# soedinglab/plass

Hardware: AMD Instinct MI355X
Metric: read-overlaps/s per assembly iteration (higher is better)
Workload: dtype u8/u64 (integer hash, byte compare; f32 ratios)

## Files before the change

plass_amd/csrc/asm_rules.hpp:

```cpp
#pragma once
#include <cmath>
#include <cstdlib>
#if defined(__HIPCC__)
#define PLASSHIP_AR_HD __host__ __device__ __forceinline__
#else
#define PLASSHIP_AR_HD static inline __attribute__((always_inline))
#endif
namespace plasship {

struct AlnCoords { int qStart, qEnd, dbStart, dbEnd; };
struct DiagSpan { bool hit = false; unsigned qo = 0, to = 0, len = 0; };

PLASSHIP_AR_HD int alnLengthOf(int qStart, int qEnd, int dbStart, int dbEnd) {
    const int aq = (qStart == -1) ? 0 : qStart, ad = (dbStart == -1) ? 0 : dbStart;
    const int dq = abs(qEnd - aq), dd = abs(dbEnd - ad);
    return (dq > dd ? dq : dd) + 1;
}
PLASSHIP_AR_HD int rawScoreOfBits(int bitScore, double ln2, double logK, double lambda) {
    return (int) (fma((double) bitScore, ln2, logK) / lambda + 0.5);
}
template <typename S> PLASSHIP_AR_HD int scorePerCol100(S score, unsigned alnLen) {
    const float scorePerCol = (float) score / (float) ((double) alnLen + 0.5);
    return (int) (scorePerCol * 100);
}
PLASSHIP_AR_HD DiagSpan diagonalSpan(int diag, unsigned qLen, unsigned tLen) {
    const unsigned dist = (unsigned) abs(diag);
    DiagSpan s;
    if (diag >= 0 && dist < qLen) { s.hit = true; s.qo = dist; s.len = tLen < qLen - dist ? tLen : qLen - dist; }
    else if (diag < 0 && dist < tLen) { s.hit = true; s.to = dist; s.len = tLen - dist < qLen ? tLen - dist : qLen; }
    return s;
}
template <typename F> PLASSHIP_AR_HD void forEachWrap(unsigned d16, unsigned qLen, unsigned tLen, F &&f) {
    for (unsigned j = 1; j <= 1u + tLen / 32768u; j++) {
        const int real = (int) (d16 - j * 65536u);
        const DiagSpan s = diagonalSpan(real, qLen, tLen);
        if (s.hit) f(real, s);
    }
    for (unsigned j = 0; j <= qLen / 65536u; j++) {
        const int real = (int) (j * 65536u + d16);
        const DiagSpan s = diagonalSpan(real, qLen, tLen);
        if (s.hit) f(real, s);
    }
}
PLASSHIP_AR_HD AlnCoords alnOnDiagonal(int diag, int startPos, int endPos) {
    const int dist = abs(diag);
    AlnCoords c;
    if (diag >= 0) { c.qStart = startPos + dist; c.qEnd = endPos + dist; c.dbStart = startPos; c.dbEnd = endPos; }
    else { c.qStart = startPos; c.qEnd = endPos; c.dbStart = startPos + dist; c.dbEnd = endPos + dist; }
    return c;
}
PLASSHIP_AR_HD float rescoredSeqId(int ids, int qStart, int qEnd) {
    return (float) ids / ((float) qEnd - (float) qStart);
}
PLASSHIP_AR_HD bool isBranchType(int qStart, int qEnd, unsigned qLen, int dbStart, int dbEnd, unsigned dbLen) {
    const bool notBoth = !(dbStart == 0 && qStart == 0);
    const bool rightStart = dbStart == 0 && (dbEnd != (int) dbLen - 1);
    const bool leftStart = qStart == 0 && (qEnd != (int) qLen - 1);
    return (rightStart || leftStart) && notBoth;
}
PLASSHIP_AR_HD unsigned rightFragLen(unsigned tLen, int dbEnd) { return tLen - ((unsigned) dbEnd + 1); }
PLASSHIP_AR_HD bool canExtendRight(unsigned fragR, int qEnd, unsigned qLen) { return fragR > 0 && (unsigned) qEnd == (qLen - 1); }
PLASSHIP_AR_HD bool canExtendLeft(int dbStart, int dbEnd, unsigned tLen) { return dbStart > 0 && (unsigned) dbEnd == (tLen - 1); }
PLASSHIP_AR_HD bool deferredRight(unsigned fragR, int qEnd, unsigned qLen, unsigned rightOff) {
    return fragR > rightOff && (unsigned) qEnd == (qLen - 1) && rightOff > 0;
}
PLASSHIP_AR_HD bool deferredLeft(int dbStart, int dbEnd, unsigned tLen, unsigned leftOff) {
    return dbStart > (int) leftOff && (unsigned) dbEnd == (tLen - 1) && leftOff > 0;
}
PLASSHIP_AR_HD AlnCoords mirrorReverseHit(int qStart, int qEnd, int dbStart, int dbEnd, unsigned dbLen) {
    AlnCoords c;
    c.qStart = qEnd; c.qEnd = qStart;
    c.dbStart = (int) (dbLen - (unsigned) dbEnd - 1); c.dbEnd = (int) (dbLen - (unsigned) dbStart - 1);
    return c;
}

}
```

plass_amd/csrc/assemble.hip:

```cpp
#include "common.hpp"
#include "device_utils.hpp"
#include "posterior_class.hpp"
#include "ref_rules.hpp"
#include "asm_rules.hpp"
#include "host_util.hpp"
#include <algorithm>
#include <memory>
#include <cstring>

namespace plasship {

struct Item {
    uint32_t target; int32_t score; uint32_t alnLength; float seqId;
    int32_t qStart, qEnd; uint32_t qLen; int32_t dbStart, dbEnd; uint32_t dbLen;
    uint32_t state;
    uint32_t pad;
};

struct AsmArgs {
    SeqView s;
    const uint64_t *qoff; const AlnRec *recs;
    Item *items;
    const uint64_t *arenaOff;
    const uint32_t *leftCap;
// ... 894 lines not shown
                        curLen += fragLen; rightOff += fragLen;
                        if (GUIDED) {
                            const unsigned aaFrag = (tLen / 3 - dbEnd / 3) - 1;
                            if (aaStart + aaLen + aaFrag > a.aaArenaOff[id + 1] - a.aaArenaOff[id]) atomicAdd(&a.stats[12], 1ull);
                            else { copyBytesSerial(aaBuf + aaStart + aaLen, aaT + dbEnd / 3 + 1, aaFrag); aaLen += aaFrag; }
                        }
                        used[nUsed++] = best.target;
                    } else if (qStart == 0 && dbEnd == (tLen - 1)) {
                        if (leftOff > 0) { def[nDef++] = bi; continue; }
                        const unsigned fragLen = dbStart;
                        if (curLen + fragLen >= a.maxSeqLen) { brokeOut = true; break; }
                        if (!copied) { job[0].dst = buf + curStart; job[0].src = orig; job[0].n = origLen; job[0].rev = 0; copied = true; }
                        curStart -= fragLen;
                        job[2].dst = buf + curStart; job[2].src = rev ? tSeq + (tLen - dbStart) : tSeq; job[2].n = fragLen; job[2].rev = rev ? 1u : 0u;
                        curLen += fragLen; leftOff += fragLen;
                        if (GUIDED) {
                            const unsigned aaFrag = fragLen / 3 + ((aaT[0] == '*') ? 1u : 0u);
                            if (aaFrag > aaStart) atomicAdd(&a.stats[12], 1ull);
                            else { aaStart -= aaFrag; copyBytesSerial(aaBuf + aaStart, aaT, aaFrag); aaLen += aaFrag; }
                        }
                        used[nUsed++] = best.target;
                    }
                }
                if (cmp.abort) active = false;
            }
#pragma unroll
            for (int k = 0; k < 3; k++) {
                unsigned long long m = __ballot(job[k].n > 0);
                while (m) {
                    const int j = __ffsll((long long) m) - 1; m &= m - 1;
                    char *dst = bcast(job[k].dst, j); const char *src = bcast(job[k].src, j);
                    const unsigned n = bcast(job[k].n, j), rv = bcast(job[k].rev, j);
                    if (rv) copyRevCompWave(dst, src, n, sComp, lane); else copyBytesG<64>(dst, src, n, lane);
                }
            }
            waveMemSync();
            if (active) {
                if (leftOff > 0 || rightOff > 0) couldExtend = true;
                if (brokeOut && nHeap > 0) active = false;
            }
            querySeqLen = (unsigned) curLen;
            const char *qs = buf + curStart;
            const uint32_t myDef = active ? nDef : 0u;
            uint32_t maxDef = myDef;
#pragma unroll
            for (int o = 32; o > 0; o >>= 1) maxDef = max(maxDef, (uint32_t) __shfl_xor((int) maxDef, o, 64));
            for (uint32_t d = 0; d < maxDef; d++) {
                const bool mine = d < myDef && !cmp.abort;
                uint32_t found = 0; Item x; memset(&x, 0, sizeof(x));
                const char *tSeq = nullptr; unsigned tLen = 0; int diag = 0; DiagSpan sp;
                if (mine) {
                    found = def[d];
                    x = it[found];
                    tSeq = a.s.data + seqOff(a.s, x.target);
                    tLen = seqLen(a.s, x.target);
                    diag = (int) ((unsigned) x.qStart + leftOff) - x.dbStart;
                    sp = diagonalSpan(diag, querySeqLen, tLen);
                }
                int startPos = -1, endPos = -1, sc = 0, ids = 0;
                unsigned long long m = __ballot(mine && sp.hit && sp.len > 0);
                while (m) {
                    const int j = __ffsll((long long) m) - 1; m &= m - 1;
                    const char *jq = bcast(qs + sp.qo, j); const char *jt = bcast(tSeq, j);
                    const unsigned jTo = bcast(sp.to, j), jLen = bcast(sp.len, j), jTLen = bcast(tLen, j), jRev = bcast((unsigned) x.pad, j);
                    unsigned first = 0, last = 0; int s = 0, idn = 0;
                    if (jRev) scoreColumnsRevWave(jq, jt, jTLen - 1 - jTo, jLen, smat, sComp, lane, first, last, s, idn);
                    else scoreColumnsG<64>(jq, jt + jTo, jLen, smat, lane, first, last, s, idn);
                    s = waveReduceSum(s); idn = waveReduceSum(idn);
                    if (lane == j) { startPos = (int) first; endPos = (int) last; sc = s; ids = idn; }
                }
                if (mine) {
                    const unsigned score = (unsigned) max(sc, 0);
                    qResc++; qRescRes += sp.len;
                    const AlnCoords c = alnOnDiagonal(diag, startPos, endPos);
                    const float seqId = rescoredSeqId(ids, c.qStart, c.qEnd);
                    x.seqId = seqId; x.qLen = querySeqLen; x.dbLen = tLen; x.alnLength = sp.len;
                    x.score = scorePerCol100(score, x.alnLength);
                    x.qStart = c.qStart; x.qEnd = c.qEnd; x.dbStart = c.dbStart; x.dbEnd = c.dbEnd;
                    it[found] = x;
                    if (seqId >= a.seqIdThr) heapPush(hp, nHeap, found, it, cmp);
                }
            }
            active = active && nHeap > 0 && !cmp.abort;
        }
        if (valid) {
            if (cmp.abort) a.redoList[atomicAdd(a.redoCount, 1u)] = id;
            else {
                nAln += h; nQRes += seqLen(a.s, id); nResc += qResc; nRescRes += qRescRes;
                for (uint32_t i = 0; i < nUsed; i++) atomicOr(&a.flags[used[i]], 0x80u);
                if (couldExtend) {
                    atomicOr(&a.flags[id], 0x20u); a.newLen[id] = (uint32_t) curLen; a.newStart[id] = aoff + curStart;
                    if (GUIDED) { a.aaNewLen[id] = (uint32_t) aaLen; a.aaNewStart[id] = a.aaArenaOff[id] + aaStart; }
                    nExt++;
                }
            }
        }
    }
    nExt = waveReduceSumU64(nExt); nResc = waveReduceSumU64(nResc); nRescRes = waveReduceSumU64(nRescRes); nAln = waveReduceSumU64(nAln); nQRes = waveReduceSumU64(nQRes);
    if (laneId() == 0) {
        if (nExt) atomicAdd(&a.stats[0], nExt); if (nResc) atomicAdd(&a.stats[1], nResc); if (nRescRes) atomicAdd(&a.stats[2], nRescRes);
        if (nAln) { atomicAdd(&a.stats[3], nAln); atomicAdd(&a.stats[4], nQRes); atomicAdd(&a.stats[5], nRescRes); }
    }
}

template <int G> __device__ __forceinline__ int groupSum(int v) {
    v = rowSum<(G < 16 ? G : 16)>(v);
#pragma unroll
    for (int o = 16; o < G; o <<= 1) v += __shfl_xor(v, o, G);
    return v;
}
template <int G> __device__ __forceinline__ unsigned long long groupMax(unsigned long long v) {
    v = rowMax<(G < 16 ? G : 16)>(v);
#pragma unroll
    for (int o = 16; o < G; o <<= 1) { const unsigned long long ok = __shfl_xor(v, o, G); v = (ok > v) ? ok : v; }
    return v;
}
template <int G> __device__ __forceinline__ uint32_t groupRank(uint32_t mine) {
    if (G == 8) return rowCountLess8(mine);
    uint32_t r = rowCountLess16(mine, mine, false);
#pragma unroll
    for (int o = 16; o < G; o += 16) r += rowCountLess16((uint32_t) __shfl_xor((int) mine, o, G), mine, true);
    return r;
}
template <int G> __device__ __forceinline__ unsigned long long groupBallot(bool p) {
    const unsigned long long m = __ballot(p);
    if (G == 64) return m;
    return (m >> ((laneId() / G) * G)) & ((1ULL << G) - 1ULL);
}

template <int G>
__device__ __forceinline__ Rescored rescoreOnDiagonalG(const char *q, unsigned qLen, const char *t, unsigned tLen, int diagonal,
                                                       const signed char *smat, int gl) {
    Rescored r; r.startPos = -1; r.endPos = -1; r.score = 0; r.diagonalLen = 0; r.idExcl = 0;
    const unsigned dist = (unsigned) abs(diagonal);
    unsigned qo, to, len;
    if (diagonal >= 0 && dist < qLen) { qo = dist; to = 0; len = min(tLen, qLen - dist); }
    else if (diagonal < 0 && dist < tLen) { qo = 0; to = dist; len = min(tLen - dist, qLen); }
    else return r;
    r.diagonalLen = len;
    if (len == 0) return r;
    unsigned first, last;
    int s = 0, ids = 0;
    scoreColumnsG<G>(q + qo, t + to, len, smat, gl, first, last, s, ids);
    s = groupSum<G>(s); ids = groupSum<G>(ids);
    r.score = (unsigned) max(s, 0); r.startPos = (int) first; r.endPos = (int) last; r.idExcl = ids;
    return r;
}

constexpr int ASM8_WPE = 5;
template <int G, int WPE>
__global__ __launch_bounds__(256) __attribute__((amdgpu_waves_per_eu(WPE, WPE))) void assembleGroupKernel(AsmArgs a) {
    __shared__ signed char smat[123 * 123 + 7];
    stageScoreTable(smat, a.mat, 256);
    __syncthreads();
    const int gl = threadIdx.x & (G - 1);
    const uint32_t groupsTotal = gridDim.x * (256 / G);
    const uint32_t nWork = (G == 64) ? a.nMid : ((G == 32) ? a.nMid32 : ((G == 16) ? a.nSmall : a.nNarrow));
    unsigned long long nExt = 0, nResc = 0, nRescRes = 0, nAln = 0, nQRes = 0;
    const uint32_t *workList = (G == 64) ? a.midList : ((G == 32) ? a.mid32List : ((G == 16) ? a.smallList : a.narrowList));
    auto loadWord = [&](uint32_t pid) -> uint64_t {
        uint64_t v = 0;
        if (pid != 0xFFFFFFFFu) {
            if (gl == 0) v = a.qoff[pid]; else if (gl == 1) v = a.qoff[pid + 1]; else if (gl == 2) v = a.arenaOff[pid]; else if (gl == 3) v = a.s.offLen[pid]; else if (gl == 4) v = a.leftCap[pid];
        }
        return v;
    };
    uint32_t w = blockIdx.x * (256 / G) + threadIdx.x / G;
    uint32_t idNext = (w < nWork) ? workList[w] : 0xFFFFFFFFu;
    uint64_t wordNext = loadWord(idNext);
    uint32_t idAhead = (w + groupsTotal < nWork) ? workList[w + groupsTotal] : 0xFFFFFFFFu;
    for (; w < nWork; w += groupsTotal) {
        const uint32_t id = idNext;
        const uint64_t h0 = __shfl(wordNext, 0, G), h1 = __shfl(wordNext, 1, G), aoff = __shfl(wordNext, 2, G), qOffLen = __shfl(wordNext, 3, G), qLeftCap = __shfl(wordNext, 4, G);
        idNext = idAhead; wordNext = loadWord(idNext);
        idAhead = (w + 2u * groupsTotal < nWork) ? workList[w + 2u * groupsTotal] : 0xFFFFFFFFu;
        const uint32_t h = (uint32_t) (h1 - h0);
        const char *orig = a.s.data + (qOffLen >> 24);
        unsigned querySeqLen = (unsigned) ((uint32_t) qOffLen & 0xFFFFFFu);
        if (gl == 0) { nAln += h; nQRes += querySeqLen; }
        uint32_t xTarget = 0xFFFFFFFFu, xAlnLen = 0, xQLen = 0, xDbLen = 0, xState = 2, xTLen = 0; uint64_t xTOff = 0;
        int xScore = 0, xQStart = 0, xQEnd = 0, xDbStart = 0, xDbEnd = 0;
        if ((uint32_t) gl < h) {
            const AlnRec r = a.recs[h0 + gl];
            xTarget = r.target;
            xAlnLen = (uint32_t) alnLengthOf(r.qStart, r.qEnd, r.dbStart, r.dbEnd);
            xScore = scorePerCol100(rawScoreOfBits(r.bitScore, a.ln2, a.logK, a.lambda), xAlnLen);
            xQStart = r.qStart; xQEnd = r.qEnd; xQLen = (uint32_t) r.qLen; xDbStart = r.dbStart; xDbEnd = r.dbEnd; xDbLen = (uint32_t) r.dbLen;
            xState = (xTarget == id || !r.accepted) ? 2u : 0u;
            const bool branchType = ((xDbStart == 0 && xDbEnd != (int) xDbLen - 1) || (xQStart == 0 && xQEnd != (int) xQLen - 1)) && !(xDbStart == 0 && xQStart == 0);
            if (xState == 0 && branchType) { xTOff = seqOff(a.s, xTarget); xTLen = seqLen(a.s, xTarget); }
        }
        const uint32_t tRank = groupRank<G>(xTarget);
        char *buf = a.arena + aoff;
        uint64_t curStart = qLeftCap;
        copyBytesG<G>(buf + curStart, orig, querySeqLen, gl);
        uint64_t curLen = querySeqLen;
        bool couldExtend = false;
        uint32_t inQueue = (uint32_t) __popcll(groupBallot<G>(xState == 0));
        while (inQueue > 0) {
            unsigned leftOff = 0, rightOff = 0;
            bool brokeOut = false;
            if (xState == 1) xState = 2;
            unsigned long long key = 0;
            bool rType = false, lType = false, rBranch = false, lBranch = false;
            unsigned fragR = 0;
            if (xState == 0) {
                key = ((unsigned long long) ((uint32_t) xScore ^ 0x80000000u) << 32) | ((unsigned long long) xAlnLen << 6) | (unsigned long long) (63u - tRank);
                if (isBranchType(xQStart, xQEnd, xQLen, xDbStart, xDbEnd, xDbLen)) {
                    if (xDbStart == 0) { rBranch = true; fragR = rightFragLen(xTLen, xDbEnd); rType = canExtendRight(fragR, xQEnd, querySeqLen); }
                    else if (xQStart == 0) { lBranch = true; lType = canExtendLeft(xDbStart, xDbEnd, xTLen); }
                }
            }
            const unsigned long long bestR = groupMax<G>(rType ? key : 0ULL), bestL = groupMax<G>(lType ? key : 0ULL);
            const bool rFirst = bestR != 0 && bestR > bestL;
            const bool isR = rType && key == bestR, isL = lType && key == bestL;
            auto extendRight = [&]() {
                const int bi = __ffsll((long long) groupBallot<G>(isR)) - 1;
                const char *tSeq = a.s.data + __shfl(xTOff, bi, G);
                const uint32_t bTarget = __shfl(xTarget, bi, G);
                const unsigned fragLen = __shfl(fragR, bi, G), dbEnd = (unsigned) __shfl(xDbEnd, bi, G);
                copyBytesG<G>(buf + curStart + curLen, tSeq + dbEnd + 1, fragLen, gl);
                curLen += fragLen; rightOff += fragLen;
                if (gl == 0) atomicOr(&a.flags[bTarget], 0x80u);
            };
            if (rFirst) extendRight();
            if (bestL != 0) {
                const int bi = __ffsll((long long) groupBallot<G>(isL)) - 1;
                const unsigned fragLen = (unsigned) __shfl(xDbStart, bi, G);
                if (curLen + fragLen >= a.maxSeqLen) brokeOut = true;
                else {
                    const char *tSeq = a.s.data + __shfl(xTOff, bi, G);
                    const uint32_t bTarget = __shfl(xTarget, bi, G);
                    curStart -= fragLen;
                    copyBytesG<G>(buf + curStart, tSeq, fragLen, gl);
                    curLen += fragLen; leftOff += fragLen;
                    if (gl == 0) atomicOr(&a.flags[bTarget], 0x80u);
                }
            }
            if (bestR != 0 && !rFirst && !brokeOut) extendRight();
            if (xState == 0 && (!brokeOut || key >= bestL)) {
                uint32_t st = 2;
                if (!(isR && (rFirst || !brokeOut)) && !isL) {
                    if (rBranch) { if (deferredRight(fragR, xQEnd, querySeqLen, rightOff)) st = 1; }
                    else if (lBranch) { if (deferredLeft(xDbStart, xDbEnd, xTLen, leftOff)) st = 1; }
                }
                xState = st;
            }
            inQueue = (uint32_t) __popcll(groupBallot<G>(xState == 0));
            if (leftOff > 0 || rightOff > 0) couldExtend = true;
            if (brokeOut && inQueue > 0) break;
            querySeqLen = (unsigned) curLen;
            const char *qs = buf + curStart;
            unsigned long long deferred = groupBallot<G>(xState == 1);
            if (deferred) waveMemSync();
            if (G >= 32 && (uint32_t) __popcll(deferred) >= a.ownLaneMin) {
                if (xState == 1) {
                    const char *tSeq = a.s.data + xTOff;
                    const int diag = (int) ((unsigned) xQStart + leftOff) - xDbStart;
                    const DiagSpan sp = diagonalSpan(diag, querySeqLen, xTLen);
                    unsigned first = 0, last = 0; int sc = 0, ids = 0; int startPos = -1, endPos = -1;
                    if (sp.hit && sp.len > 0) { scoreColumnsSerial(qs + sp.qo, tSeq + sp.to, sp.len, smat, first, last, sc, ids); startPos = (int) first; endPos = (int) last; }
                    const unsigned score = (unsigned) max(sc, 0);
                    nResc += 1; nRescRes += sp.len;
                    const AlnCoords c = alnOnDiagonal(diag, startPos, endPos);
                    xQLen = querySeqLen; xDbLen = xTLen; xAlnLen = sp.len; xScore = scorePerCol100(score, sp.len);
                    xQStart = c.qStart; xQEnd = c.qEnd; xDbStart = c.dbStart; xDbEnd = c.dbEnd;
                    xState = (rescoredSeqId(ids, c.qStart, c.qEnd) >= a.seqIdThr) ? 0u : 2u;
                }
                deferred = 0;
            }
            while (deferred) {
                const int dl = __ffsll((long long) deferred) - 1;
                deferred &= deferred - 1;
                const int dqs = __shfl(xQStart, dl, G), dds = __shfl(xDbStart, dl, G);
                const char *tSeq = a.s.data + __shfl(xTOff, dl, G);
                const unsigned tLen = __shfl(xTLen, dl, G);
                const int diag = (int) ((unsigned) dqs + leftOff) - dds;
                const Rescored rs = rescoreOnDiagonalG<G>(qs, querySeqLen, tSeq, tLen, diag, smat, gl);
                nResc += (gl == 0); nRescRes += (gl == 0) ? rs.diagonalLen : 0;
                const AlnCoords c = alnOnDiagonal(diag, rs.startPos, rs.endPos);
                const float seqId = rescoredSeqId(rs.idExcl, c.qStart, c.qEnd);
                if (gl == dl) {
                    xQLen = querySeqLen; xDbLen = tLen; xAlnLen = rs.diagonalLen; xScore = scorePerCol100(rs.score, rs.diagonalLen);
                    xQStart = c.qStart; xQEnd = c.qEnd; xDbStart = c.dbStart; xDbEnd = c.dbEnd;
                    xState = (seqId >= a.seqIdThr) ? 0u : 2u;
                }
            }
            inQueue = (uint32_t) __popcll(groupBallot<G>(xState == 0));
        }
        if (couldExtend) {
            if (gl == 0) { atomicOr(&a.flags[id], 0x20u); a.newLen[id] = (uint32_t) curLen; a.newStart[id] = aoff + curStart; nExt++; }
        }
    }
    nExt = waveReduceSumU64(nExt); nResc = waveReduceSumU64(nResc); nRescRes = waveReduceSumU64(nRescRes); nAln = waveReduceSumU64(nAln); nQRes = waveReduceSumU64(nQRes);
    if (laneId() == 0) {
        if (nExt) atomicAdd(&a.stats[0], nExt); if (nResc) atomicAdd(&a.stats[1], nResc); if (nRescRes) atomicAdd(&a.stats[2], nRescRes);
        const int tier = (G <= 16) ? 0 : 1;
        if (nAln) { atomicAdd(&a.stats[3 + 3 * tier], nAln); atomicAdd(&a.stats[4 + 3 * tier], nQRes); atomicAdd(&a.stats[5 + 3 * tier], nRescRes); }
    }
}

__global__ __launch_bounds__(256) void arenaSumKernel(const AlnRec *__restrict__ recs, uint64_t nAln, uint64_t maxSeqLen, unsigned long long *__restrict__ qSum,
                                                      unsigned long long *__restrict__ qSumAa, uint32_t *__restrict__ qCan, int mirror) {
    const int lane = laneId();
    for (uint64_t i = (uint64_t) blockIdx.x * blockDim.x + threadIdx.x; i < nAln; i += (uint64_t) gridDim.x * blockDim.x) {
        const AlnRec r = recs[i];
        const uint32_t id = r.query;
        uint32_t add = 0, addAa = 0; bool can = false;
        if (r.target != id && r.accepted) {
            add = (uint32_t) r.dbLen; addAa = (uint32_t) r.dbLen / 3 + 2;
            AlnCoords c; c.qStart = r.qStart; c.qEnd = r.qEnd; c.dbStart = r.dbStart; c.dbEnd = r.dbEnd;
            if (mirror && c.qStart > c.qEnd) c = mirrorReverseHit(r.qStart, r.qEnd, r.dbStart, r.dbEnd, (unsigned) r.dbLen);
            if (isBranchType(c.qStart, c.qEnd, (unsigned) r.qLen, c.dbStart, c.dbEnd, (unsigned) r.dbLen)) {
                if (c.dbStart == 0) can = canExtendRight(rightFragLen((unsigned) r.dbLen, c.dbEnd), c.qEnd, (unsigned) r.qLen);
                else if (c.qStart == 0) can = canExtendLeft(c.dbStart, c.dbEnd, (unsigned) r.dbLen) && ((uint64_t) r.qLen + (uint64_t) c.dbStart < maxSeqLen);
            }
        }
        const unsigned long long act = __ballot(1);
        const uint32_t prevId = (uint32_t) __shfl_up((int) id, 1, 64);
        const bool head = lane == 0 || prevId != id;
        const unsigned long long heads = __ballot(head), cans = __ballot(can);
        const int segStart = 63 - __clzll((long long) (heads & (lane == 63 ? ~0ULL : ((2ULL << lane) - 1ULL))));
        const unsigned long long later = lane == 63 ? 0ULL : (heads & ~((2ULL << lane) - 1ULL));
        const int segEnd = (later ? __ffsll((long long) later) - 1 : (int) __popcll(act)) - 1;
#pragma unroll
        for (int d = 1; d < 64; d <<= 1) {
            const uint32_t t = (uint32_t) __shfl_up((int) add, d, 64), ta = (uint32_t) __shfl_up((int) addAa, d, 64);
            if (lane - d >= segStart) { add += t; addAa += ta; }
        }
        if (lane == segEnd) {
            const unsigned long long seg = (segEnd == 63 ? ~0ULL : ((2ULL << segEnd) - 1ULL)) & ~((1ULL << segStart) - 1ULL);
            if (add) atomicAdd(&qSum[id], (unsigned long long) add);
            if (qSumAa && addAa) atomicAdd(&qSumAa[id], (unsigned long long) addAa);
            if (cans & seg) atomicOr(&qCan[id], 1u);
        }
    }
}
constexpr int N_TIERS = 5;
constexpr uint8_t TIER_NARROW = 4, TIER_NONE = 0xFF;
__global__ void arenaSizeKernel(SeqView s, const uint64_t *__restrict__ qoff, const unsigned long long *__restrict__ qSum, const unsigned long long *__restrict__ qSumAa,
                                const uint32_t *__restrict__ qCan, uint32_t *__restrict__ leftCap,
                                uint64_t *__restrict__ bytes, int nuclTiers, uint64_t threadBytes,
                                uint8_t *__restrict__ tierOf,
                                const uint32_t *__restrict__ aaLen, uint32_t *__restrict__ aaLeftCap, uint64_t *__restrict__ aaBytes) {
    for (uint32_t id = blockIdx.x * blockDim.x + threadIdx.x; id < s.n; id += gridDim.x * blockDim.x) {
        int tier = -1;
        const uint64_t sum = qSum[id], sumAa = aaBytes ? qSumAa[id] : 0;
        const bool can = qCan[id] != 0;
        leftCap[id] = (uint32_t) std::min<uint64_t>(sum, 0xFFFFFFFFull);
        const uint64_t slice = (sum && can) ? (2 * sum + s.len[id] + 40) : 0;
        bytes[id] = slice;
        if (aaBytes) { aaLeftCap[id] = (uint32_t) std::min<uint64_t>(sumAa, 0xFFFFFFFFull); aaBytes[id] = (sum && can) ? (2 * sumAa + aaLen[id] + 8) : 0; }
        if (sum && can) { const uint64_t h = qoff[id + 1] - qoff[id]; tier = nuclTiers ? ((h <= 256 && slice <= threadBytes) ? 0 : 1) : (h <= 8 ? (int) TIER_NARROW : (h <= 16 ? 0 : (h <= 32 ? 1 : (h <= 64 ? 2 : 3)))); }
        tierOf[id] = (tier < 0) ? TIER_NONE : (uint8_t) tier;
    }
}
static_assert(SCAN_TILE < (1 << 12) && N_TIERS * 12 <= 64 && SCAN_BLOCK == 256, "tier counters of a tile: 12-bit fields of one 64-bit word");
__device__ __forceinline__ unsigned long long tierField(uint8_t t) { return (t < N_TIERS) ? (1ull << (12 * t)) : 0ull; }
__device__ __forceinline__ uint64_t loadTierBytes(const uint8_t *__restrict__ tierOf, uint32_t n, uint64_t base) {
    static_assert(SCAN_ITEMS == 8, "eight tier bytes per thread");
    if (base + 8 <= n) return *reinterpret_cast<const uint64_t *>(tierOf + base);
    uint64_t w = ~0ull;
    for (int k = 0; k < 8; k++) if (base + k < n) w = (w & ~(0xFFull << (8 * k))) | ((uint64_t) tierOf[base + k] << (8 * k));
    return w;
}
__global__ __launch_bounds__(SCAN_BLOCK) void tierCountKernel(const uint8_t *__restrict__ tierOf, uint32_t n, uint64_t *__restrict__ partial, uint32_t nTiles) {
    __shared__ unsigned long long wsum[SCAN_BLOCK / WAVE];
    const uint64_t w = loadTierBytes(tierOf, n, (uint64_t) blockIdx.x * SCAN_TILE + (uint64_t) threadIdx.x * SCAN_ITEMS);
    unsigned long long s = 0;
#pragma unroll
    for (int k = 0; k < 8; k++) s += tierField((uint8_t) (w >> (8 * k)));
    s = waveReduceSumU64(s);
    if (laneId() == 0) wsum[threadIdx.x >> 6] = s;
    __syncthreads();
    if (threadIdx.x < N_TIERS) {
        unsigned long long t = 0;
        for (int j = 0; j < SCAN_BLOCK / WAVE; j++) t += wsum[j];
        partial[(size_t) threadIdx.x * (nTiles + 1) + blockIdx.x] = (t >> (12 * threadIdx.x)) & 0xFFFull;
    }
}
struct TierLists { uint32_t *list[N_TIERS]; };
__global__ __launch_bounds__(SCAN_BLOCK) void tierListKernel(const uint8_t *__restrict__ tierOf, uint32_t n, const uint64_t *__restrict__ tileOff, uint32_t nTiles,
                                                             TierLists lists) {
    __shared__ unsigned long long wsum[SCAN_BLOCK / WAVE];
    const uint64_t base = (uint64_t) blockIdx.x * SCAN_TILE + (uint64_t) threadIdx.x * SCAN_ITEMS;
    const uint64_t w = loadTierBytes(tierOf, n, base);
    unsigned long long s = 0;
#pragma unroll
    for (int k = 0; k < 8; k++) s += tierField((uint8_t) (w >> (8 * k)));
    const unsigned long long incl = waveInclusiveScanU64(s);
    const int wv = threadIdx.x >> 6;
    if (laneId() == 63) wsum[wv] = incl;
    __syncthreads();
    unsigned long long run = incl - s;
#pragma unroll
    for (int j = 0; j < SCAN_BLOCK / WAVE; j++) if (j < wv) run += wsum[j];
    if (s == 0) return;
#pragma unroll
    for (int k = 0; k < 8; k++) {
        const uint8_t t = (uint8_t) (w >> (8 * k));
        if (t < N_TIERS) {
            const uint64_t *row = tileOff + (size_t) t * (nTiles + 1);
            const uint32_t pos = (uint32_t) (row[blockIdx.x] - row[0]) + (uint32_t) ((run >> (12 * t)) & 0xFFFull);
            uint32_t *list = (t == 0) ? lists.list[0] : ((t == 1) ? lists.list[1] : ((t == 2) ? lists.list[2] : ((t == 3) ? lists.list[3] : lists.list[4])));
            list[pos] = (uint32_t) (base + k);
            run += 1ull << (12 * t);
        }
    }
}

constexpr int NW_CLASSES = 16;
__device__ __forceinline__ int nuclWorkClass(uint64_t slice) {
    const int k = 63 - __clzll((long long) (slice | 1ull));
    return NW_CLASSES - 1 - (min(max(k, 9), 9 + NW_CLASSES - 1) - 9);
}
__global__ __launch_bounds__(256) void nuclClassCountKernel(const uint32_t *__restrict__ list, uint32_t n, const uint64_t *__restrict__ bytes, uint32_t *__restrict__ counts) {
    __shared__ uint32_t sCnt[NW_CLASSES];
    if (threadIdx.x < NW_CLASSES) sCnt[threadIdx.x] = 0;
    __syncthreads();
    for (uint32_t i = blockIdx.x * 256 + threadIdx.x; i < n; i += gridDim.x * 256) atomicAdd(&sCnt[nuclWorkClass(bytes[list[i]])], 1u);
    __syncthreads();
    if (threadIdx.x < NW_CLASSES && sCnt[threadIdx.x]) atomicAdd(&counts[threadIdx.x], sCnt[threadIdx.x]);
}
__global__ __launch_bounds__(256) void nuclClassScatterKernel(const uint32_t *__restrict__ list, uint32_t n, const uint64_t *__restrict__ bytes, uint32_t *__restrict__ counts,
                                                              uint32_t *__restrict__ out) {
    __shared__ uint32_t sCnt[NW_CLASSES], sBase[NW_CLASSES];
    for (uint32_t t0 = blockIdx.x * 256; t0 < n; t0 += gridDim.x * 256) {
        if (threadIdx.x < NW_CLASSES) sCnt[threadIdx.x] = 0;
        __syncthreads();
        const uint32_t i = t0 + threadIdx.x;
        uint32_t id = 0, r = 0; int c = -1;
        if (i < n) { id = list[i]; c = nuclWorkClass(bytes[id]); r = atomicAdd(&sCnt[c], 1u); }
        __syncthreads();
        if (threadIdx.x < NW_CLASSES) {
            uint32_t before = 0;
            for (int k = 0; k < (int) threadIdx.x; k++) before += counts[k];
            sBase[threadIdx.x] = before + (sCnt[threadIdx.x] ? atomicAdd(&counts[NW_CLASSES + threadIdx.x], sCnt[threadIdx.x]) : 0u);
        }
        __syncthreads();
        if (c >= 0) out[sBase[c] + r] = id;
        __syncthreads();
    }
}

__global__ void outLenKernel(SeqView s, const uint32_t *__restrict__ flags, const uint32_t *__restrict__ newLen, int keepTarget,
                             uint64_t *__restrict__ outBytes, uint32_t *__restrict__ keep, uint64_t *__restrict__ appBytes) {
    for (uint32_t id = blockIdx.x * blockDim.x + threadIdx.x; id < s.n; id += gridDim.x * blockDim.x) {
        const uint32_t f = flags[id];
        uint64_t b = 0, ap = 0; uint32_t k = 0;
        if (f & 0x20u) { b = (uint64_t) newLen[id] + 2; k = 1; ap = b; }
        else if (keepTarget || !(f & 0x80u)) { b = (uint64_t) s.len[id] + 2; k = 1; }
        outBytes[id] = b; keep[id] = k;
        if (appBytes) appBytes[id] = ap;
    }
}

__global__ __launch_bounds__(256) void appendOutKernel(SeqView s, const uint32_t *__restrict__ flags, const uint32_t *__restrict__ newLen,
                                                       const uint64_t *__restrict__ newStart, const char *arena,
                                                       const uint64_t *__restrict__ appOff, uint64_t heapBase, const uint32_t *__restrict__ keep,
                                                       const uint64_t *__restrict__ keepPos, const uint32_t *__restrict__ inKey,
                                                       char *heap, uint64_t *__restrict__ outOffArr, uint32_t *__restrict__ outLen, uint32_t *__restrict__ outKey,
                                                       unsigned char *__restrict__ changedOut) {
    const int lane = laneId();
    for (uint32_t id0 = (blockIdx.x * 256 + (threadIdx.x & ~63u)); id0 < s.n; id0 += gridDim.x * 256) {
        const uint32_t id = id0 + (uint32_t) lane;
        bool ext = false; uint32_t L = 0; uint64_t srcOff = 0, o = 0;
        if (id < s.n && keep[id]) {
            ext = (flags[id] & 0x20u) != 0;
            if (ext) { L = newLen[id]; o = heapBase + appOff[id]; srcOff = newStart[id]; }
            else { L = s.len[id]; o = s.off[id]; }
            const uint64_t j = keepPos[id];
            outOffArr[j] = o; outLen[j] = L; outKey[j] = inKey[id];
            if (changedOut) changedOut[j] = ext ? 1 : 0;
        }
        unsigned long long m = __ballot(ext);
        while (m) {
            const int src = __ffsll((long long) m) - 1;
            m &= m - 1;
            const uint32_t cl = (uint32_t) __shfl((int) L, src, 64);
            const uint64_t co = (uint64_t) __shfl((unsigned long long) o, src, 64), cs = (uint64_t) __shfl((unsigned long long) srcOff, src, 64);
            const char *from = arena + cs; char *dst = heap + co;
            for (unsigned p = 8u * (unsigned) lane; p < cl; p += 512u) {
                const uint64_t x = loadU64Unaligned(from + p);
                if (p + 8 <= cl) storeU64Unaligned(dst + p, x); else storeTail(dst + p, x, cl - p);
            }
            if (lane == 0) { dst[cl] = '\n'; dst[cl + 1] = '\0'; }
        }
    }
}

__global__ __launch_bounds__(256) void originOutKernel(uint32_t n, const uint32_t *__restrict__ flags, const uint32_t *__restrict__ keep, const uint64_t *__restrict__ keepPos,
                                                       const uint32_t *__restrict__ srcOrigin, uint32_t *__restrict__ outOrigin) {
    for (uint32_t id = blockIdx.x * 256 + threadIdx.x; id < n; id += gridDim.x * 256)
        if (keep[id]) outOrigin[keepPos[id]] = (flags[id] & 0x20u) ? 0xFFFFFFFFu : (srcOrigin ? srcOrigin[id] : id);
}

template <int G, int U>
__global__ __launch_bounds__(256) void writeOutKernel(SeqView s, const uint32_t *__restrict__ flags, const uint32_t *__restrict__ newLen,
                                                      const uint64_t *__restrict__ newStart, const char *__restrict__ arena,
                                                      const uint64_t *__restrict__ outOff, const uint32_t *__restrict__ keep,
                                                      const uint64_t *__restrict__ keepPos, const uint32_t *__restrict__ inKey,
                                                      char *__restrict__ outData, uint64_t *__restrict__ outOffArr, uint32_t *__restrict__ outLen, uint32_t *__restrict__ outKey,
                                                      unsigned char *__restrict__ changedOut) {
    const int gl = threadIdx.x & (G - 1);
    constexpr int groupsPerBlock = 256 / G;
    const uint32_t stride = gridDim.x * groupsPerBlock;
    for (uint32_t id0 = blockIdx.x * groupsPerBlock + (threadIdx.x / G); id0 < s.n; id0 += stride * U) {
        uint32_t L[U]; const char *src[U]; uint64_t o[U]; bool k[U]; uint64_t w[U];
#pragma unroll
        for (int u = 0; u < U; u++) {
            const uint32_t id = id0 + (uint32_t) u * stride;
            k[u] = id < s.n && keep[id] != 0;
            L[u] = 0; src[u] = s.data; o[u] = 0;
            if (k[u]) {
                const uint32_t f = flags[id]; const uint32_t l0 = s.len[id]; const uint64_t o0 = s.off[id];
                o[u] = outOff[id];
                const bool ext = (f & 0x20u) != 0;
                L[u] = ext ? newLen[id] : l0;
                src[u] = ext ? (arena + newStart[id]) : (s.data + o0);
            }
        }
#pragma unroll
        for (int u = 0; u < U; u++) w[u] = (k[u] && 8u * (unsigned) gl < L[u]) ? loadU64Unaligned(src[u] + 8 * gl) : 0ULL;
#pragma unroll
        for (int u = 0; u < U; u++) {
            if (!k[u]) continue;
            const uint32_t id = id0 + (uint32_t) u * stride;
            const unsigned i = 8u * (unsigned) gl;
            char *dst = outData + o[u];
            if (i + 8 <= L[u]) storeU64Unaligned(dst + i, w[u]);
            else if (i < L[u]) storeTail(dst + i, w[u], L[u] - i);
            for (unsigned p = i + 8u * G; p < L[u]; p += 8u * G) {
                const uint64_t x = loadU64Unaligned(src[u] + p);
                if (p + 8 <= L[u]) storeU64Unaligned(dst + p, x);
                else storeTail(dst + p, x, L[u] - p);
            }
            if (gl == 0) {
                dst[L[u]] = '\n'; dst[L[u] + 1] = '\0';
                const uint64_t j = keepPos[id];
                outOffArr[j] = o[u]; outLen[j] = L[u]; outKey[j] = inKey[id];
                if (changedOut) changedOut[j] = (flags[id] & 0x20u) ? 1 : 0;
            }
        }
    }
}
struct __attribute__((aligned(16))) ExtMeta { uint32_t id, len, aaLen, pad; };
__global__ void extMarkKernel(uint32_t n, const uint32_t *__restrict__ flags, const uint32_t *__restrict__ newLen, const uint32_t *__restrict__ aaNewLen,
                              uint32_t *__restrict__ keep, uint64_t *__restrict__ bytes, uint64_t *__restrict__ aaBytes) {
    for (uint32_t id = blockIdx.x * blockDim.x + threadIdx.x; id < n; id += gridDim.x * blockDim.x) {
        const bool ext = (flags[id] & 0x20u) != 0;
        keep[id] = ext ? 1u : 0u; bytes[id] = ext ? newLen[id] : 0u;
        if (aaBytes) aaBytes[id] = ext ? aaNewLen[id] : 0u;
    }
}
__global__ __launch_bounds__(256) void extPackKernel(uint32_t n, const uint32_t *__restrict__ keep, const uint64_t *__restrict__ pos, const uint64_t *__restrict__ off,
                                                     const uint64_t *__restrict__ aaOff, const uint32_t *__restrict__ newLen, const uint64_t *__restrict__ newStart,
                                                     const char *__restrict__ arena, const uint32_t *__restrict__ aaNewLen, const uint64_t *__restrict__ aaNewStart,
                                                     const char *__restrict__ aaArena, ExtMeta *__restrict__ meta, char *__restrict__ packed, char *__restrict__ aaPacked) {
    const int G = 16, groupsPerBlock = 256 / G;
    const int gl = threadIdx.x & (G - 1);
    for (uint32_t id = blockIdx.x * groupsPerBlock + (threadIdx.x / G); id < n; id += gridDim.x * groupsPerBlock) {
        if (!keep[id]) continue;
        const uint32_t L = newLen[id];
        copyBytesG<G>(packed + off[id], arena + newStart[id], L, gl);
        uint32_t La = 0;
        if (aaPacked) { La = aaNewLen[id]; copyBytesG<G>(aaPacked + aaOff[id], aaArena + aaNewStart[id], La, gl); }
        if (gl == 0) { ExtMeta m; m.id = id; m.len = L; m.aaLen = La; m.pad = 0; meta[pos[id]] = m; }
    }
}
__global__ void extLensKernel(const ExtMeta *__restrict__ meta, uint64_t m, uint64_t *__restrict__ lens, uint64_t *__restrict__ aaLens) {
    for (uint64_t j = (uint64_t) blockIdx.x * blockDim.x + threadIdx.x; j < m; j += (uint64_t) gridDim.x * blockDim.x) { lens[j] = meta[j].len; if (aaLens) aaLens[j] = meta[j].aaLen; }
}
__global__ void extMergeKernel(const ExtMeta *__restrict__ meta, uint64_t m, const uint64_t *__restrict__ start, const uint64_t *__restrict__ aaStart,
                               uint32_t *__restrict__ flags, uint32_t *__restrict__ newLen, uint64_t *__restrict__ newStart,
                               uint32_t *__restrict__ aaNewLen, uint64_t *__restrict__ aaNewStart) {
    for (uint64_t j = (uint64_t) blockIdx.x * blockDim.x + threadIdx.x; j < m; j += (uint64_t) gridDim.x * blockDim.x) {
        const ExtMeta e = meta[j];
        atomicOr(&flags[e.id], 0x20u); newLen[e.id] = e.len; newStart[e.id] = start[j];
        if (aaStart) { aaNewLen[e.id] = e.aaLen; aaNewStart[e.id] = aaStart[j]; }
    }
}
__global__ void orFlagsKernel(const uint32_t *__restrict__ all, uint32_t n, int world, uint32_t *__restrict__ flags) {
    for (uint32_t id = blockIdx.x * blockDim.x + threadIdx.x; id < n; id += gridDim.x * blockDim.x) {
        uint32_t f = flags[id];
        for (int r = 0; r < world; r++) f |= all[(size_t) r * n + id] & 0x80u;
        flags[id] = f;
    }
}

__global__ void maxU32Kernel(const uint32_t *__restrict__ v, uint64_t n, uint32_t *__restrict__ out) {
    uint32_t m = 0;
    for (uint64_t i = (uint64_t) blockIdx.x * blockDim.x + threadIdx.x; i < n; i += (uint64_t) gridDim.x * blockDim.x) m = max(m, v[i]);
    m = (uint32_t) waveReduceMax((int) m);
    if (laneId() == 0) atomicMax(out, m);
}

}
using namespace plasship;

static int ambTableInsert(plasship_ctx *ctx, const uint32_t *tuples, uint32_t n) {
    auto hashOf = [](const uint32_t *k) { return (k[0] * 0x9E3779B1u) ^ (k[1] * 0x85EBCA77u) ^ (k[2] * 0xC2B2AE3Du) ^ (k[3] * 0x27D4EB2Fu); };
    auto insertInto = [&](std::vector<uint32_t> &keys, std::vector<uint8_t> &vals, uint32_t slots, const uint32_t *k, uint8_t v) -> bool {
        uint32_t s = hashOf(k) & (slots - 1);
        while (keys[4 * (size_t) s] != 0) {
            if (memcmp(&keys[4 * (size_t) s], k, 16) == 0) return false;
            s = (s + 1) & (slots - 1);
        }
        memcpy(&keys[4 * (size_t) s], k, 16); vals[s] = v;
        return true;
    };
    size_t have = 0;
    for (size_t i = 0; i < ctx->ambVals.size(); i++) have += ctx->ambKeys[4 * i] != 0;
    uint32_t slots = ctx->ambSlots ? ctx->ambSlots : 1024;
    while ((have + n) * 2 > slots) slots *= 2;
    if (slots != ctx->ambSlots) {
        std::vector<uint32_t> nk((size_t) slots * 4, 0); std::vector<uint8_t> nv(slots, 0);
        for (size_t i = 0; i < ctx->ambVals.size(); i++)
            if (ctx->ambKeys[4 * i] != 0) insertInto(nk, nv, slots, &ctx->ambKeys[4 * i], ctx->ambVals[i]);
        ctx->ambKeys.swap(nk); ctx->ambVals.swap(nv); ctx->ambSlots = slots;
        ctx->d_ambKeys.release(); ctx->d_ambVals.release();
        if (ctx->d_ambKeys.alloc((size_t) slots * 16) != hipSuccess || ctx->d_ambVals.alloc(slots) != hipSuccess) { setError("plasship_assemble: out of device memory"); return PLASSHIP_ERR_DEVICE; }
    }
    for (uint32_t i = 0; i < n; i++) {
        const uint32_t *k = tuples + 4 * (size_t) i;
        if (k[0] == 0) continue;
        insertInto(ctx->ambKeys, ctx->ambVals, slots, k, (uint8_t) nuclPosteriorClass(k[0], k[1], k[2], k[3]));
    }
    PH_COPY_SYNC(ctx->stream, ctx->d_ambKeys.p, ctx->ambKeys.data(), (size_t) slots * 16, hipMemcpyHostToDevice);
    PH_COPY_SYNC(ctx->stream, ctx->d_ambVals.p, ctx->ambVals.data(), slots, hipMemcpyHostToDevice);
    return PLASSHIP_OK;
}

static int buildOutputDBImpl(plasship_ctx *ctx, const plasship_seqdb *db, const uint32_t *dFlags, const uint32_t *dNewLen, const uint64_t *dNewStart,
                             const char *dArena, int keepTarget, void *dTmp, size_t tmpBytes, plasship_seqdb **out,
                             const void *dExtra, void *hExtra, size_t extraBytes, hipEvent_t doneEvent, int mode, bool noAppend = false) {
    hipStream_t st = ctx->stream;
    const uint32_t N = (uint32_t) db->n;
    const SeqView sv = db->view();
    const bool useHeaps = mode == 0 && tuneInt("DBHEAP", 1) == 1;
    const bool mayAppend = useHeaps && db->heap != nullptr && !noAppend;
    DevBuf dOutBytes, dKeep, dOutOff, dKeepPos, dMaxLen, dAppBytes, dAppOff;
    if (dOutBytes.alloc(((size_t) N + 1) * 8) != hipSuccess || dKeep.alloc(((size_t) N + 1) * 4) != hipSuccess || dOutOff.alloc(((size_t) N + 2) * 8) != hipSuccess ||
        dKeepPos.alloc(((size_t) N + 2) * 8) != hipSuccess || dMaxLen.alloc(4) != hipSuccess ||
        (mayAppend && (dAppBytes.alloc(((size_t) N + 1) * 8) != hipSuccess || dAppOff.alloc(((size_t) N + 2) * 8) != hipSuccess))) { setError("plasship_assemble: out of device memory"); return PLASSHIP_ERR_DEVICE; }
    if (N) hipLaunchKernelGGL(outLenKernel, dim3(std::min<uint32_t>((N + 255) / 256, 8192)), dim3(256), 0, st, sv, dFlags, dNewLen, keepTarget, dOutBytes.as<uint64_t>(), dKeep.as<uint32_t>(),
                              mayAppend ? dAppBytes.as<uint64_t>() : (uint64_t *) nullptr);
    if (exclusiveScanU64(st, dOutBytes.as<uint64_t>(), dOutOff.as<uint64_t>(), N, dTmp, tmpBytes) ||
        exclusiveScanU32(st, dKeep.as<uint32_t>(), dKeepPos.as<uint64_t>(), N, dTmp, tmpBytes) ||
        (mayAppend && exclusiveScanU64(st, dAppBytes.as<uint64_t>(), dAppOff.as<uint64_t>(), N, dTmp, tmpBytes))) { setError("plasship_assemble: scan failed"); return PLASSHIP_ERR_DEVICE; }
    uint64_t outBytes = 0, outN = 0, appTotal = 0;
    PH_CHECK(hipMemcpyAsync(&outBytes, dOutOff.as<uint64_t>() + N, 8, hipMemcpyDeviceToHost, st));
    PH_CHECK(hipMemcpyAsync(&outN, dKeepPos.as<uint64_t>() + N, 8, hipMemcpyDeviceToHost, st));
    if (mayAppend) PH_CHECK(hipMemcpyAsync(&appTotal, dAppOff.as<uint64_t>() + N, 8, hipMemcpyDeviceToHost, st));
    PH_CHECK(plasship::streamSync(st));
    PH_CHECK(hipGetLastError());
    std::unique_ptr<plasship_seqdb> holder(new plasship_seqdb());
    plasship_seqdb *o = holder.get();
    o->dbtype = db->dbtype; o->n = (size_t) outN; o->dataBytes = outBytes; o->residues = outBytes - 2 * outN; o->hostIndexValid = false;
    if (o->d_off.allocLong((outN + 1) * 8) != hipSuccess || o->d_len.allocLong((outN + 1) * 4) != hipSuccess || o->d_key.allocLong((outN + 1) * 4) != hipSuccess) {
        setError("plasship_assemble: out of device memory for the output DB's index"); return PLASSHIP_ERR_DEVICE;
    }
    if (outN && mode == 0) {
        if (o->d_changed.allocLong((size_t) outN) != hipSuccess) { setError("plasship_assemble: out of device memory"); return PLASSHIP_ERR_DEVICE; }
        o->ancestorGen = db->gen;
        if (outN == N) o->parentGen = db->gen;
    }
    if (outN && mode == 0 && ctx->kmPosCache.valid && ctx->kmPosCache.gen != 0) {
        const uint64_t anchor = ctx->kmPosCache.gen;
        const bool isAnchor = db->gen == anchor, descends = !isAnchor && db->originGen == anchor && db->d_origin.p != nullptr;
        if (isAnchor || descends) {
            if (o->d_origin.allocLong((size_t) outN * 4) != hipSuccess) { setError("plasship_assemble: out of device memory"); return PLASSHIP_ERR_DEVICE; }
            o->originGen = anchor;
            hipLaunchKernelGGL(originOutKernel, dim3(std::min<uint32_t>((N + 255) / 256, 4096)), dim3(256), 0, st, N, dFlags, (const uint32_t *) dKeep.as<uint32_t>(), (const uint64_t *) dKeepPos.as<uint64_t>(),
                               descends ? (const uint32_t *) db->d_origin.as<uint32_t>() : (const uint32_t *) nullptr, o->d_origin.as<uint32_t>());
        }
    }
    bool append = false; uint64_t heapBase = 0;
    if (mayAppend) {
        uint64_t cur = db->heap->used.load();
        while (cur + appTotal + 64 <= db->heap->buf.bytes) {
            if (db->heap->used.compare_exchange_weak(cur, cur + appTotal)) { heapBase = cur; append = true; break; }
        }
    }
    if (append) {
        o->heap = db->heap; o->contiguous = false;
        if (N) hipLaunchKernelGGL(appendOutKernel, dim3(std::min<uint32_t>((N + 255) / 256, (uint32_t) ctx->numCU * 16u)), dim3(256), 0, st, sv, dFlags, dNewLen, dNewStart, dArena,
                                  (const uint64_t *) dAppOff.as<uint64_t>(), heapBase, (const uint32_t *) dKeep.as<uint32_t>(), (const uint64_t *) dKeepPos.as<uint64_t>(), (const uint32_t *) db->d_key.as<uint32_t>(),
                                  db->heap->buf.as<char>(), o->d_off.as<uint64_t>(), o->d_len.as<uint32_t>(), o->d_key.as<uint32_t>(), o->d_changed.as<unsigned char>());
    } else {
        char *dst = nullptr;
        if (useHeaps && !noAppend) {
            o->heap = std::make_shared<SeqHeap>();
            const uint64_t cap = outBytes + std::min<uint64_t>(outBytes, (uint64_t) tuneInt("DBHEAP_GB", 16) << 30) + 4096;
            if (o->heap->buf.allocLong(cap) == hipSuccess) { o->heap->used = outBytes; dst = o->heap->buf.as<char>(); }
            else o->heap.reset();
        }
        if (!dst) {
            if (o->d_data.allocLong(outBytes + 64) != hipSuccess) {
                size_t fr = 0, tt = 0; (void) hipMemGetInfo(&fr, &tt);
                setError("plasship_assemble: out of device memory for the output DB (" + std::to_string(outBytes) + " bytes, " + std::to_string(outN) + " sequences; device free " + std::to_string(fr) + " of " + std::to_string(tt) + ")"); return PLASSHIP_ERR_DEVICE;
            }
            dst = o->d_data.as<char>();
        }
        o->contiguous = true;
        PH_CHECK(hipMemsetAsync(dst + outBytes, 0, 64, st));
        if (N) {
            const unsigned woGrid = std::min<uint32_t>((N + 15) / 16, (uint32_t) ctx->numCU * 16u);
            hipLaunchKernelGGL((writeOutKernel<8, 1>), dim3(woGrid), dim3(256), 0, st, sv, dFlags, dNewLen,
                               dNewStart, dArena, dOutOff.as<uint64_t>(), dKeep.as<uint32_t>(), dKeepPos.as<uint64_t>(), db->d_key.as<uint32_t>(),
                               dst, o->d_off.as<uint64_t>(), o->d_len.as<uint32_t>(), o->d_key.as<uint32_t>(), o->d_changed.as<unsigned char>());
        }
    }
    PH_CHECK(hipMemcpyAsync(o->d_off.as<uint64_t>() + outN, &outBytes, 8, hipMemcpyHostToDevice, st));
    PH_CHECK(hipMemsetAsync(dMaxLen.p, 0, 4, st));
    if (outN) hipLaunchKernelGGL(maxU32Kernel, dim3(std::min<uint64_t>((outN + 255) / 256, 1024)), dim3(256), 0, st, o->d_len.as<uint32_t>(), outN, dMaxLen.as<uint32_t>());
    uint32_t maxLen = 0;
    if (doneEvent) PH_CHECK(hipEventRecord(doneEvent, st));
    PH_CHECK(hipMemcpyAsync(&maxLen, dMaxLen.p, 4, hipMemcpyDeviceToHost, st));
    if (dExtra) PH_CHECK(hipMemcpyAsync(hExtra, dExtra, extraBytes, hipMemcpyDeviceToHost, st));
    PH_CHECK(plasship::streamSync(st));
    PH_CHECK(hipGetLastError());
    o->maxEntryLen = maxLen + 2;
    o->buildAppendedBytes = append ? appTotal : 0; o->buildCopiedBytes = append ? 0 : outBytes;
    *out = holder.release();
    return PLASSHIP_OK;
}
int plasship::buildOutputDB(plasship_ctx *ctx, const plasship_seqdb *db, const uint32_t *dFlags, const uint32_t *dNewLen, const uint64_t *dNewStart,
                            const char *dArena, int keepTarget, void *dTmp, size_t tmpBytes, plasship_seqdb **out,
                            const void *dExtra, void *hExtra, size_t extraBytes, hipEvent_t doneEvent, bool noAppend) {
    return buildOutputDBImpl(ctx, db, dFlags, dNewLen, dNewStart, dArena, keepTarget, dTmp, tmpBytes, out, dExtra, hExtra, extraBytes, doneEvent, 0, noAppend);
}
int plasship::packedCopyOf(plasship_ctx *ctx, const plasship_seqdb *db, std::unique_ptr<plasship_seqdb> &out) {
    const uint32_t N = (uint32_t) db->n;
    DevBuf dFlags, dTmp; const size_t tmpBytes = exclusiveScanTmpBytes((size_t) N + 2);
    if (dFlags.alloc(((size_t) N + 1) * 4) != hipSuccess || dTmp.alloc(tmpBytes) != hipSuccess) { setError("plasship: out of device memory while packing a sequence DB"); return PLASSHIP_ERR_DEVICE; }
    PH_CHECK(hipMemsetAsync(dFlags.p, 0, ((size_t) N + 1) * 4, ctx->stream));
    plasship_seqdb *o = nullptr;
    const int rc = buildOutputDBImpl(ctx, db, dFlags.as<uint32_t>(), nullptr, nullptr, nullptr, 1, dTmp.p, tmpBytes, &o, nullptr, nullptr, 0, nullptr, 1);
    if (rc) return rc;
    o->maxEntryLen = db->maxEntryLen;
    out.reset(o);
    return PLASSHIP_OK;
}

static int mergeExtended(plasship_ctx *ctx, uint32_t N, bool guided, int keepTarget, uint32_t *dFlags, uint32_t *dNewLen, uint64_t *dNewStart, const char *dArena,
                         uint32_t *dAaNewLen, uint64_t *dAaNewStart, const char *dAaArena, void *dTmp, size_t tmpBytes, DevBuf &gathered, DevBuf &gatheredAa) {
    hipStream_t st = ctx->stream;
    const plasship_comm *cm = commOf(ctx);
    const int W = cm->world;
    DevBuf dKeep, dBytes, dAaBytes, dPos, dOff, dAaOff;
    if (dKeep.alloc(((size_t) N + 1) * 4) != hipSuccess || dBytes.alloc(((size_t) N + 1) * 8) != hipSuccess || dPos.alloc(((size_t) N + 2) * 8) != hipSuccess ||
        dOff.alloc(((size_t) N + 2) * 8) != hipSuccess || (guided && (dAaBytes.alloc(((size_t) N + 1) * 8) != hipSuccess || dAaOff.alloc(((size_t) N + 2) * 8) != hipSuccess))) {
        setError("plasship_assemble: out of device memory"); return PLASSHIP_ERR_DEVICE;
    }
    const unsigned gridN = std::min<uint32_t>((N + 255) / 256 + 1, 8192);
    hipLaunchKernelGGL(extMarkKernel, dim3(gridN), dim3(256), 0, st, N, dFlags, dNewLen, guided ? dAaNewLen : (const uint32_t *) nullptr, dKeep.as<uint32_t>(), dBytes.as<uint64_t>(),
                       guided ? dAaBytes.as<uint64_t>() : (uint64_t *) nullptr);
    if (exclusiveScanU32(st, dKeep.as<uint32_t>(), dPos.as<uint64_t>(), N, dTmp, tmpBytes) || exclusiveScanU64(st, dBytes.as<uint64_t>(), dOff.as<uint64_t>(), N, dTmp, tmpBytes) ||
        (guided && exclusiveScanU64(st, dAaBytes.as<uint64_t>(), dAaOff.as<uint64_t>(), N, dTmp, tmpBytes))) { setError("plasship_assemble: scan failed"); return PLASSHIP_ERR_DEVICE; }
    uint64_t nExt = 0, extBytes = 0, aaExtBytes = 0;
    PH_CHECK(hipMemcpyAsync(&nExt, dPos.as<uint64_t>() + N, 8, hipMemcpyDeviceToHost, st));
    PH_CHECK(hipMemcpyAsync(&extBytes, dOff.as<uint64_t>() + N, 8, hipMemcpyDeviceToHost, st));
    if (guided) PH_CHECK(hipMemcpyAsync(&aaExtBytes, dAaOff.as<uint64_t>() + N, 8, hipMemcpyDeviceToHost, st));
    PH_CHECK(plasship::streamSync(st));
    DevBuf dMeta, dPacked, dAaPacked;
    if (dMeta.alloc(std::max<uint64_t>(nExt, 1) * sizeof(ExtMeta)) != hipSuccess || dPacked.alloc(extBytes + 64) != hipSuccess || (guided && dAaPacked.alloc(aaExtBytes + 64) != hipSuccess)) {
        setError("plasship_assemble: out of device memory"); return PLASSHIP_ERR_DEVICE;
    }
    if (N) hipLaunchKernelGGL(extPackKernel, dim3(std::min<uint32_t>((N + 15) / 16, (uint32_t) ctx->numCU * 16)), dim3(256), 0, st, N, dKeep.as<uint32_t>(), dPos.as<uint64_t>(), dOff.as<uint64_t>(),
                              guided ? dAaOff.as<uint64_t>() : (const uint64_t *) nullptr, dNewLen, dNewStart, dArena, dAaNewLen, dAaNewStart, dAaArena,
                              dMeta.as<ExtMeta>(), dPacked.as<char>(), guided ? dAaPacked.as<char>() : (char *) nullptr);
    PH_TRACE(st, "assemble: packed the extended sequences");
    DevBuf gMeta; std::vector<uint64_t> rb(W), rbMeta(W), rbSeq(W), rbAa(W);
    uint64_t M = 0;
    {
        const uint64_t mine[3] = {nExt, extBytes, aaExtBytes}; std::vector<uint64_t> all(3 * (size_t) W);
        const int rc0 = commAllgatherHost(ctx, mine, all.data(), 24); if (rc0) return rc0;
        for (int r = 0; r < W; r++) { M += all[3 * (size_t) r]; rbMeta[r] = all[3 * (size_t) r] * sizeof(ExtMeta); rbSeq[r] = all[3 * (size_t) r + 1]; rbAa[r] = all[3 * (size_t) r + 2]; }
    }
    int rc = commAllgathervBytesKnown(ctx, dMeta.p, nExt * sizeof(ExtMeta), gMeta, rbMeta); if (rc) return rc;
    rc = commAllgathervBytesKnown(ctx, dPacked.p, extBytes, gathered, rbSeq); if (rc) return rc;
    if (guided) { rc = commAllgathervBytesKnown(ctx, dAaPacked.p, aaExtBytes, gatheredAa, rbAa); if (rc) return rc; }
    PH_TRACE(st, "assemble: gathered the extended sequences");
    DevBuf dLens, dStart, dAaLens, dAaStart, dTmp2; const size_t tmp2Bytes = exclusiveScanTmpBytes(M + 2);
    if (dLens.alloc((M + 1) * 8) != hipSuccess || dStart.alloc((M + 2) * 8) != hipSuccess || dTmp2.alloc(tmp2Bytes) != hipSuccess ||
        (guided && (dAaLens.alloc((M + 1) * 8) != hipSuccess || dAaStart.alloc((M + 2) * 8) != hipSuccess))) { setError("plasship_assemble: out of device memory"); return PLASSHIP_ERR_DEVICE; }
    if (M) {
        const unsigned gridM = (unsigned) std::min<uint64_t>((M + 255) / 256, 8192);
        hipLaunchKernelGGL(extLensKernel, dim3(gridM), dim3(256), 0, st, gMeta.as<ExtMeta>(), M, dLens.as<uint64_t>(), guided ? dAaLens.as<uint64_t>() : (uint64_t *) nullptr);
        if (exclusiveScanU64(st, dLens.as<uint64_t>(), dStart.as<uint64_t>(), M, dTmp2.p, tmp2Bytes) ||
            (guided && exclusiveScanU64(st, dAaLens.as<uint64_t>(), dAaStart.as<uint64_t>(), M, dTmp2.p, tmp2Bytes))) { setError("plasship_assemble: scan failed"); return PLASSHIP_ERR_DEVICE; }
        hipLaunchKernelGGL(extMergeKernel, dim3(gridM), dim3(256), 0, st, gMeta.as<ExtMeta>(), M, dStart.as<uint64_t>(), guided ? dAaStart.as<uint64_t>() : (const uint64_t *) nullptr,
                           dFlags, dNewLen, dNewStart, dAaNewLen, dAaNewStart);
    }
    PH_TRACE(st, "assemble: merged the extended sequences");
    if (!keepTarget) {
        DevBuf gFlags;
        rc = commAllgathervBytes(ctx, dFlags, (uint64_t) N * 4, gFlags, rb); if (rc) return rc;
        if (N) hipLaunchKernelGGL(orFlagsKernel, dim3(gridN), dim3(256), 0, st, gFlags.as<uint32_t>(), N, W, dFlags);
        PH_CHECK(plasship::streamSync(st));
    }
    PH_CHECK(plasship::streamSync(st));
    PH_CHECK(hipGetLastError());
    return PLASSHIP_OK;
}

static bool asmHistOn() { return getenv("PLASSHIP_DEBUG_ASMHIST") != nullptr; }
static int asmHistRecord(hipStream_t st, uint32_t N, const uint64_t *dQoff, const uint32_t *dBigList, uint32_t nBig, const uint32_t *dRounds, const uint32_t *dCycles,
                         uint32_t cap, const uint32_t *tierQueries) {
    static int call = 0;
    std::vector<uint32_t> ids(nBig), rounds(N), cycles(N);
    std::vector<uint64_t> qoff((size_t) N + 1);
    if (nBig) PH_COPY_SYNC(st, ids.data(), dBigList, (size_t) nBig * 4, hipMemcpyDeviceToHost);
    PH_COPY_SYNC(st, qoff.data(), dQoff, ((size_t) N + 1) * 8, hipMemcpyDeviceToHost);
    PH_COPY_SYNC(st, rounds.data(), dRounds, (size_t) N * 4, hipMemcpyDeviceToHost);
    PH_COPY_SYNC(st, cycles.data(), dCycles, (size_t) N * 4, hipMemcpyDeviceToHost);
    constexpr int NH = 5, NR = 8;
    uint64_t hq[NH] = {}, hx[NH] = {}, hr[NH] = {}, hc[NH] = {}, hm[NH] = {}, rq[NR] = {}, ct = 0, over = 0, maxH = 0;
    for (uint32_t w = 0; w < nBig; w++) {
        const uint32_t id = ids[w], h = (uint32_t) (qoff[id + 1] - qoff[id]), r = rounds[id] & 0x7FFFFFFFu;
        int b = 0; while (b < NH - 1 && h > (128u << b)) b++;
        int k = 0; if (r) { k = 1; uint32_t e = 1; while (k < NR - 1 && r > e) { e <<= 1; k++; } }
        hq[b]++; hx[b] += rounds[id] >> 31; hr[b] += r; hm[b] = std::max<uint64_t>(hm[b], r); hc[b] += cycles[id]; ct += cycles[id];
        rq[k]++; over += h > cap; maxH = std::max<uint64_t>(maxH, h);
    }
    std::string s = "asmHist call " + std::to_string(call++) + " big queries " + std::to_string(nBig) + " (max h " + std::to_string(maxH) + ", over cap " +
                    std::to_string(cap) + ": " + std::to_string(over) + ") | h bins <=128,<=256,<=512,<=1024,more: queries/extended/mean rounds/max rounds/% ticks";
    for (int b = 0; b < NH; b++) {
        char t[96];
        snprintf(t, sizeof(t), " [%llu %llu %.2f %llu %.1f%%]", (unsigned long long) hq[b], (unsigned long long) hx[b], hq[b] ? (double) hr[b] / hq[b] : 0.0,
                 (unsigned long long) hm[b], ct ? 100.0 * hc[b] / ct : 0.0);
        s += t;
    }
    s += " | rounds 0,1,2,<=4,<=8,<=16,<=32,more:";
    for (int k = 0; k < NR; k++) s += " " + std::to_string(rq[k]);
    s += " | tier queries <=8,<=16,<=32,<=64,more:";
    for (int t = 0; t < 5; t++) s += " " + std::to_string(tierQueries[t]);
    fprintf(stderr, "%s\n", s.c_str());
    return PLASSHIP_OK;
}

static int assembleImpl(plasship_ctx *ctx, const plasship_seqdb *db, const plasship_seqdb *aaDb, const plasship_alns *al,
                        const plasship_assemble_params *par, plasship_seqdb **out, plasship_seqdb **outAa, plasship_assemble_stats *stats) {
    const bool guided = aaDb != nullptr;
    const bool nucl = db->dbtype == PLASSHIP_DBTYPE_NUCLEOTIDES;
    if (!nucl && db->dbtype != PLASSHIP_DBTYPE_AMINO_ACIDS) { setError("plasship_assemble: the sequence DB is neither amino acids nor nucleotides"); return PLASSHIP_ERR_ARG; }
    if (par->rescore_mode != 3) { setError("plasship_assemble: only --rescore-mode 3"); return PLASSHIP_ERR_UNSUPPORTED; }
    if (al->nQueries != db->n) { setError("plasship_assemble: alignment list does not belong to the DB"); return PLASSHIP_ERR_ARG; }
    PH_ENTER(ctx);
    hipStream_t st = ctx->stream;
    const uint32_t N = (uint32_t) db->n;
    if (nucl) { const int rcS = finishSelfAlns(ctx, al); if (rcS) return rcS; }
    const uint64_t nLines = al->nSlots;
    DevBuf dLeftCap, dBytes, dArenaOff, dTmp, dItems, dFlags, dNewLen, dNewStart, dMat, dStats, dArena;
    const size_t tmpBytes = exclusiveScanTmpBytes((size_t) N + 2);
    if (dLeftCap.alloc(((size_t) N + 1) * 4) != hipSuccess || dBytes.alloc(((size_t) N + 1) * 8) != hipSuccess || dArenaOff.alloc(((size_t) N + 2) * 8) != hipSuccess ||
        dTmp.alloc(tmpBytes) != hipSuccess || dItems.alloc(std::max<uint64_t>(nLines, 1) * sizeof(Item)) != hipSuccess || dFlags.alloc(((size_t) N + 1) * 4) != hipSuccess ||
        dNewLen.alloc(((size_t) N + 1) * 4) != hipSuccess || dNewStart.alloc(((size_t) N + 1) * 8) != hipSuccess || dMat.alloc(123 * 123) != hipSuccess || dStats.alloc(128) != hipSuccess) {
        setError("plasship_assemble: out of device memory"); return PLASSHIP_ERR_DEVICE;
    }
    PH_CHECK(hipMemsetAsync(dFlags.p, 0, ((size_t) N + 1) * 4, st));
    PH_CHECK(hipMemsetAsync(dNewLen.p, 0, ((size_t) N + 1) * 4, st));
    PH_CHECK(hipMemsetAsync(dStats.p, 0, 128, st));
    PH_CHECK(hipMemcpyAsync(dMat.p, asciiSubMat(nucl), 123 * 123, hipMemcpyHostToDevice, st));
    { const int rcOL = ensureOffLen(ctx, db); if (rcOL) return rcOL; }
    const SeqView sv = db->view();
    PH_CHECK(hipEventRecord(ctx->ev[0], st));
    const uint32_t nTiles = (uint32_t) (((size_t) N + SCAN_TILE - 1) / SCAN_TILE);
    DevBuf dBigList, dMidList, dMid32List, dSmallList, dNarrowList, dTierOf, dTierPart, dAaLeftCap, dAaBytes, dAaArenaOff, dAaArena, dAaNewLen, dAaNewStart;
    if (guided && (dAaLeftCap.alloc(((size_t) N + 1) * 4) != hipSuccess || dAaBytes.alloc(((size_t) N + 1) * 8) != hipSuccess || dAaArenaOff.alloc(((size_t) N + 2) * 8) != hipSuccess ||
                   dAaNewLen.alloc(((size_t) N + 1) * 4) != hipSuccess || dAaNewStart.alloc(((size_t) N + 1) * 8) != hipSuccess)) { setError("plasship_assemble: out of device memory"); return PLASSHIP_ERR_DEVICE; }
    if (guided) PH_CHECK(hipMemsetAsync(dAaNewLen.p, 0, ((size_t) N + 1) * 4, st));
    if (dBigList.alloc(((size_t) N + 1) * 4) != hipSuccess || dMidList.alloc(((size_t) N + 1) * 4) != hipSuccess || dMid32List.alloc(((size_t) N + 1) * 4) != hipSuccess ||
        dSmallList.alloc(((size_t) N + 1) * 4) != hipSuccess || (!nucl && dNarrowList.alloc(((size_t) N + 1) * 4) != hipSuccess) || dTierOf.alloc((size_t) N + 8) != hipSuccess ||
        dTierPart.alloc(((size_t) N_TIERS * (nTiles + 1) + 1) * 8) != hipSuccess) { setError("plasship_assemble: out of device memory"); return PLASSHIP_ERR_DEVICE; }
    DevBuf dQSum, dQSumAa, dQCan;
    if (dQSum.alloc(((size_t) N + 1) * 8) != hipSuccess || dQCan.alloc(((size_t) N + 1) * 4) != hipSuccess || (guided && dQSumAa.alloc(((size_t) N + 1) * 8) != hipSuccess)) { setError("plasship_assemble: out of device memory"); return PLASSHIP_ERR_DEVICE; }
    PH_CHECK(hipMemsetAsync(dQSum.p, 0, ((size_t) N + 1) * 8, st));
    PH_CHECK(hipMemsetAsync(dQCan.p, 0, ((size_t) N + 1) * 4, st));
    if (guided) PH_CHECK(hipMemsetAsync(dQSumAa.p, 0, ((size_t) N + 1) * 8, st));
    if (nLines) hipLaunchKernelGGL(arenaSumKernel, dim3((unsigned) std::min<uint64_t>((nLines + 255) / 256, (uint64_t) ctx->numCU * 32)), dim3(256), 0, st, al->d_recs.as<AlnRec>(), (uint64_t) nLines,
                                       (uint64_t) par->max_seq_len, dQSum.as<unsigned long long>(), guided ? dQSumAa.as<unsigned long long>() : (unsigned long long *) nullptr, dQCan.as<uint32_t>(),
                                       (nucl && !guided) ? 1 : 0);
    if (N) hipLaunchKernelGGL(arenaSizeKernel, dim3(std::min<uint32_t>((N + 255) / 256, 8192)), dim3(256), 0, st, sv, al->d_qoff.as<uint64_t>(), (const unsigned long long *) dQSum.as<unsigned long long>(),
                              (const unsigned long long *) dQSumAa.as<unsigned long long>(), (const uint32_t *) dQCan.as<uint32_t>(), dLeftCap.as<uint32_t>(), dBytes.as<uint64_t>(), nucl ? 1 : 0, (uint64_t) 1 << 30,
                              dTierOf.as<uint8_t>(),
                              guided ? aaDb->d_len.as<uint32_t>() : (const uint32_t *) nullptr, dAaLeftCap.as<uint32_t>(), guided ? dAaBytes.as<uint64_t>() : (uint64_t *) nullptr);
    if (guided && exclusiveScanU64(st, dAaBytes.as<uint64_t>(), dAaArenaOff.as<uint64_t>(), N, dTmp.p, tmpBytes)) { setError("plasship_assemble: scan failed"); return PLASSHIP_ERR_DEVICE; }
    PH_CHECK(hipMemsetAsync(dTierPart.p, 0, ((size_t) N_TIERS * (nTiles + 1) + 1) * 8, st));
    if (nTiles) hipLaunchKernelGGL(tierCountKernel, dim3(nTiles), dim3(SCAN_BLOCK), 0, st, (const uint8_t *) dTierOf.as<uint8_t>(), N, dTierPart.as<uint64_t>(), nTiles);
    if (exclusiveScanU64(st, dTierPart.as<uint64_t>(), dTierPart.as<uint64_t>(), (size_t) N_TIERS * (nTiles + 1), dTmp.p, tmpBytes)) { setError("plasship_assemble: scan failed"); return PLASSHIP_ERR_DEVICE; }
    {
        TierLists tl;
        tl.list[0] = dSmallList.as<uint32_t>(); tl.list[1] = dMid32List.as<uint32_t>(); tl.list[2] = dMidList.as<uint32_t>(); tl.list[3] = dBigList.as<uint32_t>();
        tl.list[TIER_NARROW] = dNarrowList.as<uint32_t>();
        if (nTiles) hipLaunchKernelGGL(tierListKernel, dim3(nTiles), dim3(SCAN_BLOCK), 0, st, (const uint8_t *) dTierOf.as<uint8_t>(), N, (const uint64_t *) dTierPart.as<uint64_t>(), nTiles, tl);
    }
    if (exclusiveScanU64(st, dBytes.as<uint64_t>(), dArenaOff.as<uint64_t>(), N, dTmp.p, tmpBytes)) { setError("plasship_assemble: scan failed"); return PLASSHIP_ERR_DEVICE; }
    uint64_t arenaBytes = 0, aaArenaBytes = 0;
    uint64_t rowStart[N_TIERS + 1] = {};
    if (guided) PH_CHECK(hipMemcpyAsync(&aaArenaBytes, dAaArenaOff.as<uint64_t>() + N, 8, hipMemcpyDeviceToHost, st));
    PH_CHECK(hipMemcpyAsync(&arenaBytes, dArenaOff.as<uint64_t>() + N, 8, hipMemcpyDeviceToHost, st));
    PH_CHECK(hipMemcpy2DAsync(rowStart, 8, dTierPart.p, (size_t) (nTiles + 1) * 8, 8, N_TIERS + 1, hipMemcpyDeviceToHost, st));
    PH_CHECK(plasship::streamSync(st));
    uint32_t cnts[N_TIERS];
    for (int t = 0; t < N_TIERS; t++) cnts[t] = (uint32_t) (rowStart[t + 1] - rowStart[t]);
    if (dArena.alloc(arenaBytes + 64) != hipSuccess || (guided && dAaArena.alloc(aaArenaBytes + 64) != hipSuccess)) {
        size_t fr = 0, tt = 0; (void) hipMemGetInfo(&fr, &tt);
        setError("plasship_assemble: out of device memory for the extension arena (" + std::to_string(arenaBytes) + " bytes; device free " + std::to_string(fr) + " of " + std::to_string(tt) + ")"); return PLASSHIP_ERR_DEVICE;
    }
    HostEvaluer ev(nucl, db->residues);
    AsmArgs a; memset(&a, 0, sizeof(a));
    a.s = sv; a.qoff = al->d_qoff.as<uint64_t>(); a.recs = al->d_recs.as<AlnRec>(); a.items = dItems.as<Item>(); a.arenaOff = dArenaOff.as<uint64_t>();
    a.leftCap = dLeftCap.as<uint32_t>(); a.arena = dArena.as<char>(); a.flags = dFlags.as<uint32_t>(); a.newLen = dNewLen.as<uint32_t>(); a.newStart = dNewStart.as<uint64_t>();
    a.mat = dMat.as<signed char>(); a.lambda = ev.g[0]; a.logK = ev.logK; a.ln2 = ev.ln2; a.seqIdThr = par->seq_id_thr; a.maxSeqLen = par->max_seq_len; a.rescoreMode = par->rescore_mode;
    a.ownLaneMin = 6;
    a.stats = dStats.as<unsigned long long>();
    a.smallList = dSmallList.as<uint32_t>(); a.nSmall = cnts[0];
    a.narrowList = dNarrowList.as<uint32_t>(); a.nNarrow = cnts[TIER_NARROW];
    a.mid32List = dMid32List.as<uint32_t>(); a.nMid32 = cnts[1];
    a.midList = dMidList.as<uint32_t>(); a.nMid = cnts[2];
    a.bigList = dBigList.as<uint32_t>(); a.nBig = cnts[3];
    if (!nucl && a.nBig) { const int rcS = finishSelfAlns(ctx, al, dBigList.as<uint32_t>(), a.nBig); if (rcS) return rcS; }
    std::unique_ptr<plasship_seqdb> aaPacked;
    if (guided && !aaDb->contiguous) {
        const int rcP = packedCopyOf(ctx, aaDb, aaPacked); if (rcP) return rcP;
    }
    if (guided) {
        a.aa = (aaPacked ? aaPacked.get() : aaDb)->view(); a.aaArena = dAaArena.as<char>(); a.aaArenaOff = dAaArenaOff.as<uint64_t>(); a.aaLeftCap = dAaLeftCap.as<uint32_t>();
        a.aaNewLen = dAaNewLen.as<uint32_t>(); a.aaNewStart = dAaNewStart.as<uint64_t>();
    }
    DevBuf dHeap, dNeed, dRedo[2], dCnt;
    if (nucl) {
        const uint32_t needCap = 1u << 16;
        if (dHeap.alloc(std::max<uint64_t>(nLines, 1) * 12) != hipSuccess || dNeed.alloc((size_t) needCap * 16) != hipSuccess || dRedo[0].alloc(((size_t) N + 1) * 4) != hipSuccess ||
            dRedo[1].alloc(((size_t) N + 1) * 4) != hipSuccess || dCnt.alloc(8) != hipSuccess) { setError("plasship_assemble: out of device memory"); return PLASSHIP_ERR_DEVICE; }
        a.heap = dHeap.as<uint32_t>();
        if (!ctx->d_cmpCache.p) {
            const size_t cb = (size_t) CMP_LEN * CMP_MM * CMP_LEN * CMP_MM;
            if (ctx->d_cmpCache.alloc(cb) != hipSuccess) { setError("plasship_assemble: out of device memory"); return PLASSHIP_ERR_DEVICE; }
            PH_CHECK(hipMemsetAsync(ctx->d_cmpCache.p, 0, cb, st));
        }
        a.cmpCache = ctx->d_cmpCache.as<uint8_t>();
        a.needKeys = dNeed.as<uint32_t>(); a.needCount = dCnt.as<uint32_t>(); a.needCap = needCap; a.redoCount = dCnt.as<uint32_t>() + 1;
        PH_CHECK(hipEventRecord(ctx->ev[2], st));
        uint32_t nWork = cnts[0] + cnts[1];
        for (int pass = 0; nWork > 0; pass++) {
            if (pass > 256) { setError("plasship_assemble: comparator table did not converge"); return PLASSHIP_ERR_DEVICE; }
            a.ambKeys = ctx->d_ambKeys.as<uint32_t>(); a.ambVals = ctx->d_ambVals.as<uint8_t>(); a.ambMask = ctx->ambSlots ? ctx->ambSlots - 1 : 0;
            a.redoList = dRedo[pass & 1].as<uint32_t>();
            PH_CHECK(hipMemsetAsync(dCnt.p, 0, 8, st));
            auto launchWave = [&](const uint32_t *list, uint32_t n) {
                if (!n) return;
                a.queryList = list; a.nQueryList = n;
                if (guided) hipLaunchKernelGGL(assembleNuclKernel<true>, dim3(std::min<uint32_t>(n, (uint32_t) ctx->numCU * 16)), dim3(64), 0, st, a);
                else hipLaunchKernelGGL(assembleNuclKernel<false>, dim3(std::min<uint32_t>(n, (uint32_t) ctx->numCU * 16)), dim3(64), 0, st, a);
            };
            if (pass == 0) {
                if (cnts[0]) {
                    DevBuf dCls;
                    if (dCls.alloc(2 * NW_CLASSES * 4) != hipSuccess) { setError("plasship_assemble: out of device memory"); return PLASSHIP_ERR_DEVICE; }
                    PH_CHECK(hipMemsetAsync(dCls.p, 0, 2 * NW_CLASSES * 4, st));
                    const unsigned g = std::min<uint32_t>((cnts[0] + 255) / 256, (uint32_t) ctx->numCU * 8);
                    hipLaunchKernelGGL(nuclClassCountKernel, dim3(g), dim3(256), 0, st, (const uint32_t *) dSmallList.as<uint32_t>(), cnts[0], (const uint64_t *) dBytes.as<uint64_t>(), dCls.as<uint32_t>());
                    hipLaunchKernelGGL(nuclClassScatterKernel, dim3(g), dim3(256), 0, st, (const uint32_t *) dSmallList.as<uint32_t>(), cnts[0], (const uint64_t *) dBytes.as<uint64_t>(), dCls.as<uint32_t>(),
                                       dMidList.as<uint32_t>());
                    a.queryList = dMidList.as<uint32_t>(); a.nQueryList = cnts[0];
                    const uint32_t grid = std::min<uint32_t>((cnts[0] + NT_BLOCK - 1) / NT_BLOCK, (uint32_t) ctx->numCU * 8);
                    if (guided) hipLaunchKernelGGL(assembleNuclThreadKernel<true>, dim3(grid), dim3(NT_BLOCK), 0, st, a);
                    else hipLaunchKernelGGL(assembleNuclThreadKernel<false>, dim3(grid), dim3(NT_BLOCK), 0, st, a);
                }
                launchWave(dMid32List.as<uint32_t>(), cnts[1]);
            } else launchWave(dRedo[(pass + 1) & 1].as<uint32_t>(), nWork);
            uint32_t cnt[2] = {0, 0};
            PH_CHECK(hipMemcpyAsync(cnt, dCnt.p, 8, hipMemcpyDeviceToHost, st));
            PH_CHECK(plasship::streamSync(st));
            PH_CHECK(hipGetLastError());
            nWork = cnt[1];
            if (nWork == 0) break;
            const uint32_t nNeed = std::min(cnt[0], needCap);
            if (nNeed == 0) { setError("plasship_assemble: queries aborted without a missing comparator tuple"); return PLASSHIP_ERR_DEVICE; }
            std::vector<uint32_t> need((size_t) nNeed * 4);
            PH_COPY_SYNC(ctx->stream, need.data(), dNeed.p, need.size() * 4, hipMemcpyDeviceToHost);
            const int rc = ambTableInsert(ctx, need.data(), nNeed);
            if (rc != PLASSHIP_OK) return rc;
        }
        PH_CHECK(hipEventRecord(ctx->ev[3], st));
        for (int e = 4; e <= 7; e++) PH_CHECK(hipEventRecord(ctx->ev[e], st));
    } else {
    const dim3 g16(std::min<uint32_t>((a.nSmall + 15) / 16, (uint32_t) ctx->numCU * 5u)), g64(std::min<uint32_t>((a.nMid + 3) / 4, (uint32_t) ctx->numCU * 4u));
    PH_CHECK(hipEventRecord(ctx->ev[2], st));
    if (a.nNarrow) hipLaunchKernelGGL((assembleGroupKernel<8, ASM8_WPE>), dim3(std::min<uint32_t>((a.nNarrow + 31) / 32, (uint32_t) ctx->numCU * ASM8_WPE)), dim3(256), 0, st, a);
    if (a.nSmall) hipLaunchKernelGGL((assembleGroupKernel<16, 5>), g16, dim3(256), 0, st, a);
    PH_CHECK(hipEventRecord(ctx->ev[3], st));
    PH_CHECK(hipEventRecord(ctx->ev[4], st));
    if (a.nMid32) hipLaunchKernelGGL((assembleGroupKernel<32, 5>), dim3(std::min<uint32_t>((a.nMid32 + 7) / 8, (uint32_t) ctx->numCU * 5u)), dim3(256), 0, st, a);
    if (a.nMid) hipLaunchKernelGGL((assembleGroupKernel<64, 4>), g64, dim3(256), 0, st, a);
    PH_CHECK(hipEventRecord(ctx->ev[5], st));
    PH_CHECK(hipEventRecord(ctx->ev[6], st));
    DevBuf dDbgRounds, dDbgCycles;
    const bool hist = asmHistOn();
    const uint32_t tierQ[5] = {a.nNarrow, a.nSmall, a.nMid32, a.nMid, a.nBig};
    if (hist) {
        if (dDbgRounds.alloc(((size_t) N + 1) * 4) != hipSuccess || dDbgCycles.alloc(((size_t) N + 1) * 4) != hipSuccess) { setError("plasship_assemble: out of device memory"); return PLASSHIP_ERR_DEVICE; }
        PH_CHECK(hipMemsetAsync(dDbgRounds.p, 0, ((size_t) N + 1) * 4, st));
        PH_CHECK(hipMemsetAsync(dDbgCycles.p, 0, ((size_t) N + 1) * 4, st));
        a.dbgRounds = dDbgRounds.as<uint32_t>(); a.dbgCycles = dDbgCycles.as<uint32_t>();
    }
    const bool onChip = tuneInt("ASMQ", 1) != 2;
    const uint32_t qCap = (uint32_t) std::max(0, std::min(tuneInt("ASMQ_CAP", (int) ASMQ_CAP), (int) ASMQ_CAP));
    const dim3 gBig(std::min<uint32_t>((a.nBig + 3) / 4, (uint32_t) ctx->numCU * 4u));
    DevBuf dOverList[2], dOverCount;
    if (a.nBig && onChip) {
        if (dOverList[0].alloc(((size_t) a.nBig + 1) * 4) != hipSuccess || dOverList[1].alloc(((size_t) a.nBig + 1) * 4) != hipSuccess || dOverCount.alloc(8) != hipSuccess) {
            setError("plasship_assemble: out of device memory"); return PLASSHIP_ERR_DEVICE;
        }
        PH_CHECK(hipMemsetAsync(dOverCount.p, 0, 8, st));
        AsmArgs q1 = a; q1.overList = dOverList[0].as<uint32_t>(); q1.overCount = dOverCount.as<uint32_t>(); q1.queueCap = qCap;
        hipLaunchKernelGGL((assembleQueueKernel<ASMQ_CAP1, 4>), dim3(std::min<uint32_t>((a.nBig + 3) / 4, (uint32_t) ctx->numCU * 4u)), dim3(256), 0, st, q1);
        AsmArgs q2 = q1; q2.bigList = dOverList[0].as<uint32_t>(); q2.bigCount = dOverCount.as<uint32_t>(); q2.overList = dOverList[1].as<uint32_t>(); q2.overCount = dOverCount.as<uint32_t>() + 1;
        hipLaunchKernelGGL((assembleQueueKernel<ASMQ_CAP, 2>), dim3(std::min<uint32_t>((a.nBig + 3) / 4, (uint32_t) ctx->numCU * 2u)), dim3(256), 0, st, q2);
        AsmArgs o = a; o.bigList = dOverList[1].as<uint32_t>(); o.bigCount = dOverCount.as<uint32_t>() + 1;
        hipLaunchKernelGGL(assembleBigKernel, gBig, dim3(256), 0, st, o);
    } else if (a.nBig) hipLaunchKernelGGL(assembleBigKernel, gBig, dim3(256), 0, st, a);
    PH_CHECK(hipEventRecord(ctx->ev[7], st));
    if (hist) { const int rcH = asmHistRecord(st, N, a.qoff, a.bigList, a.nBig, a.dbgRounds, a.dbgCycles, onChip ? qCap : 64, tierQ); if (rcH) return rcH; }
    }
    PH_TRACE(st, "assemble: extension kernels");
    plasship_seqdb *o = nullptr, *oAa = nullptr;
    unsigned long long hs[16] = {0};
    DevBuf dGathered, dGatheredAa;
    const char *arenaP = dArena.as<char>(), *aaArenaP = dAaArena.as<char>();
    if (commOf(ctx)) {
        const int rc = mergeExtended(ctx, N, guided, par->keep_target, dFlags.as<uint32_t>(), dNewLen.as<uint32_t>(), dNewStart.as<uint64_t>(), dArena.as<char>(),
                                     dAaNewLen.as<uint32_t>(), dAaNewStart.as<uint64_t>(), dAaArena.as<char>(), dTmp.p, tmpBytes, dGathered, dGatheredAa);
        if (rc != PLASSHIP_OK) return rc;
        arenaP = dGathered.as<char>(); aaArenaP = dGatheredAa.as<char>();
    }
    int rcOut = buildOutputDB(ctx, db, dFlags.as<uint32_t>(), dNewLen.as<uint32_t>(), dNewStart.as<uint64_t>(), arenaP, par->keep_target, dTmp.p, tmpBytes, &o,
                              dStats.p, hs, 128, guided ? (hipEvent_t) nullptr : ctx->ev[1], guided);
    if (rcOut != PLASSHIP_OK) return rcOut;
    std::unique_ptr<plasship_seqdb> holdO(o), holdAa;
    if (guided) {
        rcOut = buildOutputDB(ctx, aaDb, dFlags.as<uint32_t>(), dAaNewLen.as<uint32_t>(), dAaNewStart.as<uint64_t>(), aaArenaP, par->keep_target, dTmp.p, tmpBytes, &oAa,
                              nullptr, nullptr, 0, nullptr, true);
        if (rcOut != PLASSHIP_OK) return rcOut;
        holdAa.reset(oAa);
    }
    if (guided) { PH_CHECK(hipEventRecord(ctx->ev[1], st)); PH_CHECK(plasship::streamSync(st)); }
    if (hs[12]) { setError("plasship_guided_assemble: an alignment asks for a protein fragment the twin does not have (coordinates are not codon aligned)"); return PLASSHIP_ERR_ARG; }
    if (stats) {
        stats->n_extended = hs[0]; stats->n_rescored = hs[1]; stats->out_residues = o->residues;
        float ms = 0; (void) hipEventElapsedTime(&ms, ctx->ev[0], ctx->ev[1]); stats->ms_kernel = ms;
        float sum = 0;
        for (int t = 0; t < 3; t++) {
            ms = 0; (void) hipEventElapsedTime(&ms, ctx->ev[2 + 2 * t], ctx->ev[3 + 2 * t]); stats->ms_tier_kernel[t] = ms; sum += ms;
            stats->tier_alignments[t] = hs[3 + 3 * t]; stats->tier_query_residues[t] = hs[4 + 3 * t]; stats->tier_rescored_residues[t] = hs[5 + 3 * t];
        }
        stats->ms_assemble_kernel = sum;
        stats->n_alignments = al->nLines; stats->rescored_residues = hs[2];
        stats->db_appended_bytes = o->buildAppendedBytes; stats->db_copied_bytes = o->buildCopiedBytes;
    }
    *out = holdO.release();
    if (guided) *outAa = holdAa.release();
    return PLASSHIP_OK;
}

extern "C" int plasship_assemble(plasship_ctx *ctx, const plasship_seqdb *db, const plasship_alns *al,
                                 const plasship_assemble_params *par, plasship_seqdb **out, plasship_assemble_stats *stats) {
    if (!ctx || !db || !al || !par || !out) { setError("plasship_assemble: bad argument"); return PLASSHIP_ERR_ARG; }
    return commFinish(ctx, assembleImpl(ctx, db, nullptr, al, par, out, nullptr, stats));
}

extern "C" int plasship_guided_assemble(plasship_ctx *ctx, const plasship_seqdb *nucl_db, const plasship_seqdb *aa_db, const plasship_alns *al,
                                        const plasship_assemble_params *par, plasship_seqdb **out_nucl, plasship_seqdb **out_aa,
                                        plasship_assemble_stats *stats) {
    if (!ctx || !nucl_db || !aa_db || !al || !par || !out_nucl || !out_aa) { setError("plasship_guided_assemble: bad argument"); return PLASSHIP_ERR_ARG; }
    if (nucl_db->dbtype != PLASSHIP_DBTYPE_NUCLEOTIDES || aa_db->dbtype != PLASSHIP_DBTYPE_AMINO_ACIDS) { setError("plasship_guided_assemble: needs a nucleotide DB and its protein twin DB"); return PLASSHIP_ERR_ARG; }
    if (nucl_db->n != aa_db->n) { setError("plasship_guided_assemble: the two DBs differ in size"); return PLASSHIP_ERR_ARG; }
    PH_ENTER(ctx);
    bool differ = false;
    { const int rc = deviceKeysDiffer(ctx, nucl_db->d_key.as<uint32_t>(), aa_db->d_key.as<uint32_t>(), nucl_db->n, &differ); if (rc) return commFinish(ctx, rc); }
    if (differ) { setError("plasship_guided_assemble: nucleotide and protein DB have different keys"); return commFinish(ctx, PLASSHIP_ERR_ARG); }
    return commFinish(ctx, assembleImpl(ctx, nucl_db, aa_db, al, par, out_nucl, out_aa, stats));
}
```

plass_amd/csrc/common.hpp:

```cpp
#pragma once
#include <hip/hip_runtime.h>
#include <algorithm>
#include <cstdint>
#include <cstddef>
#include <cstdio>
#include <atomic>
#include <functional>
#include <memory>
#include <mutex>
#include <string>
#include <map>
#include <vector>
#include "../../include/plasship.h"

namespace plasship {

void setError(const std::string &msg);
hipError_t streamSync(hipStream_t st);
}
struct plasship_seqdb; struct plasship_ctx;
namespace plasship {
int ensureOffLen(plasship_ctx *ctx, const plasship_seqdb *db);
std::string hipErrStr(hipError_t e, const char *what, const char *file, int line);

#define PH_CHECK(call)                                                                   \
    do {                                                                                 \
        hipError_t e_ = (call);                                                          \
        if (e_ != hipSuccess) {                                                          \
            plasship::setError(plasship::hipErrStr(e_, #call, __FILE__, __LINE__));     \
            return PLASSHIP_ERR_DEVICE;                                                  \
        }                                                                                \
    } while (0)
#define PH_COPY_SYNC(st, dst, src, bytes, kind)                                          \
    do {                                                                                 \
        PH_CHECK(hipMemcpyAsync((dst), (src), (bytes), (kind), (st)));                   \
        PH_CHECK(plasship::streamSync(st));                                              \
    } while (0)

int tuneInt(const char *name, int dflt);
bool traceOn();
#define PH_TRACE(st, what)                                                                \
    do {                                                                                 \
        if (plasship::traceOn()) {                                                       \
            hipError_t e_ = plasship::streamSync(st);                                    \
            fprintf(stderr, "[plasship] %s: %s\n", (what), hipGetErrorString(e_));       \
        }                                                                                \
    } while (0)

hipError_t poolMalloc(void **p, size_t n, bool longLived = false);
void poolEnter(hipStream_t stream);
void watchEnter(const plasship_ctx *ctx);
void watchCollective(const char *what);
#define PH_ENTER(ctx)                                                                    \
    do {                                                                                 \
        PH_CHECK(hipSetDevice((ctx)->device));                                           \
        plasship::poolEnter((ctx)->stream);                                              \
        plasship::watchEnter(ctx);                                                       \
    } while (0)
void poolFree(void *p);
void poolTrim();

struct DevBuf {
    void *p = nullptr; size_t bytes = 0;
    DevBuf() {}
    DevBuf(const DevBuf &) = delete; DevBuf &operator=(const DevBuf &) = delete;
    ~DevBuf() { release(); }
    hipError_t alloc(size_t n, bool longLived = false) { release(); bytes = n; if (n == 0) { p = nullptr; return hipSuccess; } return poolMalloc(&p, n, longLived); }
    hipError_t allocLong(size_t n) { return alloc(n, true); }
    void release() { if (p) { poolFree(p); p = nullptr; } bytes = 0; }
    template <typename T> T *as() const { return reinterpret_cast<T *>(p); }
};

struct SeqView {
    const char *data;
    const uint64_t *off;
    const uint32_t *len;
    const uint64_t *offLen;
    uint32_t n;
    int nucl;
};

#ifdef __HIPCC__
__device__ __forceinline__ uint64_t seqOff(const SeqView &s, uint32_t id) { return s.offLen[id] >> 24; }
__device__ __forceinline__ uint32_t seqLen(const SeqView &s, uint32_t id) { return (uint32_t) s.offLen[id] & 0xFFFFFFu; }
#endif

struct __attribute__((aligned(8))) CandHit { uint32_t target; int32_t prefScore; uint32_t diag16; uint32_t query; };

struct AlnRec {
    uint32_t query, target;
    int32_t bitScore, rawScore;
    float seqId;
    int32_t qStart, qEnd, qLen, dbStart, dbEnd, dbLen, alnLen;
    int32_t reversed;
    int32_t accepted;
    int32_t fromText;
    int32_t btKind;
};
constexpr int32_t ALN_SELF_PENDING = 3;

}

struct plasship_ctx {
    int device = 0;
    hipStream_t stream = nullptr;
    hipEvent_t ev[16] = {};
    int numCU = 0;
    std::vector<uint32_t> ambKeys;
    std::vector<uint8_t> ambVals;
    plasship::DevBuf d_ambKeys, d_ambVals;
    plasship::DevBuf d_cmpCache;
    uint32_t ambSlots = 0;
    char *stage[2] = {nullptr, nullptr};
    hipEvent_t stageEv[2] = {nullptr, nullptr};
    size_t stageBytes = 0;
    void *pinnedTable = nullptr;
    bool hasComm = false;
    plasship_comm comm = {};
    int debugFailCollective = -1;
    struct KmCache {
        plasship::DevBuf lines; uint64_t n = 0, gen = 0; bool valid = false, seenEligible = false;
        int k = 0, alph = 0, kps = 0, ignoreMulti = 0, hashShift = 0;
    } kmCache;
    struct KmPosCache {
        plasship::DevBuf pos, slotOff, idHash; uint64_t n = 0, gen = 0; bool valid = false, seen = false, lng = false;
        int k = 0, kps = 0, ignoreMulti = 0, hashShift = 0; float scale = 0;
    } kmPosCache;
    uint64_t kmermatchCalls = 0;
    uint64_t cycKnownGen = 0, cycKnownMaxLen = 0;
    std::map<int, plasship::DevBuf> gencodeTables;
};

namespace plasship {
uint64_t newDbGeneration();
struct SeqHeap { DevBuf buf; std::atomic<uint64_t> used{0}; };
}
struct plasship_seqdb {
    int dbtype = 0;
    uint64_t gen = plasship::newDbGeneration(), parentGen = 0, ancestorGen = 0;
    plasship::DevBuf d_changed;
    uint64_t originGen = 0;
    plasship::DevBuf d_origin;
    size_t n = 0;
    uint64_t dataBytes = 0, residues = 0;
    uint32_t maxEntryLen = 0;
    plasship::DevBuf d_data, d_off, d_len, d_key;
    std::shared_ptr<plasship::SeqHeap> heap;
    bool contiguous = true;
    uint64_t buildAppendedBytes = 0, buildCopiedBytes = 0;
    const char *borrowedData = nullptr;
    const char *dataPtr() const { return heap ? heap->buf.as<char>() : borrowedData ? borrowedData : d_data.as<char>(); }
    plasship::DevBuf d_fileRank;
    mutable plasship::DevBuf d_offLen;
    mutable std::mutex offLenMu; mutable hipEvent_t offLenEv = nullptr; mutable hipStream_t offLenStream = nullptr;
    ~plasship_seqdb() { if (offLenEv) (void) hipEventDestroy(offLenEv); }
    bool hostIndexValid = false;
    std::vector<uint32_t> h_key, h_elen;
    std::vector<uint64_t> h_off;
    plasship::SeqView view() const {
        plasship::SeqView v; v.data = dataPtr(); v.off = d_off.as<uint64_t>(); v.len = d_len.as<uint32_t>(); v.offLen = d_offLen.as<uint64_t>();
        v.n = (uint32_t) n; v.nucl = (dbtype == PLASSHIP_DBTYPE_NUCLEOTIDES); return v;
    }
};

struct plasship_cands {
    bool reverseCapable = false;
    size_t nQueries = 0;
    uint64_t nHits = 0;
    uint64_t nNonSelf = 0;
    plasship::DevBuf d_qoff;
    plasship::DevBuf d_hits;
    std::vector<uint8_t> h_present;
};

namespace plasship {
struct PairList {
    size_t n = 0;
    uint64_t nClusters = 0;
    uint64_t dbGen = 0;
    DevBuf d_pairs;
};
}
struct plasship_clusters : plasship::PairList {
    plasship::DevBuf d_repOf;
};
struct plasship_merged : plasship::PairList {};

struct plasship_alns {
    size_t nQueries = 0;
    uint64_t nLines = 0;
    uint64_t nSlots = 0;
    bool sparse = false;
    mutable bool selfPending = false;
    plasship_rescore_params rsPar = {};
    bool rsSameDB = false; int rsReverseCapable = 0;
    bool nucl = false;
    bool addBacktrace = false;
    uint64_t dbResidues = 0;
    int gappedOpen = 0, gappedExtend = 0;
    plasship::DevBuf d_qoff;
    plasship::DevBuf d_recs;
    const plasship_seqdb *qdb = nullptr, *tdb = nullptr;
};

namespace plasship {
inline int refuseSharded(const plasship_ctx *ctx, const char *what) {
    if (ctx->hasComm && ctx->comm.world > 1) { setError(std::string(what) + ": not part of a sharded run (a communicator of more than one rank is set)"); return PLASSHIP_ERR_UNSUPPORTED; }
    return PLASSHIP_OK;
}
inline int refuseForeign(const char *what, const PairList *list, const plasship_seqdb *db) {
    if (list->n != db->n || list->dbGen != db->gen) { setError(std::string(what) + ": the clustering does not belong to this DB"); return PLASSHIP_ERR_ARG; }
    return PLASSHIP_OK;
}
inline int refuseWideIds(const char *what, const plasship_seqdb *db) {
    if (db->n >= 0xFFFFFFFFull) { setError(std::string(what) + ": ids are 32-bit"); return PLASSHIP_ERR_UNSUPPORTED; }
    return PLASSHIP_OK;
}
inline unsigned flatGrid(uint64_t n, int numCU) { return (unsigned) std::max<uint64_t>(1, std::min<uint64_t>((n + 255) / 256, (uint64_t) numCU * 32)); }

inline const plasship_comm *commOf(const plasship_ctx *ctx) { return ctx->hasComm ? &ctx->comm : nullptr; }
inline uint64_t ownedBegin(uint64_t n, int r, int world) { return ((uint64_t) r * n + (uint64_t) world - 1) / (uint64_t) world; }
int commAllgatherHost(plasship_ctx *ctx, const void *send, void *recv, uint64_t bytesPerRank);
int commAllReduceSumU64(plasship_ctx *ctx, uint64_t *v, size_t n);
int commAllReduceMaxU64(plasship_ctx *ctx, uint64_t *v, size_t n);
int commAllReduceMinU64(plasship_ctx *ctx, uint64_t *v, size_t n);
int commAgreeOk(plasship_ctx *ctx, bool ok, const char *what);
int commFinish(plasship_ctx *ctx, int rc);
int commAlltoallvRecords(plasship_ctx *ctx, const void *dSend, const uint64_t *sendCount, size_t recordBytes, DevBuf &recv,
                         uint64_t *recvTotal, uint64_t slackRecords, uint64_t *allTotal = nullptr);
int commAllgathervBytes(plasship_ctx *ctx, const void *dSend, uint64_t sendBytes, DevBuf &recv, std::vector<uint64_t> &recvBytes);
int commAllgathervBytesKnown(plasship_ctx *ctx, const void *dSend, uint64_t sendBytes, DevBuf &recv, const std::vector<uint64_t> &recvBytes);
int packedCopyOf(plasship_ctx *ctx, const plasship_seqdb *db, std::unique_ptr<plasship_seqdb> &out);
int buildOutputDB(plasship_ctx *ctx, const plasship_seqdb *db, const uint32_t *dFlags, const uint32_t *dNewLen, const uint64_t *dNewStart,
                  const char *dArena, int keepTarget, void *dTmp, size_t tmpBytes, plasship_seqdb **out,
                  const void *dExtra = nullptr, void *hExtra = nullptr, size_t extraBytes = 0, hipEvent_t doneEvent = nullptr, bool noAppend = false);
int stagedUpload(plasship_ctx *ctx, void *dDst, uint64_t total, const std::function<void(char *, uint64_t, uint64_t)> &produce,
                 uint64_t chunk = 0, const std::function<int(uint64_t)> *enqueued = nullptr);
int stagedDownload(plasship_ctx *ctx, const void *dSrc, uint64_t total, const std::function<bool(const char *, uint64_t, uint64_t)> &consume);
void *ctxPinnedTable(plasship_ctx *ctx, size_t bytes);
int stagedCopyToDevice(plasship_ctx *ctx, void *dDst, const void *hSrc, uint64_t bytes);
int stagedCopyToHost(plasship_ctx *ctx, void *hDst, const void *dSrc, uint64_t bytes);
int deviceKeysDiffer(plasship_ctx *ctx, const uint32_t *a, const uint32_t *b, size_t n, bool *differ);
int gencodeInfo(int table, char residues[65], char starts[65]);
int extractOrfsGencode(plasship_ctx *ctx, const plasship_seqdb *reads, const plasship_orf_params *par, plasship_seqdb **out_orfs, plasship_orfhdr **out_hdr, plasship_orf_stats *stats);
int translateNucsGencode(plasship_ctx *ctx, const plasship_seqdb *orfs, const plasship_orfhdr *hdr, const plasship_translate_params *par, plasship_seqdb **out_aa, plasship_orf_stats *stats);
int compactCsr(plasship_ctx *ctx, const char *what, const uint64_t *dInQoff, uint64_t nQ, const void *dRecs, size_t recBytes, const uint32_t *dKeep,
               uint64_t nRecs, uint64_t nKept, DevBuf &outQoff, DevBuf &outRecs);
struct HostEvaluer;
int evalueGateTable(plasship_ctx *ctx, const char *what, const plasship_seqdb *qdb, const HostEvaluer &ev, double evalThr, DevBuf &dMinScore,
                    std::vector<uint32_t> &hMinScore);
enum RescoreStat { RL_KEPT, RL_RESIDUES, RL_VISIBLE, RL_BAD, RL_NSTATS };
struct RescoreListArgs {
    const CandHit *hits;
    uint64_t nHits;
    uint32_t *keep;
    const uint32_t *minScore;
    uint32_t minScoreLen;
    const signed char *mat;
    int reverseCapable;
    double lambda, logK, ln2;
    unsigned long long *stats;
};
struct RescoreList {
    plasship_ctx *ctx; const char *what;
    const plasship_seqdb *qdb, *tdb;
    const plasship_cands *c;
    bool nucl = false; size_t slotBytes = 0;
    uint64_t residues = 0;
    DevBuf dKeep, dSlots, dStats, dMinScore, dMat;
    std::vector<uint32_t> hMinScore;
    RescoreListArgs args = {};
    uint64_t nKept = 0, nNonSelf = 0;
    int prepare(size_t slotBytes, bool wrapped, const double *evalThr, const plasship_clusters *subset);
    int collect(DevBuf &outQoff, DevBuf &outRecs, plasship_rescore_stats *stats);
};
int denseAlnsCopy(plasship_ctx *ctx, const plasship_alns *a, DevBuf &qoffBuf, DevBuf &recsBuf, const uint64_t **qoff, const AlnRec **recs);
int finishSelfAlns(plasship_ctx *ctx, const plasship_alns *a, const uint32_t *dQueryList = nullptr, uint32_t nQueryList = 0);
}
```

plass_amd/csrc/core.hip:

```cpp
#include "common.hpp"
#include "host_util.hpp"
#include "device_utils.hpp"
#include <algorithm>
#include <atomic>
#include <condition_variable>
#include <thread>
#include <memory>
#include <chrono>
#include <cstdio>
#include <cstdlib>
#include <cstring>
#include <map>
#include <mutex>
#include <numeric>
#include <unordered_map>
#include <unistd.h>

namespace plasship {
namespace {
std::mutex g_poolMu;
constexpr size_t POOL_ALIGN = 256;
struct FreeRange { size_t size; hipStream_t stream; bool mixed; };
struct Slab { char *base; size_t size; size_t used; std::map<size_t, FreeRange> free; };
struct DevicePool { std::vector<Slab> slabs; size_t total = 0; };
std::map<int, DevicePool> g_pools;
struct PoolLive { int device; int slab; size_t off, size; hipStream_t stream; };
std::unordered_map<void *, PoolLive> g_poolLive;
thread_local hipStream_t tl_poolStream = nullptr;
int g_ctxCount = 0;
std::mutex g_reserveMu; std::condition_variable g_reserveCv; int g_reserving = 0;
thread_local bool tl_isReserver = false;
struct ReserveJoin { ~ReserveJoin() { std::unique_lock<std::mutex> lk(g_reserveMu); g_reserveCv.wait(lk, [] { return g_reserving == 0; }); } } g_reserveJoin;
size_t g_poolHits = 0, g_poolMisses = 0; double g_poolMissMs = 0, g_poolMissBytes = 0;

bool takeRange(DevicePool &dp, int dev, size_t n, void **p, hipStream_t *waitFor, bool *waitAll, bool longLived) {
    int bs = -1; size_t bo = 0, bsz = ~(size_t) 0; const char *bestEnd = nullptr;
    for (size_t i = 0; i < dp.slabs.size(); i++)
        for (auto &kv : dp.slabs[i].free) {
            if (kv.second.size < n) continue;
            if (longLived) {
                const char *end = dp.slabs[i].base + kv.first + kv.second.size;
                if (bs < 0 || dp.slabs[i].size > dp.slabs[bs].size || (dp.slabs[i].size == dp.slabs[bs].size && end > bestEnd)) { bs = (int) i; bo = kv.first; bsz = kv.second.size; bestEnd = end; }
            } else if (kv.second.size < bsz) { bs = (int) i; bo = kv.first; bsz = kv.second.size; }
        }
    if (bs < 0) return false;
    Slab &sl = dp.slabs[bs];
    const FreeRange fr = sl.free[bo];
    sl.free.erase(bo);
    size_t at = bo;
    if (longLived) { at = bo + fr.size - n; if (fr.size > n) sl.free[bo] = FreeRange{fr.size - n, fr.stream, fr.mixed}; }
    else if (fr.size > n) sl.free[bo + n] = FreeRange{fr.size - n, fr.stream, fr.mixed};
    sl.used += n;
    *p = sl.base + at;
    bo = at;
    g_poolLive[*p] = PoolLive{dev, bs, bo, n, tl_poolStream};
    *waitAll = fr.mixed; *waitFor = (!fr.mixed && fr.stream != tl_poolStream) ? fr.stream : nullptr;
    return true;
}
void trimLocked(int onlyDevice) {
    int cur = 0; (void) hipGetDevice(&cur);
    for (auto &dv : g_pools) {
        if (onlyDevice >= 0 && dv.first != onlyDevice) continue;
        bool any = false; for (auto &sl : dv.second.slabs) any |= (sl.used == 0 && sl.base != nullptr);
        if (!any) continue;
        (void) hipSetDevice(dv.first); (void) hipDeviceSynchronize();
        for (auto &sl : dv.second.slabs) if (sl.used == 0 && sl.base) { (void) hipFree(sl.base); dv.second.total -= sl.size; sl.base = nullptr; sl.size = 0; sl.free.clear(); }
    }
    (void) hipSetDevice(cur);
}
}
static int poisonByte() { static const int v = [] { const char *e = getenv("PLASSHIP_POOL_POISON"); return e ? atoi(e) : -1; }(); return v; }
static hipError_t poolMallocRaw(void **p, size_t n, bool longLived);
hipError_t poolMalloc(void **p, size_t n, bool longLived) {
    const hipError_t e = poolMallocRaw(p, n, longLived);
    if (e == hipSuccess && poisonByte() >= 0) { (void) hipDeviceSynchronize(); (void) hipMemset(*p, poisonByte(), n); (void) hipDeviceSynchronize(); }
    return e;
}
void poolEnter(hipStream_t stream) { tl_poolStream = stream; }
static void poolForgetStream(hipStream_t stream) {
    std::lock_guard<std::mutex> g(g_poolMu);
    for (auto &dv : g_pools) for (auto &sl : dv.second.slabs) for (auto &kv : sl.free) if (!kv.second.mixed && kv.second.stream == stream) kv.second.stream = nullptr;
    for (auto &kv : g_poolLive) if (kv.second.stream == stream) kv.second.stream = nullptr;
    if (tl_poolStream == stream) tl_poolStream = nullptr;
}
static double poolFraction() { static const double v = [] { const char *e = getenv("PLASSHIP_POOL_FRACTION"); const double x = e ? atof(e) : 0.0; return (x > 0.05 && x <= 0.98) ? x : 0.88; }(); return v; }
static hipError_t poolMallocRaw(void **p, size_t n, bool longLived) {
    n = std::max<size_t>((n + POOL_ALIGN - 1) / POOL_ALIGN * POOL_ALIGN, POOL_ALIGN);
    int dev = 0; (void) hipGetDevice(&dev);
    const size_t MB2 = (size_t) 2 << 20;
    for (int fails = 0;;) {
        hipStream_t waitFor = nullptr; bool waitAll = false, hit = false;
        size_t slabBytes = 0;
        {
            std::lock_guard<std::mutex> g(g_poolMu);
            DevicePool &dp = g_pools[dev];
            hit = takeRange(dp, dev, n, p, &waitFor, &waitAll, longLived);
            if (hit) g_poolHits++;
            else {
                size_t fr = 0, tt = 0; (void) hipMemGetInfo(&fr, &tt);
                const size_t keepFree = (size_t) 3 << 29;
                const size_t most = std::min<size_t>((size_t) ((double) fr * poolFraction()), fr > keepFree ? fr - keepFree : 0);
                bool haveBigSlab = false;
                for (const auto &sl : dp.slabs) if (sl.base && sl.size >= ((size_t) 16 << 30)) haveBigSlab = true;
                const bool bigJob = !haveBigSlab && (dp.total >= ((size_t) 8 << 30) || n >= ((size_t) 4 << 30));
                slabBytes = bigJob ? most : std::min<size_t>(std::max<size_t>(2 * n, (size_t) 1 << 30), most);
                if (slabBytes < n || fails) slabBytes = n;
                slabBytes = (slabBytes + MB2 - 1) / MB2 * MB2;
            }
        }
        if (hit) {
            if (waitAll) (void) hipDeviceSynchronize();
            else if (waitFor) (void) plasship::streamSync(waitFor);
            return hipSuccess;
        }
        if (!tl_isReserver) {
            std::unique_lock<std::mutex> lk(g_reserveMu);
            if (g_reserving) { g_reserveCv.wait(lk, [] { return g_reserving == 0; }); continue; }
        }
        const auto t0 = std::chrono::steady_clock::now();
        void *base = nullptr;
        const hipError_t e = hipMalloc(&base, slabBytes);
        const double ms = std::chrono::duration<double, std::milli>(std::chrono::steady_clock::now() - t0).count();
        std::lock_guard<std::mutex> g(g_poolMu);
        if (e != hipSuccess) {
            (void) hipGetLastError();
            if (++fails >= 3) return e;
            trimLocked(dev);
            continue;
        }
        DevicePool &dp = g_pools[dev];
        Slab sl; sl.base = static_cast<char *>(base); sl.size = slabBytes; sl.used = 0; sl.free[0] = FreeRange{slabBytes, nullptr, false};
        size_t idx = dp.slabs.size();
        for (size_t i = 0; i < dp.slabs.size(); i++) if (!dp.slabs[i].base) { idx = i; break; }
        if (idx == dp.slabs.size()) dp.slabs.push_back(std::move(sl)); else dp.slabs[idx] = std::move(sl);
        dp.total += slabBytes; g_poolMisses++; g_poolMissMs += ms; g_poolMissBytes += (double) slabBytes;
    }
}
void poolFree(void *p) {
    std::lock_guard<std::mutex> g(g_poolMu);
    auto it = g_poolLive.find(p);
    if (it == g_poolLive.end()) { (void) hipFree(p); return; }
    const PoolLive lv = it->second;
    g_poolLive.erase(it);
    Slab &sl = g_pools[lv.device].slabs[lv.slab];
    sl.used -= lv.size;
    size_t off = lv.off, size = lv.size; hipStream_t stream = lv.stream; bool mixed = (tl_poolStream != nullptr && tl_poolStream != lv.stream);
    auto nx = sl.free.lower_bound(off);
    if (nx != sl.free.end() && off + size == nx->first) {
        if (nx->second.mixed || nx->second.stream != stream) mixed = !(nx->second.stream == nullptr && !nx->second.mixed) || mixed;
        size += nx->second.size; nx = sl.free.erase(nx);
    }
    if (nx != sl.free.begin()) {
        auto pv = std::prev(nx);
        if (pv->first + pv->second.size == off) {
            if (pv->second.mixed || pv->second.stream != stream) mixed = !(pv->second.stream == nullptr && !pv->second.mixed) || mixed;
            off = pv->first; size += pv->second.size; sl.free.erase(pv);
        }
    }
    sl.free[off] = FreeRange{size, stream, mixed};
}
void poolTrim() {
    std::lock_guard<std::mutex> g(g_poolMu);
    trimLocked(-1);
}
static thread_local std::string g_err;
int tuneInt(const char *name, int dflt) {
    char key[96]; snprintf(key, sizeof(key), "PLASSHIP_TUNE_%s", name);
    const char *e = getenv(key); const int v = e ? atoi(e) : 0;
    return v > 0 ? v : dflt;
}
static const char *const TUNE_NAMES[] = {"AGGWAVE", "AGGWAVE_CAP", "ASMQ", "ASMQ_CAP", "ROWTIER", "KMCACHE", "FORCE_LONG", "CYC_PASSES", "CYCSKIP", "SHARD_EXTRACT",
                                         "FASTA_CHUNK_MB", "DBHEAP", "DBHEAP_GB", "LAZY_SELF", "FASTQ_CHUNK_KB", "PART_BITS", "GROUP_SHAPE"};
static void reportUnknownTunes() {
    static const char PREFIX[] = "PLASSHIP_TUNE_";
    for (char **e = environ; e && *e; e++) {
        if (strncmp(*e, PREFIX, sizeof(PREFIX) - 1) != 0) continue;
        const char *x = *e + sizeof(PREFIX) - 1, *eq = strchr(x, '=');
        const std::string name(x, eq ? (size_t) (eq - x) : strlen(x));
        bool known = false;
        for (const char *k : TUNE_NAMES) known = known || name == k;
        if (!known) fprintf(stderr, "[plasship] PLASSHIP_TUNE_%s is not a switch of this build (ignored)\n", name.c_str());
    }
}
bool traceOn() { static const bool v = getenv("PLASSHIP_TRACE") != nullptr; return v; }
void setError(const std::string &msg) { g_err = msg; }
static std::atomic<unsigned long long> g_hostSyncs(0);
thread_local int tl_watchRank = -1, tl_watchWorld = 1;
thread_local const char *tl_watchLast = "none yet";
thread_local unsigned long long tl_watchCount = 0;
thread_local std::string tl_watchMsg;
void watchEnter(const plasship_ctx *ctx) {
    if (ctx && ctx->hasComm && ctx->comm.world > 1) { tl_watchRank = ctx->comm.rank; tl_watchWorld = ctx->comm.world; }
    else { tl_watchRank = -1; tl_watchWorld = 1; }
    tl_watchMsg.clear();
}
void watchCollective(const char *what) { tl_watchLast = what; tl_watchCount++; }
static double commTimeoutSeconds() { static const double v = [] { const char *e = getenv("PLASSHIP_COMM_TIMEOUT_S"); return e ? atof(e) : 300.0; }(); return v; }
hipError_t streamSync(hipStream_t st) {
    g_hostSyncs++;
    const double limit = tl_watchWorld > 1 ? commTimeoutSeconds() : 0.0;
    if (limit <= 0.0) return hipStreamSynchronize(st);
    const auto t0 = std::chrono::steady_clock::now();
    for (unsigned spins = 0;; spins++) {
        const hipError_t e = hipStreamQuery(st);
        if (e != hipErrorNotReady) return e;
        if (spins < 512) continue;
        const double el = std::chrono::duration<double>(std::chrono::steady_clock::now() - t0).count();
        if (el > limit) {
            tl_watchMsg = "sharded run, rank " + std::to_string(tl_watchRank) + " of " + std::to_string(tl_watchWorld) + ": the stream did not drain within " + std::to_string((int) limit) +
                          " s (PLASSHIP_COMM_TIMEOUT_S); last collective enqueued: " + tl_watchLast + " (#" + std::to_string(tl_watchCount) + " on this thread) - a peer that left the call, "
                          "or a link that is down (NCCL_DEBUG=INFO shows RCCL's view)";
            fprintf(stderr, "[plasship] %s\n", tl_watchMsg.c_str());
            return hipErrorNotReady;
        }
        std::this_thread::sleep_for(std::chrono::microseconds(el < 0.01 ? 20 : 200));
    }
}
std::string hipErrStr(hipError_t e, const char *what, const char *file, int line) {
    const std::string std_ = std::string("HIP error ") + hipGetErrorString(e) + " in " + what + " at " + file + ":" + std::to_string(line);
    if (!tl_watchMsg.empty()) { const std::string m = tl_watchMsg + " [" + std_ + "]"; tl_watchMsg.clear(); return m; }
    return std_;
}
__global__ void keysDifferKernel(const uint32_t *__restrict__ a, const uint32_t *__restrict__ b, uint32_t n, uint32_t *__restrict__ flag) {
    for (uint32_t i = blockIdx.x * blockDim.x + threadIdx.x; i < n; i += gridDim.x * blockDim.x) if (a[i] != b[i]) *flag = 1u;
}
int deviceKeysDiffer(plasship_ctx *ctx, const uint32_t *a, const uint32_t *b, size_t n, bool *differ) {
    DevBuf dFlag; uint32_t d = 0;
    if (dFlag.alloc(4) != hipSuccess) { setError("out of device memory"); return PLASSHIP_ERR_DEVICE; }
    PH_CHECK(hipMemsetAsync(dFlag.p, 0, 4, ctx->stream));
    if (n) hipLaunchKernelGGL(keysDifferKernel, dim3(std::min<uint32_t>(((uint32_t) n + 255) / 256, 1024)), dim3(256), 0, ctx->stream, a, b, (uint32_t) n, dFlag.as<uint32_t>());
    PH_COPY_SYNC(ctx->stream, &d, dFlag.p, 4, hipMemcpyDeviceToHost);
    *differ = d != 0;
    return PLASSHIP_OK;
}
}
using namespace plasship;

extern "C" const char *plasship_last_error(void) { return g_err.c_str(); }
extern "C" const char *plasship_version(void) { return "plasship 0.1 (gfx950)"; }

extern "C" int plasship_ctx_create(int device_ordinal, plasship_ctx **out) {
    if (!out) { setError("plasship_ctx_create: out is NULL"); return PLASSHIP_ERR_ARG; }
    static std::once_flag tunesChecked;
    std::call_once(tunesChecked, reportUnknownTunes);
    int count = 0;
    hipError_t e = hipGetDeviceCount(&count);
    if (e != hipSuccess || count == 0) {
        setError("plasship_ctx_create: no HIP device available (this library has no CPU fallback)");
        return PLASSHIP_ERR_DEVICE;
    }
    if (device_ordinal < 0) {
        const char *lr = getenv("LOCAL_RANK");
        device_ordinal = lr ? atoi(lr) % count : 0;
    }
    if (device_ordinal >= count) { setError("plasship_ctx_create: device ordinal out of range"); return PLASSHIP_ERR_ARG; }
    PH_CHECK(hipSetDevice(device_ordinal));
    std::unique_ptr<plasship_ctx> holder(new plasship_ctx());
    plasship_ctx *c = holder.get();
    c->device = device_ordinal;
    hipDeviceProp_t prop;
    PH_CHECK(hipGetDeviceProperties(&prop, device_ordinal));
    c->numCU = prop.multiProcessorCount;
    PH_CHECK(hipStreamCreateWithFlags(&c->stream, hipStreamNonBlocking));
    poolEnter(c->stream);
    for (auto &ev : c->ev) PH_CHECK(hipEventCreate(&ev));
    { std::lock_guard<std::mutex> g(g_poolMu); g_ctxCount++; }
    *out = holder.release();
    return PLASSHIP_OK;
}

extern "C" int plasship_ctx_reserve_async(plasship_ctx *ctx) {
    if (!ctx) { setError("plasship_ctx_reserve_async: ctx is NULL"); return PLASSHIP_ERR_ARG; }
    {
        std::lock_guard<std::mutex> g(g_poolMu);
        for (const auto &sl : g_pools[ctx->device].slabs) if (sl.base && sl.size >= ((size_t) 16 << 30)) return PLASSHIP_OK;
    }
    { std::lock_guard<std::mutex> lk(g_reserveMu); if (g_reserving) return PLASSHIP_OK; g_reserving = 1; }
    const int dev = ctx->device;
    std::thread([dev] {
        (void) hipSetDevice(dev);
        tl_isReserver = true;
        void *p = nullptr;
        if (poolMalloc(&p, (size_t) 4 << 30) == hipSuccess) poolFree(p);
        { std::lock_guard<std::mutex> lk(g_reserveMu); g_reserving = 0; }
        g_reserveCv.notify_all();
    }).detach();
    return PLASSHIP_OK;
}

uint64_t plasship::newDbGeneration() { static std::atomic<uint64_t> g(0); return ++g; }

extern "C" void plasship_ctx_destroy(plasship_ctx *ctx) {
    if (!ctx) return;
    (void) hipSetDevice(ctx->device);
    (void) plasship::streamSync(ctx->stream);
    for (auto &ev : ctx->ev) if (ev) (void) hipEventDestroy(ev);
    for (int i = 0; i < 2; i++) { if (ctx->stage[i]) (void) hipHostFree(ctx->stage[i]); if (ctx->stageEv[i]) (void) hipEventDestroy(ctx->stageEv[i]); }
    if (ctx->pinnedTable) (void) hipHostFree(ctx->pinnedTable);
    { std::unique_lock<std::mutex> lk(g_reserveMu); g_reserveCv.wait(lk, [] { return g_reserving == 0; }); }
    ctx->kmCache.lines.release(); ctx->d_cmpCache.release(); ctx->d_ambKeys.release(); ctx->d_ambVals.release(); ctx->gencodeTables.clear();
    if (ctx->stream) { poolForgetStream(ctx->stream); (void) hipStreamDestroy(ctx->stream); }
    bool last; { std::lock_guard<std::mutex> g(g_poolMu); last = (--g_ctxCount <= 0); }
    if (last) {
        if (getenv("PLASSHIP_POOL_STATS")) fprintf(stderr, "plasship pool: %zu hits, %zu misses (%.1f ms in hipMalloc, %.1f MB)\n", g_poolHits, g_poolMisses, g_poolMissMs, g_poolMissBytes / 1e6);
        poolTrim();
    }
    delete ctx;
}

extern "C" int plasship_ctx_sync(plasship_ctx *ctx) {
    if (!ctx) { setError("ctx is NULL"); return PLASSHIP_ERR_ARG; }
    PH_CHECK(plasship::streamSync(ctx->stream));
    return PLASSHIP_OK;
}
extern "C" unsigned long long plasship_host_syncs(void) { return plasship::g_hostSyncs.load(); }
extern "C" void *plasship_ctx_stream(plasship_ctx *ctx) { return ctx ? (void *) ctx->stream : nullptr; }

namespace plasship {
static int stageReady(plasship_ctx *ctx) {
    if (ctx->stageBytes) return PLASSHIP_OK;
    size_t want = 32u << 20;
    if (const char *e = getenv("PLASSHIP_STAGE_MB")) { const long v = atol(e); if (v >= 1 && v <= 4096) want = (size_t) v << 20; }
    for (int i = 0; i < 2; i++) {
        PH_CHECK(hipHostMalloc((void **) &ctx->stage[i], want, hipHostMallocDefault));
        PH_CHECK(hipEventCreateWithFlags(&ctx->stageEv[i], hipEventDisableTiming));
    }
    ctx->stageBytes = want;
    return PLASSHIP_OK;
}
void *ctxPinnedTable(plasship_ctx *ctx, size_t bytes) {
    if (bytes > (1u << 20)) return nullptr;
    if (!ctx->pinnedTable && hipHostMalloc(&ctx->pinnedTable, 1u << 20, hipHostMallocDefault) != hipSuccess) { ctx->pinnedTable = nullptr; (void) hipGetLastError(); }
    return ctx->pinnedTable;
}
int stagedUpload(plasship_ctx *ctx, void *dDst, uint64_t total, const std::function<void(char *, uint64_t, uint64_t)> &produce,
                 uint64_t chunk, const std::function<int(uint64_t)> *enqueued) {
    if (!total) return PLASSHIP_OK;
    int rc = stageReady(ctx); if (rc) return rc;
    const uint64_t CH = chunk ? std::min<uint64_t>(chunk, ctx->stageBytes) : ctx->stageBytes; int b = 0; bool used[2] = {false, false};
    for (uint64_t o = 0; o < total; o += CH, b ^= 1) {
        const uint64_t n = std::min<uint64_t>(CH, total - o);
        if (used[b]) PH_CHECK(hipEventSynchronize(ctx->stageEv[b]));
        produce(ctx->stage[b], o, n);
        PH_CHECK(hipMemcpyAsync((char *) dDst + o, ctx->stage[b], n, hipMemcpyHostToDevice, ctx->stream));
        PH_CHECK(hipEventRecord(ctx->stageEv[b], ctx->stream)); used[b] = true;
        if (enqueued) { rc = (*enqueued)(o + n); if (rc) { (void) plasship::streamSync(ctx->stream); return rc; } }
    }
    PH_CHECK(plasship::streamSync(ctx->stream));
    return PLASSHIP_OK;
}
int stagedDownload(plasship_ctx *ctx, const void *dSrc, uint64_t total, const std::function<bool(const char *, uint64_t, uint64_t)> &consume) {
    if (!total) return PLASSHIP_OK;
    int rc = stageReady(ctx); if (rc) return rc;
    const uint64_t CH = ctx->stageBytes;
    auto issue = [&](uint64_t o, int b) -> int {
        const uint64_t n = std::min<uint64_t>(CH, total - o);
        PH_CHECK(hipMemcpyAsync(ctx->stage[b], (const char *) dSrc + o, n, hipMemcpyDeviceToHost, ctx->stream));
        PH_CHECK(hipEventRecord(ctx->stageEv[b], ctx->stream));
        return PLASSHIP_OK;
    };
    rc = issue(0, 0); if (rc) return rc;
    int b = 0;
    for (uint64_t o = 0; o < total; o += CH, b ^= 1) {
        if (o + CH < total) { rc = issue(o + CH, b ^ 1); if (rc) return rc; }
        PH_CHECK(hipEventSynchronize(ctx->stageEv[b]));
        if (!consume(ctx->stage[b], o, std::min<uint64_t>(CH, total - o))) { (void) plasship::streamSync(ctx->stream); return PLASSHIP_ERR_IO; }
    }
    return PLASSHIP_OK;
}
static void parallelCopy(char *dst, const char *src, uint64_t n) {
    const size_t SL = 1u << 20;
    parallelRanges((size_t) ((n + SL - 1) / SL), [&](int, size_t b, size_t e) {
        const uint64_t o = (uint64_t) b * SL, end = std::min<uint64_t>(n, (uint64_t) e * SL);
        if (end > o) memcpy(dst + o, src + o, (size_t) (end - o));
    }, nullptr, 4);
}
int stagedCopyToDevice(plasship_ctx *ctx, void *dDst, const void *hSrc, uint64_t bytes) {
    return stagedUpload(ctx, dDst, bytes, [&](char *dst, uint64_t o, uint64_t n) { parallelCopy(dst, (const char *) hSrc + o, n); });
}
int stagedCopyToHost(plasship_ctx *ctx, void *hDst, const void *dSrc, uint64_t bytes) {
    return stagedDownload(ctx, dSrc, bytes, [&](const char *src, uint64_t o, uint64_t n) { parallelCopy((char *) hDst + o, src, n); return true; });
}
}
using namespace plasship;

namespace plasship {
__global__ __launch_bounds__(256) void validateBytesKernel(const uint4 *__restrict__ data, uint64_t nWords, const uint64_t *__restrict__ off, uint64_t n, unsigned long long *__restrict__ counts) {
    unsigned long long hi = 0, zero = 0, bad = 0;
    for (uint64_t i = (uint64_t) blockIdx.x * 256 + threadIdx.x; i < nWords; i += (uint64_t) gridDim.x * 256) {
        const uint4 w = data[i];
        const uint32_t v[4] = {w.x, w.y, w.z, w.w};
#pragma unroll
        for (int j = 0; j < 4; j++) {
            const uint32_t x = v[j];
            hi += (unsigned) __popc((((x & 0x7F7F7F7Fu) + 0x05050505u) | x) & 0x80808080u);
            zero += (unsigned) __popc(~(((x & 0x7F7F7F7Fu) + 0x7F7F7F7Fu) | x | 0x7F7F7F7Fu));
        }
    }
    const char *bytes = reinterpret_cast<const char *>(data);
    for (uint64_t i = (uint64_t) blockIdx.x * 256 + threadIdx.x; i < n; i += (uint64_t) gridDim.x * 256) bad += bytes[off[i + 1] - 1] != 0;
    hi = waveReduceSumU64(hi); zero = waveReduceSumU64(zero); bad = waveReduceSumU64(bad);
    if ((threadIdx.x & 63) == 0) { if (hi) atomicAdd(&counts[0], hi); if (zero) atomicAdd(&counts[1], zero); if (bad) atomicAdd(&counts[2], bad); }
}
}

extern "C" int plasship_seqdb_upload(plasship_ctx *ctx, const char *data, size_t data_bytes, const uint64_t *off,
                                     const uint32_t *elen, const uint32_t *key, size_t n, int dbtype,
                                     plasship_seqdb **out) {
    if (!ctx || !out || (n && (!data || !off || !elen || !key))) { setError("plasship_seqdb_upload: bad argument"); return PLASSHIP_ERR_ARG; }
    if (dbtype != PLASSHIP_DBTYPE_AMINO_ACIDS && dbtype != PLASSHIP_DBTYPE_NUCLEOTIDES) {
        setError("plasship_seqdb_upload: dbtype must be amino acids (0) or nucleotides (1)"); return PLASSHIP_ERR_UNSUPPORTED;
    }
    if (n >= 0xFFFFFFFFull) { setError("plasship_seqdb_upload: too many sequences"); return PLASSHIP_ERR_UNSUPPORTED; }
    PH_ENTER(ctx);
    std::vector<uint32_t> perm(n);
    std::atomic<bool> sortedA(true);
    parallelRanges(n, [&](int, size_t b, size_t e) {
        bool ok = true;
        for (size_t i = b; i < e; i++) { perm[i] = (uint32_t) i; if (i > 0 && key[i - 1] > key[i]) ok = false; }
        if (!ok) sortedA = false;
    });
    const bool sorted = sortedA;
    const double tu0 = ioNow();
    if (!sorted) std::stable_sort(perm.begin(), perm.end(), [&](uint32_t a, uint32_t b) { return key[a] < key[b]; });
    std::unique_ptr<plasship_seqdb> holder(new plasship_seqdb());
    plasship_seqdb *db = holder.get();
    db->dbtype = dbtype; db->n = n;
    db->h_key.resize(n); db->h_elen.resize(n); db->h_off.resize(n);
    std::vector<uint32_t> hlen(n);
    uint64_t total = 0; uint32_t maxE = 0;
    {
        const int maxT = hostThreads();
        std::vector<uint64_t> rangeSum((size_t) maxT + 1, 0), rangeBeg((size_t) maxT + 1, 0); std::vector<uint32_t> rangeMax((size_t) maxT + 1, 0);
        std::vector<std::pair<size_t, size_t>> ranges((size_t) maxT + 1, std::make_pair((size_t) 0, (size_t) 0));
        std::atomic<int> bad(0);
        const int used = parallelRanges(n, [&](int t, size_t b, size_t e) {
            uint64_t sum = 0; uint32_t mx = 0;
            for (size_t i = b; i < e; i++) {
                const uint32_t sI = perm[i];
                if (off[sI] + elen[sI] > data_bytes) { bad = 1; return; }
                if (elen[sI] < 2) { bad = 2; return; }
                sum += elen[sI]; mx = std::max(mx, elen[sI]);
            }
            rangeSum[(size_t) t] = sum; rangeMax[(size_t) t] = mx; ranges[(size_t) t] = std::make_pair(b, e);
        });
        if (bad == 1) { setError("plasship_seqdb_upload: entry beyond data"); return PLASSHIP_ERR_ARG; }
        if (bad == 2) { setError("plasship_seqdb_upload: sequence entry shorter than \"\\n\\0\""); return PLASSHIP_ERR_ARG; }
        std::vector<int> order((size_t) used); for (int t = 0; t < used; t++) order[(size_t) t] = t;
        std::sort(order.begin(), order.end(), [&](int x, int y) { return ranges[(size_t) x].first < ranges[(size_t) y].first; });
        for (int q = 0; q < used; q++) { const int t = order[(size_t) q]; rangeBeg[(size_t) t] = total; total += rangeSum[(size_t) t]; maxE = std::max(maxE, rangeMax[(size_t) t]); }
        std::vector<std::pair<size_t, size_t>> rs(ranges.begin(), ranges.begin() + used);
        parallelRanges((size_t) used, [&](int, size_t qb, size_t qe) {
            for (size_t q = qb; q < qe; q++) {
                uint64_t o = rangeBeg[q];
                for (size_t i = rs[q].first; i < rs[q].second; i++) {
                    const uint32_t sI = perm[i];
                    db->h_key[i] = key[sI]; db->h_elen[i] = elen[sI]; db->h_off[i] = o; hlen[i] = elen[sI] - 2;
                    o += elen[sI];
                }
            }
        }, nullptr, 1);
    }
    db->dataBytes = total; db->maxEntryLen = maxE; db->residues = total - 2 * (uint64_t) n; db->hostIndexValid = true;
    if (db->d_data.allocLong(total + 64) != hipSuccess || db->d_off.allocLong((n + 1) * 8) != hipSuccess ||
        db->d_len.allocLong((n + 1) * 4) != hipSuccess || db->d_key.allocLong((n + 1) * 4) != hipSuccess) {
        setError("plasship_seqdb_upload: out of device memory"); return PLASSHIP_ERR_DEVICE;
    }
    const double tu1 = ioNow();
    PH_CHECK(hipMemsetAsync((char *) db->d_data.p + total, 0, 64, ctx->stream));
    {
        const uint64_t *newOff = db->h_off.data();
        const int rc = stagedUpload(ctx, db->d_data.p, total, [&](char *dst, uint64_t o, uint64_t nb) {
            const size_t first = (size_t) (std::upper_bound(newOff, newOff + n, o) - newOff) - 1;
            const size_t last = (size_t) (std::upper_bound(newOff, newOff + n, o + nb - 1) - newOff);
            parallelRanges(last - first, [&](int, size_t b, size_t e) {
// ... 206 lines not shown
```

plass_amd/csrc/device_utils.hpp:

```cpp
#pragma once
#include <hip/hip_runtime.h>
#include <cstdint>

namespace plasship {

constexpr int WAVE = 64;

__device__ __forceinline__ int laneId() { return (int) (threadIdx.x & 63); }

template <int CTRL> __device__ __forceinline__ uint32_t dppMov(uint32_t v) {
    return (uint32_t) __builtin_amdgcn_mov_dpp((int) v, CTRL, 0xF, 0xF, true);
}
template <int CTRL> __device__ __forceinline__ unsigned long long dppMov64(unsigned long long v) {
    const uint32_t lo = dppMov<CTRL>((uint32_t) v), hi = dppMov<CTRL>((uint32_t) (v >> 32));
    return ((unsigned long long) hi << 32) | lo;
}
template <int W> __device__ __forceinline__ int rowSum(int v) {
    static_assert(W == 8 || W == 16, "a row of 16 lanes or half of one");
    v += (int) dppMov<0xB1>((uint32_t) v); v += (int) dppMov<0x4E>((uint32_t) v);
    v += (int) dppMov<0x141>((uint32_t) v);
    if (W == 16) v += (int) dppMov<0x140>((uint32_t) v);
    return v;
}
template <int W> __device__ __forceinline__ unsigned long long rowMax(unsigned long long v) {
    static_assert(W == 8 || W == 16, "a row of 16 lanes or half of one");
    unsigned long long o;
    o = dppMov64<0xB1>(v); v = o > v ? o : v;
    o = dppMov64<0x4E>(v); v = o > v ? o : v;
    o = dppMov64<0x141>(v); v = o > v ? o : v;
    if (W == 16) { o = dppMov64<0x140>(v); v = o > v ? o : v; }
    return v;
}
__device__ __forceinline__ int rowSum16(int v) { return rowSum<16>(v); }
__device__ __forceinline__ unsigned long long rowMax16(unsigned long long v) { return rowMax<16>(v); }
__device__ __forceinline__ uint32_t rowMin16U32(uint32_t v) {
    uint32_t o;
    o = dppMov<0xB1>(v); v = o < v ? o : v;
    o = dppMov<0x4E>(v); v = o < v ? o : v;
    o = dppMov<0x141>(v); v = o < v ? o : v;
    o = dppMov<0x140>(v); v = o < v ? o : v;
    return v;
}
__device__ __forceinline__ uint32_t rowOr16(uint32_t v) {
    v |= dppMov<0xB1>(v); v |= dppMov<0x4E>(v); v |= dppMov<0x141>(v); v |= dppMov<0x140>(v);
    return v;
}
template <int N> struct RowCountLess {
    static __device__ __forceinline__ uint32_t run(uint32_t other, uint32_t mine) {
        return ((dppMov<0x120 + N>(other) < mine) ? 1u : 0u) + RowCountLess<N - 1>::run(other, mine);
    }
};
template <> struct RowCountLess<0> { static __device__ __forceinline__ uint32_t run(uint32_t, uint32_t) { return 0u; } };
__device__ __forceinline__ uint32_t rowCountLess16(uint32_t other, uint32_t mine, bool includeUnrotated) {
    return RowCountLess<15>::run(other, mine) + ((includeUnrotated && other < mine) ? 1u : 0u);
}

__device__ __forceinline__ uint32_t rowCountLess8(uint32_t mine) {
    const uint32_t far = dppMov<0x141>(mine);
    return ((dppMov<0x39>(mine) < mine) ? 1u : 0u) + ((dppMov<0x4E>(mine) < mine) ? 1u : 0u) + ((dppMov<0x93>(mine) < mine) ? 1u : 0u) +
           ((far < mine) ? 1u : 0u) + ((dppMov<0x39>(far) < mine) ? 1u : 0u) + ((dppMov<0x4E>(far) < mine) ? 1u : 0u) + ((dppMov<0x93>(far) < mine) ? 1u : 0u);
}

__device__ __forceinline__ int waveReduceSum(int v) {
#pragma unroll
    for (int o = 32; o > 0; o >>= 1) v += __shfl_xor(v, o, 64);
    return v;
}
__device__ __forceinline__ unsigned long long waveReduceSumU64(unsigned long long v) {
#pragma unroll
    for (int o = 32; o > 0; o >>= 1) v += __shfl_xor(v, o, 64);
    return v;
}
__device__ __forceinline__ int waveReduceMax(int v) {
#pragma unroll
    for (int o = 32; o > 0; o >>= 1) v = max(v, __shfl_xor(v, o, 64));
    return v;
}
__device__ __forceinline__ unsigned waveInclusiveScan(unsigned v) {
    const int l = laneId();
#pragma unroll
    for (int o = 1; o < 64; o <<= 1) { unsigned t = __shfl_up(v, o, 64); if (l >= o) v += t; }
    return v;
}
__device__ __forceinline__ unsigned long long waveInclusiveScanU64(unsigned long long v) {
    const int l = laneId();
#pragma unroll
    for (int o = 1; o < 64; o <<= 1) { unsigned long long t = __shfl_up(v, o, 64); if (l >= o) v += t; }
    return v;
}

__device__ __forceinline__ uint64_t loadU64Unaligned(const char *p) { uint64_t w; __builtin_memcpy(&w, p, 8); return w; }
__device__ __forceinline__ void storeU64Unaligned(char *p, uint64_t w) { __builtin_memcpy(p, &w, 8); }
__device__ __forceinline__ void storeTail(char *d, uint64_t v, unsigned r) {
    if (r & 4u) { const uint32_t x = (uint32_t) v; __builtin_memcpy(d, &x, 4); d += 4; v >>= 32; }
    if (r & 2u) { const uint16_t x = (uint16_t) v; __builtin_memcpy(d, &x, 2); d += 2; v >>= 16; }
    if (r & 1u) *d = (char) v;
}

constexpr int SCAN_BLOCK = 256;
constexpr int SCAN_ITEMS = 8;
constexpr int SCAN_TILE = SCAN_BLOCK * SCAN_ITEMS;

int exclusiveScanU32(hipStream_t stream, const uint32_t *d_in, uint64_t *d_out, size_t n, void *d_tmp, size_t tmpBytes);
size_t exclusiveScanTmpBytes(size_t n);
int exclusiveScanU64(hipStream_t stream, const uint64_t *d_in, uint64_t *d_out, size_t n, void *d_tmp, size_t tmpBytes);

}
```

plass_amd/csrc/rescore.hip:

```cpp
#include "common.hpp"
#include "device_utils.hpp"
#include "host_util.hpp"
#include "ref_rules.hpp"
#include "asm_rules.hpp"
#include <algorithm>
#include <memory>
#include <cfloat>
#include <cstring>

namespace plasship {

struct RescoreArgs {
    SeqView q, t;
    const uint64_t *qoff;
    const CandHit *hits;
    uint64_t nHits;
    AlnRec *out;
    const uint32_t *minScore;
    uint32_t minScoreLen;
    const signed char *mat;
    int sameDB, includeIdentity, reverseCapable;
    int covMode; float covThr;
    float seqIdThr; int alnLenThr, seqIdMode;
    double lambda, logK, ln2;
    unsigned long long *stats;
    unsigned long long *longList, *longCount;
    uint32_t shortMax;
    int mode, lazySelf;
    const uint32_t *queryList; uint32_t nQueryList;
};

constexpr int RS_BLOCK = 256;
constexpr uint32_t RS_SHORT_MAX = 768;

template <int G> __device__ __forceinline__ int groupReduceSumG(int v) {
#pragma unroll
    for (int o = G / 2; o > 0; o >>= 1) v += __shfl_xor(v, o, G);
    return v;
}
__device__ __forceinline__ uint32_t loadU32Unaligned(const char *p) { uint32_t w; __builtin_memcpy(&w, p, 4); return w; }

struct DiagScore { bool valid; unsigned score; int first, last; unsigned diagLen; int idCnt; };

template <bool REV, int G>
__device__ __forceinline__ DiagScore scoreDiagonal(const char *__restrict__ q, unsigned qLen, const char *__restrict__ t,
                                                   unsigned tLen, int diagonal, const signed char *__restrict__ smat, const unsigned char *__restrict__ comp, int sl) {
    DiagScore r; r.valid = false; r.score = 0; r.first = -1; r.last = -1; r.diagLen = 0; r.idCnt = 0;
    const DiagSpan sp = diagonalSpan(diagonal, qLen, tLen);
    if (!sp.hit) return r;
    const unsigned qo = sp.qo, to = sp.to, len = sp.len;
    r.valid = true; r.diagLen = len;
    if (len == 0) { r.first = 0; r.last = -1; return r; }
    auto Q = [&](unsigned i) -> char { return REV ? (char) comp[(unsigned char) q[qLen - 1 - (qo + i)]] : q[qo + i]; };
    unsigned first, last;
    int s = 0, ids = 0;
    if (G == 1) {
        auto fetchQ = [&](unsigned p, uint32_t *w) {
            if (!REV) __builtin_memcpy(w, q + qo + p, 16);
            else {
                const unsigned rem = qLen - (qo + p);
                if (rem >= 16) {
                    uint32_t v[4]; __builtin_memcpy(v, q + (qLen - 1 - (qo + p)) - 15, 16);
                    w[0] = __builtin_bswap32(v[3]); w[1] = __builtin_bswap32(v[2]); w[2] = __builtin_bswap32(v[1]); w[3] = __builtin_bswap32(v[0]);
                } else {
                    uint64_t lo = 0, hi = 0;
                    for (unsigned j = rem; j-- > 0;) { hi = (hi << 8) | (lo >> 56); lo = (lo << 8) | (uint64_t) (unsigned char) q[qLen - 1 - (qo + p + j)]; }
                    w[0] = (uint32_t) lo; w[1] = (uint32_t) (lo >> 32); w[2] = (uint32_t) hi; w[3] = (uint32_t) (hi >> 32);
                }
            }
        };
        uint32_t qn[4], tn[4];
        __builtin_memcpy(tn, t + to, 16); fetchQ(0, qn);
        const char te = t[to + len - 1];
        const char qeStored = REV ? q[qLen - 1 - (qo + len - 1)] : q[qo + len - 1];
        const char qe = REV ? (char) comp[(unsigned char) qeStored] : qeStored;
        const char t0 = (char) (tn[0] & 0xFFu);
        const char q0 = REV ? (char) comp[qn[0] & 0xFFu] : (char) (qn[0] & 0xFFu);
        first = (q0 == '*' || t0 == '*') ? 1u : 0u;
        last = len - 1;
        if (last > 0 && (qe == '*' || te == '*')) last--;
        for (unsigned p = 0; p <= last; p += 16u) {
            uint32_t qw[4], tw[4];
#pragma unroll
            for (int k = 0; k < 4; k++) { qw[k] = qn[k]; tw[k] = tn[k]; }
            if (p + 16u <= last) { __builtin_memcpy(tn, t + to + p + 16, 16); fetchQ(p + 16, qn); }
            const unsigned n = min(16u, last - p + 1);
            const unsigned skip = p ? 0u : first;
            const unsigned blanks = (16u - n) + skip;
            if (blanks) {
#pragma unroll
                for (int k = 0; k < 4; k++) {
                    const int nb = (int) n - 4 * k;
                    uint32_t m = nb >= 4 ? 0xFFFFFFFFu : (nb <= 0 ? 0u : ((1u << (8 * nb)) - 1u));
                    if (k == 0 && skip) m &= 0xFFFFFF00u;
                    qw[k] &= m; tw[k] &= m;
                }
            }
            if (!REV) {
                int z = 0;
#pragma unroll
                for (int k = 0; k < 4; k++) {
                    const uint32_t x = (qw[k] ^ tw[k]) & 0xDFDFDFDFu;
                    z += __popc(~(((x & 0x7F7F7F7Fu) + 0x7F7F7F7Fu) | x | 0x7F7F7F7Fu));
                }
                ids += z - (int) blanks;
            }
#pragma unroll
            for (unsigned j = 0; j < 16; j++) {
                unsigned a = (qw[j >> 2] >> (8 * (j & 3))) & 0xFFu;
                if (REV) a = (unsigned) comp[a];
                const unsigned b = (tw[j >> 2] >> (8 * (j & 3))) & 0xFFu;
                s += (int) smat[(a << 7) | b];
                if (REV) ids += ((a & ~0x20u) == (b & ~0x20u)) ? 1 : 0;
            }
            if (REV) ids -= (int) blanks;
        }
    } else {
    const char q0 = Q(0), t0 = t[to], qe = Q(len - 1), te = t[to + len - 1];
    first = (q0 == '*' || t0 == '*') ? 1u : 0u;
    last = len - 1;
    if (last > 0 && (qe == '*' || te == '*')) last--;
    for (unsigned p = first + 8u * (unsigned) sl; p <= last; p += 8u * G) {
        uint64_t tw; __builtin_memcpy(&tw, t + to + p, 8);
        uint64_t qw;
        if (REV) {
            const unsigned rem = qLen - (qo + p);
            if (rem >= 8) { uint64_t v; __builtin_memcpy(&v, q + (qLen - 1 - (qo + p)) - 7, 8); qw = __builtin_bswap64(v); }
            else { qw = 0; for (unsigned j = 0; j < rem; j++) qw |= (uint64_t) (unsigned char) q[qLen - 1 - (qo + p + j)] << (8 * j); }
        }
        else __builtin_memcpy(&qw, q + qo + p, 8);
        const unsigned n = min(8u, last - p + 1);
        if (n < 8u) { const uint64_t m = (1ULL << (8 * n)) - 1ULL; qw &= m; tw &= m; }
#pragma unroll
        for (unsigned j = 0; j < 8; j++) {
            unsigned a = (unsigned) (qw >> (8 * j)) & 0xFFu;
            const unsigned b = (unsigned) (tw >> (8 * j)) & 0xFFu;
            if (REV) a = (unsigned) comp[a];
            s += (int) smat[(a << 7) | b];
            ids += ((a & ~0x20u) == (b & ~0x20u)) ? 1 : 0;
        }
        ids -= (int) (8u - n);
    }
    }
    if (G > 1) { s = groupReduceSumG<G>(s); ids = groupReduceSumG<G>(ids); }
    r.score = (unsigned) max(s, 0); r.first = (int) first; r.last = (int) last; r.idCnt = ids;
    return r;
}

template <int G, int WPE, int MODE = -1>
__global__ __launch_bounds__(RS_BLOCK) __attribute__((amdgpu_waves_per_eu(WPE, WPE))) void rescoreKernel(RescoreArgs a) {
    const int mode = MODE >= 0 ? MODE : a.mode;
    __shared__ signed char smat[123 * 128];
    __shared__ unsigned char sComp[256];
    for (int i = threadIdx.x; i < 123 * 128; i += RS_BLOCK) smat[i] = (i & 127) < 123 ? a.mat[(i >> 7) * 123 + (i & 127)] : (signed char) 0;
    for (int i = threadIdx.x; i < 256; i += RS_BLOCK) sComp[i] = i ? nuclComplement((unsigned char) i) : (unsigned char) 0;
    __syncthreads();
    if (threadIdx.x == 0) smat[0] = 0;
    __syncthreads();
    const int groupsPerBlock = RS_BLOCK / G;
    const int sl = threadIdx.x & (G - 1);
    const uint64_t stride = (uint64_t) gridDim.x * groupsPerBlock;
    unsigned long long accLocal = 0, ovLocal = 0;
    const uint64_t nWork = (G == 1) ? (mode == 2 ? (uint64_t) a.nQueryList : a.nHits) : (uint64_t) *a.longCount;
    const bool finish = mode != 0;
    struct Meta { uint64_t qOff, tOff; uint32_t qLen, tLen; };
    auto loadMeta = [&](const CandHit &c) { Meta m; const uint64_t qv = a.q.offLen[c.query], tv = a.t.offLen[c.target]; m.qOff = qv >> 24; m.qLen = (uint32_t) qv & 0xFFFFFFu; m.tOff = tv >> 24; m.tLen = (uint32_t) tv & 0xFFFFFFu; return m; };
    uint64_t w = (uint64_t) blockIdx.x * groupsPerBlock + (threadIdx.x / G);
    CandHit hitNext; Meta metaNext; CandHit hitAfter;
    memset(&hitNext, 0, sizeof(hitNext)); memset(&hitAfter, 0, sizeof(hitAfter)); memset(&metaNext, 0, sizeof(metaNext));
    if (G == 1 && !finish) {
        if (w < nWork) { hitNext = a.hits[w]; metaNext = loadMeta(hitNext); }
        if (w + stride < nWork) hitAfter = a.hits[w + stride];
    }
    for (; w < nWork; w += stride) {
        uint64_t h = (G == 1) ? w : a.longList[w];
        CandHit hit; Meta me;
        if (G == 1 && mode == 2) {
            const uint32_t qq = a.queryList[w];
            uint64_t j = a.qoff[qq]; const uint64_t j1 = a.qoff[qq + 1];
            while (j < j1 && a.out[j].btKind != ALN_SELF_PENDING) j++;
            if (j == j1) continue;
            h = j;
        }
        if (finish) {
            const AlnRec stub = a.out[h];
            if (stub.btKind != ALN_SELF_PENDING) continue;
            hit.query = stub.query; hit.target = stub.target; hit.prefScore = stub.rawScore; hit.diag16 = (uint32_t) stub.qStart;
            me = loadMeta(hit);
        } else if (G == 1) {
            hit = hitNext; me = metaNext;
            hitNext = hitAfter;
            if (w + stride < nWork) metaNext = loadMeta(hitNext);
            if (w + 2 * stride < nWork) hitAfter = a.hits[w + 2 * stride];
        } else { hit = a.hits[h]; me = loadMeta(hit); }
        const uint32_t qid = hit.query, tid = hit.target;
        const char *q = a.q.data + me.qOff;
        const unsigned qLen = me.qLen;
        const char *t = a.t.data + me.tOff;
        const unsigned tLen = me.tLen;
        if (G == 1 && !finish && a.lazySelf && qid == tid && (a.includeIdentity || a.sameDB)) {
            AlnRec stub; memset(&stub, 0, sizeof(stub));
            stub.query = qid; stub.target = tid; stub.rawScore = hit.prefScore; stub.qStart = (int32_t) hit.diag16; stub.qLen = (int) qLen; stub.dbLen = (int) tLen;
            stub.accepted = 1; stub.btKind = ALN_SELF_PENDING;
            a.out[h] = stub;
            accLocal += 1;
            continue;
        }
        if (G == 1) {
            const bool toLong = min(qLen, tLen) > a.shortMax;
            const unsigned long long m = __ballot(toLong);
            if (m) {
                const int leader = __ffsll((long long) m) - 1;
                unsigned long long basePos = 0;
                if (laneId() == leader) basePos = atomicAdd(a.longCount, (unsigned long long) __popcll(m));
                basePos = __shfl(basePos, leader, 64);
                if (toLong) a.longList[basePos + (unsigned long long) __popcll(m & ((1ULL << laneId()) - 1ULL))] = h;
            }
            if (toLong) continue;
        }
        const bool isReverse = a.reverseCapable && hit.prefScore < 0;
        const bool isIdentity = (qid == tid) && (a.includeIdentity || a.sameDB);
        AlnRec rec; memset(&rec, 0, sizeof(rec));
        rec.query = qid; rec.target = tid;
        bool accepted = false;
        if (canBeCovered(a.covThr, a.covMode, (float) qLen, (float) tLen)) {
            int bStart = -1, bEnd = -1, bDiag = 0, bIds = 0; unsigned bScore = 0, bDiagLen = 0, bDist = 0;
            const unsigned d16 = hit.diag16 & 0xFFFFu;
            const unsigned nNeg = 1 + tLen / 32768, nPos = 1 + qLen / 65536;
            const unsigned nWrap = nNeg + nPos;
            auto wrapDiag = [&](unsigned c) -> int { return c < nNeg ? (int) (d16 - (c + 1) * 65536u) : (int) ((c - nNeg) * 65536u + d16); };
            auto nextWrap = [&](unsigned c) -> unsigned {
                for (; c < nWrap; c++) { const int real = wrapDiag(c); const unsigned dist = (unsigned) abs(real); if (real >= 0 ? dist < qLen : dist < tLen) break; }
                return c;
            };
            for (unsigned c = nextWrap(0); c < nWrap; c = nextWrap(c + 1)) {
                const int real = wrapDiag(c);
                const unsigned dist = (unsigned) abs(real);
                DiagScore s = isReverse ? scoreDiagonal<true, G>(q, qLen, t, tLen, real, smat, sComp, sl) : scoreDiagonal<false, G>(q, qLen, t, tLen, real, smat, sComp, sl);
                if (s.score > bScore) { bScore = s.score; bStart = s.first; bEnd = s.last; bDiag = real; bDiagLen = s.diagLen; bDist = dist; bIds = s.idCnt; }
            }
            if (sl == 0) ovLocal += bDiagLen;
            const int distance = (int) bScore;
            const int bitScore = (int) (fma(a.lambda, (double) distance, -a.logK) / a.ln2 + 0.5);
            const int alnLen = (bEnd - bStart) + 1;
            int qS, qE, dS, dE;
            if (bDiag >= 0) { qS = bStart + (int) bDist; qE = bEnd + (int) bDist; dS = bStart; dE = bEnd; }
            else { qS = bStart; qE = bEnd; dS = bStart + (int) bDist; dE = bEnd + (int) bDist; }
            const uint32_t ms = (qLen < a.minScoreLen) ? a.minScore[qLen] : 0xFFFFFFFFu;
            const bool hasEvalue = (uint32_t) distance >= ms;
            int idCnt = bIds;
            if (bStart < 0) idCnt = isIdentity ? 1 : 0;
            float seqId = 0.0f;
            if (hasEvalue || isIdentity) seqId = computeSeqId(a.seqIdMode, idCnt, (int) qLen, (int) tLen, alnLen);
            const float queryCov = computeCov((unsigned) qS, (unsigned) qE, qLen);
            const float targetCov = computeCov((unsigned) dS, (unsigned) dE, tLen);
            if (isReverse) { qS = (int) qLen - qS - 1; qE = (int) qLen - qE - 1; }
            const bool hasCov = hasCoverage(a.covThr, a.covMode, queryCov, targetCov);
            const bool hasSeqId = (double) seqId >= (double) (a.seqIdThr - FLT_EPSILON);
            const bool hasAlnLen = alnLen >= a.alnLenThr;
            accepted = isIdentity || (hasAlnLen && hasCov && hasSeqId && hasEvalue);
            rec.bitScore = bitScore; rec.rawScore = distance; rec.seqId = seqId;
            rec.qStart = qS; rec.qEnd = qE; rec.qLen = (int) qLen; rec.dbStart = dS; rec.dbEnd = dE; rec.dbLen = (int) tLen;
            rec.alnLen = alnLen; rec.reversed = isReverse ? 1 : 0;
        }
        rec.accepted = accepted ? 1 : 0; rec.btKind = 1;
        if (sl == 0) {
            a.out[h] = rec;
            accLocal += accepted ? 1 : 0;
        }
    }
    accLocal = waveReduceSumU64(accLocal); ovLocal = waveReduceSumU64(ovLocal);
    if (laneId() == 0) {
        if (accLocal) atomicAdd(&a.stats[0], accLocal);
        if (ovLocal) atomicAdd(&a.stats[1], ovLocal);
    }
}

__global__ void acceptFlagsKernel(const AlnRec *__restrict__ recs, uint32_t *__restrict__ accept, uint64_t n) {
    for (uint64_t i = (uint64_t) blockIdx.x * blockDim.x + threadIdx.x; i < n; i += (uint64_t) gridDim.x * blockDim.x) accept[i] = recs[i].accepted ? 1u : 0u;
}
__global__ void markLengthsKernel(const uint32_t *__restrict__ len, uint32_t n, uint32_t *__restrict__ present, uint32_t cap) {
    for (uint32_t i = blockIdx.x * blockDim.x + threadIdx.x; i < n; i += gridDim.x * blockDim.x) {
        uint32_t l = len[i];
        if (l < cap) present[l] = 1;
    }
}

int evalueGateTable(plasship_ctx *ctx, const char *what, const plasship_seqdb *qdb, const HostEvaluer &ev, double evalThr, DevBuf &dMinScore,
                    std::vector<uint32_t> &hMinScore) {
    const uint32_t maxQLen = qdb->maxEntryLen >= 2 ? qdb->maxEntryLen - 2 : 0;
    const uint32_t tabLen = maxQLen + 1;
    DevBuf dPresent;
    if (dPresent.alloc((size_t) tabLen * 4) != hipSuccess || dMinScore.alloc((size_t) tabLen * 4) != hipSuccess) {
        setError(std::string(what) + ": out of device memory"); return PLASSHIP_ERR_DEVICE;
    }
    PH_CHECK(hipMemsetAsync(dPresent.p, 0, (size_t) tabLen * 4, ctx->stream));
    if (qdb->n) hipLaunchKernelGGL(markLengthsKernel, dim3(std::min<size_t>(4096, (qdb->n + 255) / 256)), dim3(256), 0, ctx->stream,
                                   qdb->d_len.as<uint32_t>(), (uint32_t) qdb->n, dPresent.as<uint32_t>(), tabLen);
    std::vector<uint32_t> present(tabLen);
    hMinScore.assign(tabLen, 0xFFFFFFFFu);
    PH_CHECK(hipMemcpyAsync(present.data(), dPresent.p, (size_t) tabLen * 4, hipMemcpyDeviceToHost, ctx->stream));
    PH_CHECK(plasship::streamSync(ctx->stream));
    const int maxEntry = qdb->dbtype == PLASSHIP_DBTYPE_NUCLEOTIDES ? 2 : 11;
    int guess = -1;
    for (uint32_t l = 1; l < tabLen; l++)
        if (present[l]) { guess = ev.minScoreForEvalue(evalThr, (int) l, maxEntry * (int) l + 1, guess); hMinScore[l] = (uint32_t) guess; }
    PH_CHECK(hipMemcpyAsync(dMinScore.p, hMinScore.data(), (size_t) tabLen * 4, hipMemcpyHostToDevice, ctx->stream));
    return PLASSHIP_OK;
}

int denseAlnsCopy(plasship_ctx *ctx, const plasship_alns *a, DevBuf &qoffBuf, DevBuf &recsBuf, const uint64_t **qoff, const AlnRec **recs) {
    *qoff = a->d_qoff.as<uint64_t>(); *recs = a->d_recs.as<AlnRec>();
    if (!a->sparse) return PLASSHIP_OK;
    const uint64_t n = a->nSlots;
    DevBuf dAccept;
    if (dAccept.alloc(std::max<uint64_t>(n, 1) * 4) != hipSuccess) { setError("alignment list: out of device memory for the dense copy"); return PLASSHIP_ERR_DEVICE; }
    if (n) hipLaunchKernelGGL(acceptFlagsKernel, dim3((unsigned) std::min<uint64_t>((n + 255) / 256, (uint64_t) ctx->numCU * 32)), dim3(256), 0, ctx->stream, a->d_recs.as<AlnRec>(), dAccept.as<uint32_t>(), n);
    const int rc = compactCsr(ctx, "alignment list: the dense copy", a->d_qoff.as<uint64_t>(), a->nQueries, a->d_recs.p, sizeof(AlnRec), dAccept.as<uint32_t>(), n, a->nLines, qoffBuf, recsBuf);
    if (rc) return rc;
    *qoff = qoffBuf.as<uint64_t>(); *recs = recsBuf.as<AlnRec>();
    return PLASSHIP_OK;
}

int finishSelfAlns(plasship_ctx *ctx, const plasship_alns *al, const uint32_t *dQueryList, uint32_t nQueryList) {
    if (!al->selfPending) return PLASSHIP_OK;
    if (!al->qdb || !al->tdb) { setError("alignment list: the DBs it was made from are gone (they must outlive the list)"); return PLASSHIP_ERR_ARG; }
    const bool nucl = al->nucl;
    const uint64_t n = al->nSlots;
    DevBuf dMat, dStats, dLongList, dLongCount;
    if (dMat.alloc(123 * 123) != hipSuccess || dStats.alloc(16) != hipSuccess || dLongList.alloc(((uint64_t) al->nQueries + 1) * 8) != hipSuccess || dLongCount.alloc(8) != hipSuccess) {
        setError("alignment list: out of device memory"); return PLASSHIP_ERR_DEVICE;
    }
    PH_CHECK(hipMemsetAsync(dStats.p, 0, 16, ctx->stream));
    PH_CHECK(hipMemsetAsync(dLongCount.p, 0, 8, ctx->stream));
    PH_CHECK(hipMemcpyAsync(dMat.p, asciiSubMat(nucl), 123 * 123, hipMemcpyHostToDevice, ctx->stream));
    { int rcOL = ensureOffLen(ctx, al->qdb); if (!rcOL) rcOL = ensureOffLen(ctx, al->tdb); if (rcOL) return rcOL; }
    HostEvaluer ev(nucl, al->dbResidues);
    const plasship_rescore_params &par = al->rsPar;
    RescoreArgs a; memset(&a, 0, sizeof(a));
    a.q = al->qdb->view(); a.t = al->tdb->view(); a.qoff = al->d_qoff.as<uint64_t>(); a.hits = nullptr; a.nHits = n;
    a.out = al->d_recs.as<AlnRec>(); a.minScore = nullptr; a.minScoreLen = 0;
    a.mat = dMat.as<signed char>(); a.sameDB = al->rsSameDB; a.includeIdentity = par.include_identity; a.reverseCapable = al->rsReverseCapable;
    a.covMode = par.cov_mode; a.covThr = par.cov_thr; a.seqIdThr = par.seq_id_thr; a.alnLenThr = par.min_aln_len; a.seqIdMode = par.seq_id_mode;
    a.lambda = ev.g[0]; a.logK = ev.logK; a.ln2 = ev.ln2; a.stats = dStats.as<unsigned long long>();
    a.longList = dLongList.as<unsigned long long>(); a.longCount = dLongCount.as<unsigned long long>();
    a.shortMax = RS_SHORT_MAX;
    a.mode = dQueryList ? 2 : 1; a.lazySelf = 0; a.queryList = dQueryList; a.nQueryList = nQueryList;
    const uint64_t work = dQueryList ? (uint64_t) nQueryList : n;
    if (work) {
        const unsigned grid = (unsigned) std::min<uint64_t>((work + 255) / 256 + 1, (uint64_t) ctx->numCU * 32);
        hipLaunchKernelGGL((rescoreKernel<1, 4>), dim3(grid), dim3(RS_BLOCK), 0, ctx->stream, a);
        hipLaunchKernelGGL((rescoreKernel<16, 6>), dim3((unsigned) ctx->numCU * 8), dim3(RS_BLOCK), 0, ctx->stream, a);
    }
    PH_CHECK(plasship::streamSync(ctx->stream));
    PH_CHECK(hipGetLastError());
    if (!dQueryList) al->selfPending = false;
    return PLASSHIP_OK;
}

}
using namespace plasship;

extern "C" int plasship_rescore(plasship_ctx *ctx, const plasship_seqdb *qdb, const plasship_seqdb *tdb,
                                const plasship_cands *c, const plasship_rescore_params *par, plasship_alns **out,
                                plasship_rescore_stats *stats) {
    if (!ctx || !qdb || !tdb || !c || !par || !out) { setError("plasship_rescore: bad argument"); return PLASSHIP_ERR_ARG; }
    if (par->rescore_mode != 3) { setError("plasship_rescore: only --rescore-mode 3 (end-to-end) runs on the GPU path"); return PLASSHIP_ERR_UNSUPPORTED; }
    if (c->nQueries != qdb->n) { setError("plasship_rescore: candidate list does not belong to the query DB"); return PLASSHIP_ERR_ARG; }
    if (qdb->dbtype != tdb->dbtype) { setError("plasship_rescore: query and target DB types differ"); return PLASSHIP_ERR_ARG; }
    PH_ENTER(ctx);
    const bool nucl = qdb->dbtype == PLASSHIP_DBTYPE_NUCLEOTIDES;
    const uint64_t nHits = c->nHits;

    DevBuf dMinScore, dMat, dStats;
    std::vector<uint32_t> minScore;
    if (dMat.alloc(123 * 123) != hipSuccess || dStats.alloc(16) != hipSuccess) { setError("plasship_rescore: out of device memory"); return PLASSHIP_ERR_DEVICE; }
    PH_CHECK(hipMemsetAsync(dStats.p, 0, 16, ctx->stream));
    HostEvaluer ev(nucl, tdb->residues);
    if (const int rc = evalueGateTable(ctx, "plasship_rescore", qdb, ev, par->eval_thr, dMinScore, minScore)) return rc;
    const uint32_t tabLen = (uint32_t) minScore.size();
    PH_CHECK(hipMemcpyAsync(dMat.p, asciiSubMat(nucl), 123 * 123, hipMemcpyHostToDevice, ctx->stream));

    std::unique_ptr<plasship_alns> holder(new plasship_alns());
    plasship_alns *al = holder.get();
    al->nQueries = qdb->n; al->nucl = nucl; al->addBacktrace = par->add_backtrace != 0; al->dbResidues = tdb->residues;
    if (al->d_qoff.alloc((qdb->n + 1) * 8) != hipSuccess || al->d_recs.alloc(std::max<uint64_t>(nHits, 1) * sizeof(AlnRec)) != hipSuccess) {
        setError("plasship_rescore: out of device memory"); return PLASSHIP_ERR_DEVICE;
    }

    { int rcOL = ensureOffLen(ctx, qdb); if (!rcOL) rcOL = ensureOffLen(ctx, tdb); if (rcOL) return rcOL; }
    RescoreArgs a;
    a.q = qdb->view(); a.t = tdb->view(); a.qoff = c->d_qoff.as<uint64_t>(); a.hits = c->d_hits.as<CandHit>(); a.nHits = nHits;
    a.out = al->d_recs.as<AlnRec>(); a.minScore = dMinScore.as<uint32_t>(); a.minScoreLen = tabLen;
    a.mat = dMat.as<signed char>(); a.sameDB = (qdb == tdb); a.includeIdentity = par->include_identity; a.reverseCapable = c->reverseCapable;
    a.covMode = par->cov_mode; a.covThr = par->cov_thr; a.seqIdThr = par->seq_id_thr; a.alnLenThr = par->min_aln_len; a.seqIdMode = par->seq_id_mode;
    a.lambda = ev.g[0]; a.logK = ev.logK; a.ln2 = ev.ln2; a.stats = dStats.as<unsigned long long>();
    DevBuf dLongList, dLongCount;
    if (dLongList.alloc(std::max<uint64_t>(nHits, 1) * 8) != hipSuccess || dLongCount.alloc(8) != hipSuccess) { setError("plasship_rescore: out of device memory"); return PLASSHIP_ERR_DEVICE; }
    PH_CHECK(hipMemsetAsync(dLongCount.p, 0, 8, ctx->stream));
    a.longList = dLongList.as<unsigned long long>(); a.longCount = dLongCount.as<unsigned long long>();
    a.shortMax = RS_SHORT_MAX;
    a.mode = 0; a.lazySelf = tuneInt("LAZY_SELF", 1) == 1 ? 1 : 0;
    const unsigned grid = (unsigned) std::min<uint64_t>((nHits + 255) / 256 + 1, (uint64_t) ctx->numCU * (nHits > 50000000ull ? 32u : 12u));
    PH_CHECK(hipEventRecord(ctx->ev[0], ctx->stream));
    hipLaunchKernelGGL((rescoreKernel<1, 4, 0>), dim3(grid), dim3(RS_BLOCK), 0, ctx->stream, a);
    hipLaunchKernelGGL((rescoreKernel<16, 6>), dim3((unsigned) ctx->numCU * 8), dim3(RS_BLOCK), 0, ctx->stream, a);
    PH_CHECK(hipEventRecord(ctx->ev[1], ctx->stream));
    PH_CHECK(hipMemcpyAsync(al->d_qoff.p, c->d_qoff.p, (qdb->n + 1) * 8, hipMemcpyDeviceToDevice, ctx->stream));
    unsigned long long hs[2] = {0, 0};
    PH_CHECK(hipMemcpyAsync(hs, dStats.p, 16, hipMemcpyDeviceToHost, ctx->stream));
    PH_CHECK(plasship::streamSync(ctx->stream));
    PH_CHECK(hipGetLastError());
    const uint64_t nAcc = hs[0];
    al->nLines = nAcc; al->nSlots = nHits; al->sparse = true;
    al->qdb = qdb; al->tdb = tdb;
    al->selfPending = a.lazySelf != 0 && (a.sameDB || a.includeIdentity); al->rsPar = *par; al->rsSameDB = (qdb == tdb); al->rsReverseCapable = c->reverseCapable;
    if (stats) {
        stats->n_scored = nHits; stats->n_accepted = nAcc; stats->overlap_residues = hs[1];
        float ms = 0; (void) hipEventElapsedTime(&ms, ctx->ev[0], ctx->ev[1]); stats->ms_kernel = ms;
    }
    *out = holder.release();
    return PLASSHIP_OK;
}
```

Before: 776.2 million.

## Hand over per-query arena sums and pre-screen from rescore to assemble

```diff
diff --git a/plass_amd/csrc/asm_rules.hpp b/plass_amd/csrc/asm_rules.hpp
--- a/plass_amd/csrc/asm_rules.hpp
+++ b/plass_amd/csrc/asm_rules.hpp
@@ -61,6 +61,19 @@
 PLASSHIP_AR_HD unsigned rightFragLen(unsigned tLen, int dbEnd) { return tLen - ((unsigned) dbEnd + 1); }
 PLASSHIP_AR_HD bool canExtendRight(unsigned fragR, int qEnd, unsigned qLen) { return fragR > 0 && (unsigned) qEnd == (qLen - 1); }
 PLASSHIP_AR_HD bool canExtendLeft(int dbStart, int dbEnd, unsigned tLen) { return dbStart > 0 && (unsigned) dbEnd == (tLen - 1); }
+constexpr unsigned PRESCREEN_NO_LEFT = 0xFFFFFFFFu;
+struct PreScreen { bool right = false; unsigned left = PRESCREEN_NO_LEFT; };
+PLASSHIP_AR_HD PreScreen preScreenOf(const AlnCoords &c, unsigned qLen, unsigned dbLen) {
+    PreScreen p;
+    if (isBranchType(c.qStart, c.qEnd, qLen, c.dbStart, c.dbEnd, dbLen)) {
+        if (c.dbStart == 0) p.right = canExtendRight(rightFragLen(dbLen, c.dbEnd), c.qEnd, qLen);
+        else if (c.qStart == 0 && canExtendLeft(c.dbStart, c.dbEnd, dbLen)) p.left = (unsigned) c.dbStart;
+    }
+    return p;
+}
+PLASSHIP_AR_HD bool preScreenPasses(bool right, unsigned minLeft, unsigned qLen, unsigned long long maxSeqLen) {
+    return right || (minLeft != PRESCREEN_NO_LEFT && (unsigned long long) qLen + (unsigned long long) minLeft < maxSeqLen);
+}
 PLASSHIP_AR_HD bool deferredRight(unsigned fragR, int qEnd, unsigned qLen, unsigned rightOff) {
     return fragR > rightOff && (unsigned) qEnd == (qLen - 1) && rightOff > 0;
 }
diff --git a/plass_amd/csrc/assemble.hip b/plass_amd/csrc/assemble.hip
--- a/plass_amd/csrc/assemble.hip
+++ b/plass_amd/csrc/assemble.hip
@@ -1220,7 +1220,6 @@
 
 __global__ __launch_bounds__(256) void arenaSumKernel(const AlnRec *__restrict__ recs, uint64_t nAln, uint64_t maxSeqLen, unsigned long long *__restrict__ qSum,
                                                       unsigned long long *__restrict__ qSumAa, uint32_t *__restrict__ qCan, int mirror) {
-    const int lane = laneId();
     for (uint64_t i = (uint64_t) blockIdx.x * blockDim.x + threadIdx.x; i < nAln; i += (uint64_t) gridDim.x * blockDim.x) {
         const AlnRec r = recs[i];
         const uint32_t id = r.query;
@@ -1229,48 +1228,45 @@
             add = (uint32_t) r.dbLen; addAa = (uint32_t) r.dbLen / 3 + 2;
             AlnCoords c; c.qStart = r.qStart; c.qEnd = r.qEnd; c.dbStart = r.dbStart; c.dbEnd = r.dbEnd;
             if (mirror && c.qStart > c.qEnd) c = mirrorReverseHit(r.qStart, r.qEnd, r.dbStart, r.dbEnd, (unsigned) r.dbLen);
-            if (isBranchType(c.qStart, c.qEnd, (unsigned) r.qLen, c.dbStart, c.dbEnd, (unsigned) r.dbLen)) {
-                if (c.dbStart == 0) can = canExtendRight(rightFragLen((unsigned) r.dbLen, c.dbEnd), c.qEnd, (unsigned) r.qLen);
-                else if (c.qStart == 0) can = canExtendLeft(c.dbStart, c.dbEnd, (unsigned) r.dbLen) && ((uint64_t) r.qLen + (uint64_t) c.dbStart < maxSeqLen);
-            }
-        }
-        const unsigned long long act = __ballot(1);
-        const uint32_t prevId = (uint32_t) __shfl_up((int) id, 1, 64);
-        const bool head = lane == 0 || prevId != id;
-        const unsigned long long heads = __ballot(head), cans = __ballot(can);
-        const int segStart = 63 - __clzll((long long) (heads & (lane == 63 ? ~0ULL : ((2ULL << lane) - 1ULL))));
-        const unsigned long long later = lane == 63 ? 0ULL : (heads & ~((2ULL << lane) - 1ULL));
-        const int segEnd = (later ? __ffsll((long long) later) - 1 : (int) __popcll(act)) - 1;
-#pragma unroll
-        for (int d = 1; d < 64; d <<= 1) {
-            const uint32_t t = (uint32_t) __shfl_up((int) add, d, 64), ta = (uint32_t) __shfl_up((int) addAa, d, 64);
-            if (lane - d >= segStart) { add += t; addAa += ta; }
-        }
-        if (lane == segEnd) {
-            const unsigned long long seg = (segEnd == 63 ? ~0ULL : ((2ULL << segEnd) - 1ULL)) & ~((1ULL << segStart) - 1ULL);
+            const PreScreen p = preScreenOf(c, (unsigned) r.qLen, (unsigned) r.dbLen);
+            can = preScreenPasses(p.right, p.left, (unsigned) r.qLen, maxSeqLen);
+        }
+        const WaveSegment seg = waveSegmentOf(id);
+        const unsigned long long cans = __ballot(can);
+        add = segmentScanSum(add, seg); addAa = segmentScanSum(addAa, seg);
+        if (laneId() == seg.last) {
             if (add) atomicAdd(&qSum[id], (unsigned long long) add);
             if (qSumAa && addAa) atomicAdd(&qSumAa[id], (unsigned long long) addAa);
-            if (cans & seg) atomicOr(&qCan[id], 1u);
+            if (cans & seg.lanes) atomicOr(&qCan[id], 1u);
         }
     }
 }
 constexpr int N_TIERS = 5;
 constexpr uint8_t TIER_NARROW = 4, TIER_NONE = 0xFF;
 __global__ void arenaSizeKernel(SeqView s, const uint64_t *__restrict__ qoff, const unsigned long long *__restrict__ qSum, const unsigned long long *__restrict__ qSumAa,
-                                const uint32_t *__restrict__ qCan, uint32_t *__restrict__ leftCap,
+                                const uint32_t *__restrict__ qCan, const uint32_t *__restrict__ qCanRight, const uint32_t *__restrict__ qMinLeft, uint64_t maxSeqLen,
+                                uint32_t *__restrict__ leftCap,
                                 uint64_t *__restrict__ bytes, int nuclTiers, uint64_t threadBytes,
                                 uint8_t *__restrict__ tierOf,
                                 const uint32_t *__restrict__ aaLen, uint32_t *__restrict__ aaLeftCap, uint64_t *__restrict__ aaBytes) {
     for (uint32_t id = blockIdx.x * blockDim.x + threadIdx.x; id < s.n; id += gridDim.x * blockDim.x) {
         int tier = -1;
         const uint64_t sum = qSum[id], sumAa = aaBytes ? qSumAa[id] : 0;
-        const bool can = qCan[id] != 0;
+        const bool can = qCan ? qCan[id] != 0 : preScreenPasses(qCanRight[id] != 0, qMinLeft[id], s.len[id], maxSeqLen);
         leftCap[id] = (uint32_t) std::min<uint64_t>(sum, 0xFFFFFFFFull);
         const uint64_t slice = (sum && can) ? (2 * sum + s.len[id] + 40) : 0;
         bytes[id] = slice;
         if (aaBytes) { aaLeftCap[id] = (uint32_t) std::min<uint64_t>(sumAa, 0xFFFFFFFFull); aaBytes[id] = (sum && can) ? (2 * sumAa + aaLen[id] + 8) : 0; }
         if (sum && can) { const uint64_t h = qoff[id + 1] - qoff[id]; tier = nuclTiers ? ((h <= 256 && slice <= threadBytes) ? 0 : 1) : (h <= 8 ? (int) TIER_NARROW : (h <= 16 ? 0 : (h <= 32 ? 1 : (h <= 64 ? 2 : 3)))); }
         tierOf[id] = (tier < 0) ? TIER_NONE : (uint8_t) tier;
+    }
+}
+__global__ void handoverDiffKernel(SeqView s, const unsigned long long *__restrict__ qSum, const uint32_t *__restrict__ qCan, const uint8_t *__restrict__ tierOf,
+                                   const unsigned long long *__restrict__ lSum, const uint32_t *__restrict__ lCanRight, const uint32_t *__restrict__ lMinLeft,
+                                   const uint8_t *__restrict__ lTierOf, uint64_t maxSeqLen, uint32_t *__restrict__ firstDiff) {
+    for (uint32_t id = blockIdx.x * blockDim.x + threadIdx.x; id < s.n; id += gridDim.x * blockDim.x) {
+        const bool can = preScreenPasses(lCanRight[id] != 0, lMinLeft[id], s.len[id], maxSeqLen);
+        if (qSum[id] != lSum[id] || (qCan[id] != 0) != can || tierOf[id] != lTierOf[id]) atomicMin(firstDiff, id);
     }
 }
 static_assert(SCAN_TILE < (1 << 12) && N_TIERS * 12 <= 64 && SCAN_BLOCK == 256, "tier counters of a tile: 12-bit fields of one 64-bit word");
@@ -1725,7 +1721,7 @@
 
 static bool asmHistOn() { return getenv("PLASSHIP_DEBUG_ASMHIST") != nullptr; }
 static int asmHistRecord(hipStream_t st, uint32_t N, const uint64_t *dQoff, const uint32_t *dBigList, uint32_t nBig, const uint32_t *dRounds, const uint32_t *dCycles,
-                         uint32_t cap, const uint32_t *tierQueries) {
+                         uint32_t cap, const uint32_t *tierQueries, bool handed) {
     static int call = 0;
     std::vector<uint32_t> ids(nBig), rounds(N), cycles(N);
     std::vector<uint64_t> qoff((size_t) N + 1);
@@ -1754,6 +1750,7 @@
     for (int k = 0; k < NR; k++) s += " " + std::to_string(rq[k]);
     s += " | tier queries <=8,<=16,<=32,<=64,more:";
     for (int t = 0; t < 5; t++) s += " " + std::to_string(tierQueries[t]);
+    s += handed ? " | pass 1: handed over by rescorediagonal" : " | pass 1: arenaSumKernel";
     fprintf(stderr, "%s\n", s.c_str());
     return PLASSHIP_OK;
 }
@@ -1792,18 +1789,39 @@
     if (dBigList.alloc(((size_t) N + 1) * 4) != hipSuccess || dMidList.alloc(((size_t) N + 1) * 4) != hipSuccess || dMid32List.alloc(((size_t) N + 1) * 4) != hipSuccess ||
         dSmallList.alloc(((size_t) N + 1) * 4) != hipSuccess || (!nucl && dNarrowList.alloc(((size_t) N + 1) * 4) != hipSuccess) || dTierOf.alloc((size_t) N + 8) != hipSuccess ||
         dTierPart.alloc(((size_t) N_TIERS * (nTiles + 1) + 1) * 8) != hipSuccess) { setError("plasship_assemble: out of device memory"); return PLASSHIP_ERR_DEVICE; }
+    const int handover = tuneInt("HANDOVER", 1);
+    const bool handed = handover != 2 && !nucl && !guided && al->d_qSum.p && al->qdb == db && al->tdb == db && al->handoverGen == db->gen;
+    const bool summed = !handed || handover == 3;
     DevBuf dQSum, dQSumAa, dQCan;
-    if (dQSum.alloc(((size_t) N + 1) * 8) != hipSuccess || dQCan.alloc(((size_t) N + 1) * 4) != hipSuccess || (guided && dQSumAa.alloc(((size_t) N + 1) * 8) != hipSuccess)) { setError("plasship_assemble: out of device memory"); return PLASSHIP_ERR_DEVICE; }
-    PH_CHECK(hipMemsetAsync(dQSum.p, 0, ((size_t) N + 1) * 8, st));
-    PH_CHECK(hipMemsetAsync(dQCan.p, 0, ((size_t) N + 1) * 4, st));
-    if (guided) PH_CHECK(hipMemsetAsync(dQSumAa.p, 0, ((size_t) N + 1) * 8, st));
-    if (nLines) hipLaunchKernelGGL(arenaSumKernel, dim3((unsigned) std::min<uint64_t>((nLines + 255) / 256, (uint64_t) ctx->numCU * 32)), dim3(256), 0, st, al->d_recs.as<AlnRec>(), (uint64_t) nLines,
+    if (summed) {
+        if (dQSum.alloc(((size_t) N + 1) * 8) != hipSuccess || dQCan.alloc(((size_t) N + 1) * 4) != hipSuccess || (guided && dQSumAa.alloc(((size_t) N + 1) * 8) != hipSuccess)) { setError("plasship_assemble: out of device memory"); return PLASSHIP_ERR_DEVICE; }
+        PH_CHECK(hipMemsetAsync(dQSum.p, 0, ((size_t) N + 1) * 8, st));
+        PH_CHECK(hipMemsetAsync(dQCan.p, 0, ((size_t) N + 1) * 4, st));
+        if (guided) PH_CHECK(hipMemsetAsync(dQSumAa.p, 0, ((size_t) N + 1) * 8, st));
+        if (nLines) hipLaunchKernelGGL(arenaSumKernel, dim3((unsigned) std::min<uint64_t>((nLines + 255) / 256, (uint64_t) ctx->numCU * 32)), dim3(256), 0, st, al->d_recs.as<AlnRec>(), (uint64_t) nLines,
                                        (uint64_t) par->max_seq_len, dQSum.as<unsigned long long>(), guided ? dQSumAa.as<unsigned long long>() : (unsigned long long *) nullptr, dQCan.as<uint32_t>(),
                                        (nucl && !guided) ? 1 : 0);
-    if (N) hipLaunchKernelGGL(arenaSizeKernel, dim3(std::min<uint32_t>((N + 255) / 256, 8192)), dim3(256), 0, st, sv, al->d_qoff.as<uint64_t>(), (const unsigned long long *) dQSum.as<unsigned long long>(),
-                              (const unsigned long long *) dQSumAa.as<unsigned long long>(), (const uint32_t *) dQCan.as<uint32_t>(), dLeftCap.as<uint32_t>(), dBytes.as<uint64_t>(), nucl ? 1 : 0, (uint64_t) 1 << 30,
-                              dTierOf.as<uint8_t>(),
-                              guided ? aaDb->d_len.as<uint32_t>() : (const uint32_t *) nullptr, dAaLeftCap.as<uint32_t>(), guided ? dAaBytes.as<uint64_t>() : (uint64_t *) nullptr);
+    }
+    auto sizeArena = [&](bool fromList, uint8_t *tierOf) {
+        if (N) hipLaunchKernelGGL(arenaSizeKernel, dim3(std::min<uint32_t>((N + 255) / 256, 8192)), dim3(256), 0, st, sv, al->d_qoff.as<uint64_t>(),
+                                  (const unsigned long long *) (fromList ? al->d_qSum : dQSum).as<unsigned long long>(), (const unsigned long long *) dQSumAa.as<unsigned long long>(),
+                                  fromList ? (const uint32_t *) nullptr : (const uint32_t *) dQCan.as<uint32_t>(), (const uint32_t *) al->d_qCanRight.as<uint32_t>(), (const uint32_t *) al->d_qMinLeft.as<uint32_t>(),
+                                  (uint64_t) par->max_seq_len, dLeftCap.as<uint32_t>(), dBytes.as<uint64_t>(), nucl ? 1 : 0, (uint64_t) 1 << 30, tierOf,
+                                  guided ? aaDb->d_len.as<uint32_t>() : (const uint32_t *) nullptr, dAaLeftCap.as<uint32_t>(), guided ? dAaBytes.as<uint64_t>() : (uint64_t *) nullptr);
+    };
+    if (handed && summed) {
+        DevBuf dTierWalked, dFirstDiff;
+        if (dTierWalked.alloc((size_t) N + 8) != hipSuccess || dFirstDiff.alloc(4) != hipSuccess) { setError("plasship_assemble: out of device memory"); return PLASSHIP_ERR_DEVICE; }
+        PH_CHECK(hipMemsetAsync(dFirstDiff.p, 0xFF, 4, st));
+        sizeArena(false, dTierWalked.as<uint8_t>());
+        sizeArena(true, dTierOf.as<uint8_t>());
+        if (N) hipLaunchKernelGGL(handoverDiffKernel, dim3(std::min<uint32_t>((N + 255) / 256, 8192)), dim3(256), 0, st, sv, (const unsigned long long *) dQSum.as<unsigned long long>(), (const uint32_t *) dQCan.as<uint32_t>(),
+                                  (const uint8_t *) dTierWalked.as<uint8_t>(), (const unsigned long long *) al->d_qSum.as<unsigned long long>(), (const uint32_t *) al->d_qCanRight.as<uint32_t>(),
+                                  (const uint32_t *) al->d_qMinLeft.as<uint32_t>(), (const uint8_t *) dTierOf.as<uint8_t>(), (uint64_t) par->max_seq_len, dFirstDiff.as<uint32_t>());
+        uint32_t firstDiff = 0xFFFFFFFFu;
+        PH_COPY_SYNC(st, &firstDiff, dFirstDiff.p, 4, hipMemcpyDeviceToHost);
+        if (firstDiff != 0xFFFFFFFFu) { setError("plasship_assemble: the sums or the pre-screen handed over by plasship_rescore differ from arenaSumKernel's, first at query " + std::to_string(firstDiff)); return PLASSHIP_ERR_DEVICE; }
+    } else sizeArena(handed, dTierOf.as<uint8_t>());
     if (guided && exclusiveScanU64(st, dAaBytes.as<uint64_t>(), dAaArenaOff.as<uint64_t>(), N, dTmp.p, tmpBytes)) { setError("plasship_assemble: scan failed"); return PLASSHIP_ERR_DEVICE; }
     PH_CHECK(hipMemsetAsync(dTierPart.p, 0, ((size_t) N_TIERS * (nTiles + 1) + 1) * 8, st));
     if (nTiles) hipLaunchKernelGGL(tierCountKernel, dim3(nTiles), dim3(SCAN_BLOCK), 0, st, (const uint8_t *) dTierOf.as<uint8_t>(), N, dTierPart.as<uint64_t>(), nTiles);
@@ -1942,7 +1960,7 @@
         hipLaunchKernelGGL(assembleBigKernel, gBig, dim3(256), 0, st, o);
     } else if (a.nBig) hipLaunchKernelGGL(assembleBigKernel, gBig, dim3(256), 0, st, a);
     PH_CHECK(hipEventRecord(ctx->ev[7], st));
-    if (hist) { const int rcH = asmHistRecord(st, N, a.qoff, a.bigList, a.nBig, a.dbgRounds, a.dbgCycles, onChip ? qCap : 64, tierQ); if (rcH) return rcH; }
+    if (hist) { const int rcH = asmHistRecord(st, N, a.qoff, a.bigList, a.nBig, a.dbgRounds, a.dbgCycles, onChip ? qCap : 64, tierQ, handed); if (rcH) return rcH; }
     }
     PH_TRACE(st, "assemble: extension kernels");
     plasship_seqdb *o = nullptr, *oAa = nullptr;
diff --git a/plass_amd/csrc/common.hpp b/plass_amd/csrc/common.hpp
--- a/plass_amd/csrc/common.hpp
+++ b/plass_amd/csrc/common.hpp
@@ -200,6 +200,8 @@
     int gappedOpen = 0, gappedExtend = 0;
     plasship::DevBuf d_qoff;
     plasship::DevBuf d_recs;
+    plasship::DevBuf d_qSum, d_qCanRight, d_qMinLeft;
+    uint64_t handoverGen = 0;
     const plasship_seqdb *qdb = nullptr, *tdb = nullptr;
 };
 
diff --git a/plass_amd/csrc/core.hip b/plass_amd/csrc/core.hip
--- a/plass_amd/csrc/core.hip
+++ b/plass_amd/csrc/core.hip
@@ -170,7 +170,7 @@
     return v > 0 ? v : dflt;
 }
 static const char *const TUNE_NAMES[] = {"AGGWAVE", "AGGWAVE_CAP", "ASMQ", "ASMQ_CAP", "ROWTIER", "KMCACHE", "FORCE_LONG", "CYC_PASSES", "CYCSKIP", "SHARD_EXTRACT",
-                                         "FASTA_CHUNK_MB", "DBHEAP", "DBHEAP_GB", "LAZY_SELF", "FASTQ_CHUNK_KB", "PART_BITS", "GROUP_SHAPE"};
+                                         "FASTA_CHUNK_MB", "DBHEAP", "DBHEAP_GB", "LAZY_SELF", "FASTQ_CHUNK_KB", "PART_BITS", "GROUP_SHAPE", "HANDOVER"};
 static void reportUnknownTunes() {
     static const char PREFIX[] = "PLASSHIP_TUNE_";
     for (char **e = environ; e && *e; e++) {
diff --git a/plass_amd/csrc/device_utils.hpp b/plass_amd/csrc/device_utils.hpp
--- a/plass_amd/csrc/device_utils.hpp
+++ b/plass_amd/csrc/device_utils.hpp
@@ -89,6 +89,33 @@
     return v;
 }
 
+struct WaveSegment { int first, last; unsigned long long lanes; };
+__device__ __forceinline__ WaveSegment waveSegmentOf(uint32_t key) {
+    const int lane = laneId();
+    const unsigned long long act = __ballot(1);
+    const uint32_t prev = (uint32_t) __shfl_up((int) key, 1, 64);
+    const unsigned long long heads = __ballot(lane == 0 || prev != key);
+    const unsigned long long upTo = lane == 63 ? ~0ULL : ((2ULL << lane) - 1ULL);
+    WaveSegment s;
+    s.first = 63 - __clzll((long long) (heads & upTo));
+    const unsigned long long later = heads & ~upTo;
+    s.last = (later ? __ffsll((long long) later) - 1 : (int) __popcll(act)) - 1;
+    s.lanes = (s.last == 63 ? ~0ULL : ((2ULL << s.last) - 1ULL)) & ~((1ULL << s.first) - 1ULL);
+    return s;
+}
+__device__ __forceinline__ uint32_t segmentScanSum(uint32_t v, const WaveSegment &s) {
+    const int lane = laneId();
+#pragma unroll
+    for (int d = 1; d < 64; d <<= 1) { const uint32_t t = (uint32_t) __shfl_up((int) v, d, 64); if (lane - d >= s.first) v += t; }
+    return v;
+}
+__device__ __forceinline__ uint32_t segmentScanMin(uint32_t v, const WaveSegment &s) {
+    const int lane = laneId();
+#pragma unroll
+    for (int d = 1; d < 64; d <<= 1) { const uint32_t t = (uint32_t) __shfl_up((int) v, d, 64); if (lane - d >= s.first && t < v) v = t; }
+    return v;
+}
+
 __device__ __forceinline__ uint64_t loadU64Unaligned(const char *p) { uint64_t w; __builtin_memcpy(&w, p, 8); return w; }
 __device__ __forceinline__ void storeU64Unaligned(char *p, uint64_t w) { __builtin_memcpy(p, &w, 8); }
 __device__ __forceinline__ void storeTail(char *d, uint64_t v, unsigned r) {
diff --git a/plass_amd/csrc/rescore.hip b/plass_amd/csrc/rescore.hip
--- a/plass_amd/csrc/rescore.hip
+++ b/plass_amd/csrc/rescore.hip
@@ -28,6 +28,7 @@
     uint32_t shortMax;
     int mode, lazySelf;
     const uint32_t *queryList; uint32_t nQueryList;
+    unsigned long long *qSum; uint32_t *qCanRight, *qMinLeft;
 };
 
 constexpr int RS_BLOCK = 256;
@@ -173,18 +174,20 @@
         if (w + stride < nWork) hitAfter = a.hits[w + stride];
     }
     for (; w < nWork; w += stride) {
+        uint32_t hoQuery = 0, hoAdd = 0; PreScreen hoScreen;
+        do {
         uint64_t h = (G == 1) ? w : a.longList[w];
         CandHit hit; Meta me;
         if (G == 1 && mode == 2) {
             const uint32_t qq = a.queryList[w];
             uint64_t j = a.qoff[qq]; const uint64_t j1 = a.qoff[qq + 1];
             while (j < j1 && a.out[j].btKind != ALN_SELF_PENDING) j++;
-            if (j == j1) continue;
+            if (j == j1) break;
             h = j;
         }
         if (finish) {
             const AlnRec stub = a.out[h];
-            if (stub.btKind != ALN_SELF_PENDING) continue;
+            if (stub.btKind != ALN_SELF_PENDING) break;
             hit.query = stub.query; hit.target = stub.target; hit.prefScore = stub.rawScore; hit.diag16 = (uint32_t) stub.qStart;
             me = loadMeta(hit);
         } else if (G == 1) {
@@ -194,6 +197,7 @@
             if (w + 2 * stride < nWork) hitAfter = a.hits[w + 2 * stride];
         } else { hit = a.hits[h]; me = loadMeta(hit); }
         const uint32_t qid = hit.query, tid = hit.target;
+        hoQuery = qid;
         const char *q = a.q.data + me.qOff;
         const unsigned qLen = me.qLen;
         const char *t = a.t.data + me.tOff;
@@ -204,7 +208,7 @@
             stub.accepted = 1; stub.btKind = ALN_SELF_PENDING;
             a.out[h] = stub;
             accLocal += 1;
-            continue;
+            break;
         }
         if (G == 1) {
             const bool toLong = min(qLen, tLen) > a.shortMax;
@@ -216,7 +220,7 @@
                 basePos = __shfl(basePos, leader, 64);
                 if (toLong) a.longList[basePos + (unsigned long long) __popcll(m & ((1ULL << laneId()) - 1ULL))] = h;
             }
-            if (toLong) continue;
+            if (toLong) break;
         }
         const bool isReverse = a.reverseCapable && hit.prefScore < 0;
         const bool isIdentity = (qid == tid) && (a.includeIdentity || a.sameDB);
@@ -262,11 +266,29 @@
             rec.bitScore = bitScore; rec.rawScore = distance; rec.seqId = seqId;
             rec.qStart = qS; rec.qEnd = qE; rec.qLen = (int) qLen; rec.dbStart = dS; rec.dbEnd = dE; rec.dbLen = (int) tLen;
             rec.alnLen = alnLen; rec.reversed = isReverse ? 1 : 0;
+            if (a.qSum && accepted && qid != tid) {
+                AlnCoords c; c.qStart = rec.qStart; c.qEnd = rec.qEnd; c.dbStart = rec.dbStart; c.dbEnd = rec.dbEnd;
+                hoAdd = tLen; hoScreen = preScreenOf(c, qLen, tLen);
+            }
         }
         rec.accepted = accepted ? 1 : 0; rec.btKind = 1;
         if (sl == 0) {
             a.out[h] = rec;
             accLocal += accepted ? 1 : 0;
+        }
+        } while (false);
+        if (a.qSum) {
+            auto handOver = [&](uint32_t add, bool right, uint32_t minLeft) {
+                if (add) atomicAdd(&a.qSum[hoQuery], (unsigned long long) add);
+                if (right) atomicOr(&a.qCanRight[hoQuery], 1u);
+                if (minLeft != PRESCREEN_NO_LEFT) atomicMin(&a.qMinLeft[hoQuery], minLeft);
+            };
+            if (G == 1 && MODE == 0) {
+                const WaveSegment seg = waveSegmentOf(hoQuery);
+                const unsigned long long rights = __ballot(hoScreen.right);
+                const uint32_t add = segmentScanSum(hoAdd, seg), minLeft = segmentScanMin(hoScreen.left, seg);
+                if (laneId() == seg.last) handOver(add, (rights & seg.lanes) != 0, minLeft);
+            } else if (sl == 0) handOver(hoAdd, hoScreen.right, hoScreen.left);
         }
     }
     accLocal = waveReduceSumU64(accLocal); ovLocal = waveReduceSumU64(ovLocal);
@@ -388,8 +410,20 @@
         setError("plasship_rescore: out of device memory"); return PLASSHIP_ERR_DEVICE;
     }
 
+    const bool handOver = !nucl && qdb == tdb && qdb->n > 0;
+    if (handOver) {
+        if (al->d_qSum.alloc(qdb->n * 8) != hipSuccess || al->d_qCanRight.alloc(qdb->n * 4) != hipSuccess || al->d_qMinLeft.alloc(qdb->n * 4) != hipSuccess) {
+            setError("plasship_rescore: out of device memory"); return PLASSHIP_ERR_DEVICE;
+        }
+        PH_CHECK(hipMemsetAsync(al->d_qSum.p, 0, qdb->n * 8, ctx->stream));
+        PH_CHECK(hipMemsetAsync(al->d_qCanRight.p, 0, qdb->n * 4, ctx->stream));
+        PH_CHECK(hipMemsetAsync(al->d_qMinLeft.p, 0xFF, qdb->n * 4, ctx->stream));
+        al->handoverGen = qdb->gen;
+    }
+
     { int rcOL = ensureOffLen(ctx, qdb); if (!rcOL) rcOL = ensureOffLen(ctx, tdb); if (rcOL) return rcOL; }
-    RescoreArgs a;
+    RescoreArgs a; memset(&a, 0, sizeof(a));
+    a.qSum = al->d_qSum.as<unsigned long long>(); a.qCanRight = al->d_qCanRight.as<uint32_t>(); a.qMinLeft = al->d_qMinLeft.as<uint32_t>();
     a.q = qdb->view(); a.t = tdb->view(); a.qoff = c->d_qoff.as<uint64_t>(); a.hits = c->d_hits.as<CandHit>(); a.nHits = nHits;
     a.out = al->d_recs.as<AlnRec>(); a.minScore = dMinScore.as<uint32_t>(); a.minScoreLen = tabLen;
     a.mat = dMat.as<signed char>(); a.sameDB = (qdb == tdb); a.includeIdentity = par->include_identity; a.reverseCapable = c->reverseCapable;
```

New measurement: 782.8 million (median of 6 runs). No clear change (+0.9%).
